# techmum21p/hybrid-rag-ColBERTv2

Measured on AMD Instinct MI355X. Metric: queries/sec + p50 retrieval latency, 1M-chunk corpus, top-10 rerank, higher is better.
Workload: dtype fp32 (faithful: bf16 hi/lo split, fp32 accumulate)

## Files before the change

hybrid-rag-colbertv2_amd/_lib.py:

```python
from __future__ import annotations

import ctypes
import os
import re

PKG = os.path.dirname(os.path.abspath(__file__))
LIB_PATH = os.path.join(PKG, "libcolbert_mi355x.so")
HEADER = os.path.join(os.path.dirname(PKG), "include", "colbert_mi355x.h")

DTYPE_BF16 = 1
DTYPE_F32 = 2
DTYPE_MXFP8 = 3
SCORER_MAXSIM = 0
SCORER_REF_MEANPOOL_COSINE = 1
SCORERS = {"maxsim": SCORER_MAXSIM, "ref_meanpool_cosine": SCORER_REF_MEANPOOL_COSINE}
ERR_EINVAL, ERR_EUNSUPPORTED, ERR_EHIP, ERR_ESTATE = -1, -2, -3, -4
F32_SCORE, F32_SEARCH, F32_RERANK = 0, 1, 2
(OPT_FUSED_TOPK, OPT_DYNAMIC_TAIL, OPT_BAND_DOC_MAJOR, OPT_BAND_LOWER_BOUND, OPT_TOPK_BMAX, OPT_BAND_FUSED,
 OPT_RESCORE_SPLIT, OPT_BAND_REUSE, OPT_BAND_BLOCK_SKIP, OPT_RESCORE_GRID, OPT_DENSE_DOCS, OPT_P1_COLLECT_FUSED,
 OPT_FOLD_KEYS, OPT_FILTER_PATH, OPT_FILTER_BATCH_CHUNK_DOCS, OPT_FILTER_BAND) = (1, 2, 3, 4, 5, 6, 7, 8, 9, 10, 11, 12,
                                                                                 13, 14, 15, 16)
FILTER_AUTO, FILTER_SUBSET, FILTER_DENSE = 0, 1, 2
FILTER_BAND_AUTO, FILTER_BAND_ON, FILTER_BAND_OFF = 0, 1, 2

_p, _i32, _i64, _sz = ctypes.c_void_p, ctypes.c_int32, ctypes.c_int64, ctypes.c_size_t
_SIGS = {
    "cbv2_abi_version": (ctypes.c_int, []),
    "cbv2_last_error": (ctypes.c_char_p, []),
    "cbv2_build_stamp": (ctypes.c_char_p, []),
    "cbv2_index_create": (ctypes.c_int, [ctypes.c_int, _p, _i32, _i64, _i32, _i32, _p, _i64,
                                         ctypes.POINTER(ctypes.c_void_p)]),
    "cbv2_index_destroy": (ctypes.c_int, [_p]),
    "cbv2_hbm_alloc": (ctypes.c_int, [ctypes.c_int, ctypes.c_size_t, ctypes.POINTER(ctypes.c_void_p),
                                      ctypes.POINTER(ctypes.c_int32)]),
    "cbv2_hbm_free": (ctypes.c_int, [ctypes.c_int, _p]),
    "cbv2_index_time_scans": (ctypes.c_int, [_p, _i32]),
    "cbv2_index_scan_times": (ctypes.c_int, [_p, _p, _i32, ctypes.POINTER(ctypes.c_int32)]),
    "cbv2_index_band_times": (ctypes.c_int, [_p, _p, _i32, ctypes.POINTER(ctypes.c_int32)]),
    "cbv2_index_scan_clock": (ctypes.c_int, [_p, _p, _i32]),
    "cbv2_index_create_mxfp8": (ctypes.c_int, [ctypes.c_int, _p, _p, _i64, _i32, _i32, _p, _i64,
                                               ctypes.POINTER(ctypes.c_void_p)]),
    "cbv2_quantize_mxfp8": (ctypes.c_int, [_p, _i32, _i64, _p, _p, _p]),
    "cbv2_index_build_means": (ctypes.c_int, [_p, _p, _i32, _p, _p]),
    "cbv2_score": (ctypes.c_int, [_p, _i32, _p, _i32, _i32, _i32, _p, _i64, _p]),
    "cbv2_search_workspace_bytes": (_sz, [_p, _i32]),
    "cbv2_search_workspace_size": (_sz, [_p, _i32, _i32, _i32]),
    "cbv2_index_set_option": (ctypes.c_int, [_p, _i32, _i64]),
    "cbv2_search_fused_slots": (_i64, [_p, _i32, _i32, _i32]),
    "cbv2_index_last_scan_plan": (ctypes.c_int, [_p, _p]),
    "cbv2_search": (ctypes.c_int, [_p, _i32, _p, _i32, _i32, _i32, _i32, _p, _sz, _p, _p, _p]),
    "cbv2_filter_bytes": (_sz, [_i64]),
    "cbv2_filter_create": (ctypes.c_int, [_p, _p, _p, _sz, _p, ctypes.POINTER(ctypes.c_void_p)]),
    "cbv2_filter_count": (_i64, [_p]),
    "cbv2_filter_destroy": (ctypes.c_int, [_p]),
    "cbv2_search_filtered_workspace_size": (_sz, [_p, _p, _i32, _i32, _i32, _i32]),
    "cbv2_search_filtered": (ctypes.c_int, [_p, _p, _i32, _p, _i32, _i32, _i32, _i32, _p, _sz, _p, _p, _p]),
    "cbv2_search_filtered_f32_workspace_size": (_sz, [_p, _p, _i32, _i32, _i32, _i32]),
    "cbv2_search_filtered_f32": (ctypes.c_int, [_p, _p, _p, _i32, _i32, _i32, _i32, _p, _sz, _p, _p, _p, _p]),
    "cbv2_filter_batch_bytes": (_sz, [_i32]),
    "cbv2_filter_batch_create": (ctypes.c_int, [_p, _p, _i32, _p, _sz, _p, ctypes.POINTER(ctypes.c_void_p)]),
    "cbv2_filter_batch_pairs": (_i64, [_p]),
    "cbv2_filter_batch_max_count": (_i64, [_p]),
    "cbv2_filter_batch_destroy": (ctypes.c_int, [_p]),
    "cbv2_search_filtered_batch_workspace_size": (_sz, [_p, _p, _i32, _i32, _i32, _i32]),
    "cbv2_search_filtered_batch": (ctypes.c_int, [_p, _p, _i32, _p, _i32, _i32, _i32, _i32, _p, _sz, _p, _p, _p]),
    "cbv2_rerank": (ctypes.c_int, [_p, _p, _i32, _i32, _p, _i32, _i32, _p, _p, _p, _p]),
    "cbv2_rerank_workspace_bytes": (_sz, [_i32, _i32]),
    "cbv2_rerank_ws": (ctypes.c_int, [_p, _p, _i32, _i32, _p, _i32, _i32, _p, _sz, _p, _p, _p, _p]),
    "cbv2_select_topk": (ctypes.c_int, [_p, _p, _i32, _i32, _i32, _p, _p, _p, _p]),
    "cbv2_topk_workspace_bytes": (_sz, [_i32, _i64]),
    "cbv2_topk_rows": (ctypes.c_int, [_p, _i32, _i64, _i64, _i32, _i64, _p, _sz, _p, _p, _p]),
    "cbv2_merge_topk": (ctypes.c_int, [_p, _p, _i32, _i32, _i32, _p, _p, _p]),
    "cbv2_rrf_fuse": (ctypes.c_int, [_p, _i32, _p, _i32, _i32, _i32, _i32, _p, _p, _p]),
    "cbv2_bm25_build": (ctypes.c_int, [_p, _p, _i64, _i32, ctypes.c_float, ctypes.c_float,
                                       ctypes.POINTER(ctypes.c_void_p)]),
    "cbv2_bm25_search": (ctypes.c_int, [_p, _p, _p, _i32, _i32, _i32, _p, _p]),
    "cbv2_bm25_search_filtered": (ctypes.c_int, [_p, _p, _p, _i32, _i32, _i32, _p, _p, _p]),
    "cbv2_bm25_search_filtered_batch": (ctypes.c_int, [_p, _p, _p, _i32, _i32, _i32, _p, _p, _p]),
    "cbv2_bm25_doc_freq": (ctypes.c_int, [_p, _p, _i64, _i32, _p]),
    "cbv2_bm25_build_shard": (ctypes.c_int, [_p, _p, _i64, _i32, ctypes.c_float, ctypes.c_float, _i64, _i64,
                                             _i64, _p, ctypes.POINTER(ctypes.c_void_p)]),
    "cbv2_bm25_num_docs": (_i64, [_p]),
    "cbv2_stem_en": (ctypes.c_int, [_p, _p, _i64, _p, _i64, _p]),
    "cbv2_index_file_info": (ctypes.c_int, [ctypes.c_char_p, _p, _p, _p]),
    "cbv2_index_file_write": (ctypes.c_int, [ctypes.c_char_p, _i32, _i64, _p, _p, _p, _i64, _p]),
    "cbv2_index_file_read": (ctypes.c_int, [ctypes.c_char_p, _i64, _i64, _p, _p, _p, _p]),
    "cbv2_index_file_write_host": (ctypes.c_int, [ctypes.c_char_p, _i32, _i64, _p, _p, _p, _i64]),
    "cbv2_index_file_read_host": (ctypes.c_int, [ctypes.c_char_p, _i64, _i64, _p, _p, _p]),
    "cbv2_index_writer_open": (ctypes.c_int, [ctypes.c_char_p, _i32, _i64, _i64, ctypes.POINTER(ctypes.c_void_p)]),
    "cbv2_index_file_info_ld": (ctypes.c_int, [ctypes.c_char_p, _p, _p, _p, _p]),
    "cbv2_index_file_write_ld": (ctypes.c_int, [ctypes.c_char_p, _i32, _i64, _i32, _p, _p, _p, _i64, _p]),
    "cbv2_index_file_write_host_ld": (ctypes.c_int, [ctypes.c_char_p, _i32, _i64, _i32, _p, _p, _p, _i64]),
    "cbv2_index_writer_open_ld": (ctypes.c_int, [ctypes.c_char_p, _i32, _i64, _i32, _i64,
                                                 ctypes.POINTER(ctypes.c_void_p)]),
    "cbv2_index_writer_append": (ctypes.c_int, [_p, _i64, _p, _p, _p, _i32, _p]),
    "cbv2_index_writer_count": (_i64, [_p]),
    "cbv2_index_writer_close": (ctypes.c_int, [_p]),
    "cbv2_comm_init": (ctypes.c_int, [_p, ctypes.c_char_p, ctypes.POINTER(ctypes.c_void_p)]),
    "cbv2_comm_loopback_init": (ctypes.c_int, [_i32, ctypes.POINTER(ctypes.c_void_p)]),
    "cbv2_comm_size": (ctypes.c_int, [_p]),
    "cbv2_comm_rank": (ctypes.c_int, [_p]),
    "cbv2_comm_destroy": (ctypes.c_int, [_p]),
    "cbv2_sharded_workspace_bytes": (_sz, [_p, _p, _i32, _i32, _i32, _i32]),
    "cbv2_search_sharded": (ctypes.c_int, [_p, _p, _i32, _p, _i32, _i32, _i32, _i32, _p, _p, _i32, _p, _sz, _p, _p,
                                           _p, _p]),
    "cbv2_search_sharded_local": (ctypes.c_int, [_p, _p, _i32, _p, _i32, _i32, _i32, _i32, _i32, _p, _sz, _p]),
    "cbv2_search_sharded_exchange": (ctypes.c_int, [_p, _p, _p, _i32, _i32, _i32, _i32, _p, _p, _i32, _p, _sz, _p,
                                                    _p, _p, _p]),
    "cbv2_rerank_sharded": (ctypes.c_int, [_p, _p, _p, _i32, _i32, _p, _i32, _i32, _p, _sz, _p, _p, _p, _p]),
    "cbv2_rerank_sharded_prescored": (ctypes.c_int, [_p, _p, _i32, _i32, _i32, _p, _i32, _i32, _p, _sz, _p, _p, _p,
                                                     _p, _p]),
    "cbv2_comm_stats": (ctypes.c_int, [_p, _p]),
    "cbv2_bm25_destroy": (ctypes.c_int, [_p]),
    "cbv2_split_f32": (ctypes.c_int, [_p, _i64, _i32, _p, _p, _p, _p, _p]),
    "cbv2_index_attach_residual": (ctypes.c_int, [_p, _p, ctypes.c_float, ctypes.c_float]),
    "cbv2_f32_workspace_bytes": (_sz, [_p, _i32, _i32, _i32, _i32]),
    "cbv2_score_f32": (ctypes.c_int, [_p, _p, _i32, _i32, _p, _sz, _p, _i64, _p]),
    "cbv2_search_f32": (ctypes.c_int, [_p, _p, _i32, _i32, _i32, _i32, _p, _sz, _p, _p, _p, _p]),
    "cbv2_search_f32_begin": (ctypes.c_int, [_p, _p, _i32, _i32, _i32, _i32, _p, _sz, _p, _p, _p, _p, _p]),
    "cbv2_search_f32_finish": (ctypes.c_int, [_p, _i32, _i32, _i32, _i32, _p, _sz, _p, _p, _p, _p, _p]),
    "cbv2_rerank_f32": (ctypes.c_int, [_p, _p, _i32, _i32, _p, _i32, _i32, _p, _sz, _p, _p, _p, _p]),
    "cbv2_index_kind": (ctypes.c_int, [_p, ctypes.POINTER(ctypes.c_int32), ctypes.POINTER(ctypes.c_int32)]),
    "cbv2_retrieve_workspace_bytes": (_sz, [_p, _p, _i32, _i32, _i32, _i32, _i32]),
    "cbv2_retrieve_host_bytes": (_sz, [_i32, _i32, _i32, _i32]),
    "cbv2_retrieve_host_marks": (ctypes.c_int, [_p, _i32]),
    "cbv2_retrieve_cancel": (ctypes.c_int, [_p, _p, _p]),
    "cbv2_retrieve_pool_stats": (ctypes.c_int, [_p, _i32]),
    "cbv2_retrieve_begin": (ctypes.c_int, [_p, _p, _p, _i32, _i32, _i32, _i32, _i32, _i32, _p, _sz, _p]),
    "cbv2_retrieve_finish": (ctypes.c_int, [_p, _p, _p, _i32, _i32, _i32, _i32, _p, _p, _i32, _i32, _i32, _i32,
                                            _p, _sz, _p, _sz, _p, _p, _p, _p]),
    "cbv2_retrieve_finish_host": (ctypes.c_int, [_p, _p, _p, _i32, _i32, _i32, _i32, _p, _p, _i32, _i32, _i32,
                                                 _i32, _p, _sz, _p, _sz, _p, _p, _p, _p, _p, _p, _p]),
}

_lib = None


def header_symbols(path: str = HEADER):
    text = open(path).read()
    return sorted(set(re.findall(r"^\s*(?:[\w\s\*]+?)\b(cbv2_\w+)\s*\(", text, re.M)))


def lib():
    global _lib
    if _lib is None:
        from . import _build
        if not os.path.exists(LIB_PATH):
            raise RuntimeError(f"{LIB_PATH} is not built: run `python -c 'import __graft_entry__ as g; g.build()'`")
        want, have = _build.source_stamp(), _build.library_stamp(LIB_PATH)
        if have != want:
            raise RuntimeError(f"{LIB_PATH} was built from other sources (stamp {have}, sources {want}): "
                               "rebuild with `python -c 'import __graft_entry__ as g; g.build()'`")
        L = ctypes.CDLL(LIB_PATH)
        for name, (res, args) in _SIGS.items():
            fn = getattr(L, name)
            fn.restype = res
            fn.argtypes = args
        _lib = L
    return _lib


class Cbv2Error(RuntimeError):
    def __init__(self, code: int, msg: str):
        super().__init__(f"cbv2 error {code}: {msg}")
        self.code = code


def check(rc: int):
    if rc != 0:
        msg = lib().cbv2_last_error().decode(errors="replace")
        if rc == ERR_EINVAL:
            raise ValueError(msg)
        raise Cbv2Error(rc, msg)
    return rc
```

hybrid-rag-colbertv2_amd/csrc/colbert_mi355x.hip:

```cpp
#include <hip/hip_runtime.h>

#include <stdarg.h>
#include <stdint.h>

#include <algorithm>
#include <atomic>
#include <mutex>
#include <type_traits>
#include <vector>
#include <stdio.h>
#include <string.h>

#include "colbert_mi355x.h"

namespace {

constexpr int kDim = 128;
constexpr int kLd = 128;
constexpr int kLqMax = 32;
constexpr int kRowBytes = kDim * 2;
constexpr int kDocBytes = kLd * kRowBytes;
constexpr int kTopkMax = 1024;
constexpr int kSmallMax = 1024;
constexpr int kMergeMax = 8192;
// ... 3407 lines not shown
  const int b = blockIdx.y;
  const int c = blockIdx.x * kRrWaves + wave;
  if (c >= C) return;
  const int32_t id = cand[(size_t)b * C + c];
  float v;
  if constexpr (F8) {
    i32x8 qa[1][2];
    int qs[1][2];
    load_qfrag_f8(Qb, Qs, b, b + 1, lq, lane, qa[0], qs[0]);
    v = rerank_one_f8(tokens, tscales, doclens, n, id_base, qa, qs, lq, id, lane, ld);
  } else {
    bf16x8 qf[1][2][4];
    load_qfrag16(reinterpret_cast<const uint16_t*>(Qb), b, b + 1, lq, lane, qf[0]);
    v = rerank_one_bf16(tokens, doclens, n, id_base, qf, lq, id, lane, ld);
  }
  if (lane == 0) raw[(size_t)b * C + c] = v;
}

__global__ __launch_bounds__(256, 2) void rerank_split_kernel(
    const uint8_t* __restrict__ tokens, const int32_t* __restrict__ doclens, int64_t n, int64_t id_base,
    const uint16_t* __restrict__ Q, int lq, const int32_t* __restrict__ cand, int C, float* __restrict__ raw, int ld,
    TaggedCand tc = TaggedCand(), Mirror raw_words = Mirror()) {
  __shared__ float s_m[4][32];
  __shared__ int32_t s_cid;
  const int lane = threadIdx.x & 63, g = lane >> 4, c16 = lane & 15;
  const int wave = __builtin_amdgcn_readfirstlane(threadIdx.x >> 6);
  const int b = blockIdx.y, c = blockIdx.x;
  int32_t id;
  if (tc.w != nullptr) {
    if (threadIdx.x == 0) s_cid = wait_tagged(tc.w + (size_t)b * C + c, tc);
    __syncthreads();
    id = s_cid;
  } else {
    id = cand[(size_t)b * C + c];
  }
  const int64_t loc = (int64_t)id - id_base;
  if (id < 0 || loc < 0 || loc >= n) {
    if (threadIdx.x == 0) {
      raw[(size_t)b * C + c] = neg_inf();
      if (raw_words.w != nullptr) raw_words.put((size_t)b * C + c, (int32_t)__float_as_uint(neg_inf()), 0.0f);
    }
    return;
  }
  bf16x8 qf[1][2][4];
  load_qfrag16(Q, b, b + 1, lq, lane, qf[0]);
  int dl = doclens[loc];
  float m[1][2] = {{neg_inf(), neg_inf()}};
  for (int blk = 0; blk == 0 || kLd * blk < dl; ++blk) {
    const uint8_t* dbase = tokens + (size_t)loc * (size_t)ld * kRowBytes + (size_t)blk * kDocBytes;
    bf16x8 af[2][4];
#pragma unroll
    for (int t = 0; t < 2; ++t)
      if (blk == 0 || 16 * (2 * wave + t) < dl - kLd * blk) gbl_afrag16(dbase, 2 * wave + t, lane, af[t]);
    if (blk == 0) dl = dl < 0 ? 0 : (dl > ld ? ld : dl);
    const int dlb = dl - kLd * blk;
#pragma unroll
    for (int t = 0; t < 2; ++t) {
      const int rt = 2 * wave + t;
      if (16 * rt < dlb) {
        const f32x4 init = (dlb >= 16 * rt + 16) ? f32x4{} : row_mask_init16(16 * rt + 4 * g, dlb);
        tile16<1>(af[t], qf, init, m);
      }
    }
  }
  const float w0 = fold16_max(fold32_max(m[0][0])), w1 = fold16_max(fold32_max(m[0][1]));
  if (lane < 16) {
    s_m[wave][lane] = w0;
    s_m[wave][16 + lane] = w1;
  }
  __syncthreads();
  if (wave == 0) {
    const float m0 = fmaxf(fmaxf(s_m[0][c16], s_m[1][c16]), fmaxf(s_m[2][c16], s_m[3][c16]));
    const float m1 = fmaxf(fmaxf(s_m[0][16 + c16], s_m[1][16 + c16]), fmaxf(s_m[2][16 + c16], s_m[3][16 + c16]));
    const float v = dpp_row_sum16((c16 < lq ? m0 : 0.0f) + (16 + c16 < lq ? m1 : 0.0f));
    if (lane == 0) {
      raw[(size_t)b * C + c] = v;
      if (raw_words.w != nullptr) raw_words.put((size_t)b * C + c, (int32_t)__float_as_uint(v), 0.0f);
    }
  }
}

constexpr float kBoundUp = 1.0f + 1.0f / 1024.0f;
constexpr float kAccSlack = 1.0f / 4096.0f;

__device__ __forceinline__ void split_row8(const float* __restrict__ src, uint16_t* __restrict__ hi,
                                           uint16_t* __restrict__ lo, int sub, float& xx, float& rr, float& hh) {
  const f32x4* s4 = reinterpret_cast<const f32x4*>(src + 8 * sub);
  const f32x4 v0 = s4[0], v1 = s4[1];
  float x[8] = {v0[0], v0[1], v0[2], v0[3], v1[0], v1[1], v1[2], v1[3]};
  uint16_t h[8], l[8];
  xx = rr = hh = 0.0f;
#pragma unroll
  for (int e = 0; e < 8; ++e) {
    const __bf16 bh = (__bf16)x[e];
    const float fh = (float)bh;
    const float r = x[e] - fh;
    const __bf16 bl = (__bf16)r;
    h[e] = __builtin_bit_cast(uint16_t, bh);
    l[e] = __builtin_bit_cast(uint16_t, bl);
    xx += x[e] * x[e];
    rr += r * r;
    hh += fh * fh;
  }
  u32x4 ph, pl;
#pragma unroll
  for (int e = 0; e < 4; ++e) {
    ph[e] = (uint32_t)h[2 * e] | ((uint32_t)h[2 * e + 1] << 16);
    pl[e] = (uint32_t)l[2 * e] | ((uint32_t)l[2 * e + 1] << 16);
  }
  *reinterpret_cast<u32x4*>(hi + 8 * sub) = ph;
  *reinterpret_cast<u32x4*>(lo + 8 * sub) = pl;
#pragma unroll
  for (int off = 1; off < 16; off <<= 1) {
    xx += __shfl_xor(xx, off);
    rr += __shfl_xor(rr, off);
    hh += __shfl_xor(hh, off);
  }
}

__global__ __launch_bounds__(256) void split_f32_kernel(const float* __restrict__ x, int64_t rows, int ld,
                                                        const int32_t* __restrict__ doclens,
                                                        uint16_t* __restrict__ hi, uint16_t* __restrict__ lo,
                                                        float* __restrict__ bounds) {
  const int sub = threadIdx.x & 15;
  float rmax = 0.0f, hmax = 0.0f;
  for (int64_t r = ((int64_t)blockIdx.x * blockDim.x + threadIdx.x) >> 4; r < rows;
       r += ((int64_t)gridDim.x * blockDim.x) >> 4) {
    float xx, rr, hh;
    split_row8(x + r * kDim, hi + r * kDim, lo + r * kDim, sub, xx, rr, hh);
    if (doclens == nullptr || (int)(r % ld) < doclens[r / ld]) {
      rmax = fmaxf(rmax, sqrtf(rr) * kBoundUp);
      hmax = fmaxf(hmax, sqrtf(hh) * kBoundUp);
    }
  }
#pragma unroll
  for (int off = 16; off < 64; off <<= 1) {
    rmax = fmaxf(rmax, __shfl_xor(rmax, off));
    hmax = fmaxf(hmax, __shfl_xor(hmax, off));
  }
  if ((threadIdx.x & 63) == 0) {
    atomicMax(reinterpret_cast<unsigned int*>(bounds), __float_as_uint(rmax));
    atomicMax(reinterpret_cast<unsigned int*>(bounds) + 1, __float_as_uint(hmax));
  }
}

constexpr int kArriveSlotsK = 4;
constexpr int kArrPhase1K = 3;
constexpr int64_t kSplitZeroInts = 16384;
__global__ __launch_bounds__(512) void split_query_kernel(const float* __restrict__ Q, int lq,
                                                          uint16_t* __restrict__ qhi, uint16_t* __restrict__ qlo,
                                                          float E, float M, float* __restrict__ beta,
                                                          int32_t* __restrict__ count = nullptr,
                                                          uint32_t* __restrict__ lbu = nullptr,
                                                          int32_t* __restrict__ done = nullptr, int count0 = 0,
                                                          int32_t* __restrict__ arrive = nullptr, int narrive = 0,
                                                          int* __restrict__ ctr = nullptr, int nctr = 0,
                                                          uint32_t ready_seq = 0, int nrows = 0,
                                                          uint32_t* __restrict__ zkeys = nullptr, int64_t nz = 0,
                                                          int32_t* __restrict__ ready_words = nullptr) {
  __shared__ float s_t[kLqMax];
  const int b = blockIdx.x, tid = threadIdx.x, r = tid >> 4, sub = tid & 15;
  if (nrows > 0 && b >= nrows) {
    const int64_t per = kSplitZeroInts, i0 = (int64_t)(b - nrows) * per;
    for (int64_t i = i0 + 4 * tid; i < i0 + per && i < nz; i += 4 * blockDim.x) {
      if (i + 3 < nz)
        *reinterpret_cast<uint4*>(zkeys + i) = make_uint4(0u, 0u, 0u, 0u);
      else
        for (int64_t e = i; e < nz; ++e) zkeys[e] = 0u;
    }
    return;
  }
  if (r < lq) {
    const size_t row = (size_t)b * lq + r;
    float xx, rr, hh;
    split_row8(Q + row * kDim, qhi + row * kDim, qlo + row * kDim, sub, xx, rr, hh);
    const float nq = sqrtf(xx) * kBoundUp, eq = sqrtf(rr) * kBoundUp;
    const float t = nq * E + eq * M + kAccSlack * (nq + eq) * M;
    if (sub == 0) s_t[r] = t;
  }
  __syncthreads();
  if (tid == 0) {
    float a[4];
#pragma unroll
    for (int g = 0; g < 4; ++g) {
      a[g] = 0.0f;
      for (int rr = g; rr < lq; rr += 4) a[g] += s_t[rr];
    }
    beta[b] = ((a[0] + a[1]) + (a[2] + a[3])) * kBoundUp;
    if (count != nullptr) count[b] = count0;
    if (lbu != nullptr) lbu[b] = 0xffffffffu;
    if (done != nullptr) done[b] = 0;
  }
  if (arrive != nullptr) {
    const int per = narrive / kArriveSlotsK;
    for (int i = tid; i < narrive; i += blockDim.x) {
      const int j = i / per, e = i - j * per;
      arrive[((size_t)j * nrows + b) * per + e] = 0;
    }
  }
  if (ctr != nullptr && b == 0)
    for (int i = tid; i < nctr; i += blockDim.x) ctr[i] = 0;
  if (ready_seq != 0 && ready_words != nullptr) {
    __syncthreads();
    if (tid == 0) {
      __threadfence();
      asm volatile("s_waitcnt vmcnt(0)" ::: "memory");
      __hip_atomic_store(ready_words + b, (int32_t)ready_seq, __ATOMIC_RELAXED, __HIP_MEMORY_SCOPE_SYSTEM);
    }
  }
}

__device__ __forceinline__ void tile16_x3(const bf16x8 (&ah)[4], const bf16x8 (&al)[4], const bf16x8 (&qh)[2][4],
                                          const bf16x8 (&ql)[2][4], const f32x4& init, float (&m)[2]) {
#pragma unroll
  for (int ct = 0; ct < 2; ++ct) {
    f32x4 acc = init;
#pragma unroll
    for (int s = 0; s < 4; ++s) acc = __builtin_amdgcn_mfma_f32_16x16x32_bf16(al[s], qh[ct][s], acc, 0, 0, 0);
#pragma unroll
    for (int s = 0; s < 4; ++s) acc = __builtin_amdgcn_mfma_f32_16x16x32_bf16(ah[s], ql[ct][s], acc, 0, 0, 0);
#pragma unroll
    for (int s = 0; s < 4; ++s) acc = __builtin_amdgcn_mfma_f32_16x16x32_bf16(ah[s], qh[ct][s], acc, 0, 0, 0);
    m[ct] = fmaxf(fmaxf(m[ct], fmaxf(acc[0], acc[1])), fmaxf(acc[2], acc[3]));
  }
}

template <bool LONG>
__device__ __forceinline__ float faithful_doc16(const uint8_t* __restrict__ hi, const uint8_t* __restrict__ lo,
                                                int64_t loc, int ld, int dl, const bf16x8 (&qh)[2][4],
                                                const bf16x8 (&ql)[2][4], int lane, int lq) {
  const int g = lane >> 4;
  const int lmax = LONG ? ld : kLd;
  float m[2] = {neg_inf(), neg_inf()};
  for (int blk = 0; blk == 0 || (LONG && kLd * blk < dl); ++blk) {
    const int dlb = dl - kLd * blk;
    const size_t at = ((size_t)loc * lmax + (size_t)kLd * blk) * kRowBytes;
    const uint8_t* dh = hi + at;
    const uint8_t* dlo = lo + at;
#pragma unroll
    for (int half = 0; half < 2; ++half) {
      bf16x8 ah[4][4], al[4][4];
#pragma unroll
      for (int t = 0; t < 4; ++t) {
        const int rt = 4 * half + t;
        if (16 * rt < dlb) {
          gbl_afrag16(dh, rt, lane, ah[t]);
          gbl_afrag16(dlo, rt, lane, al[t]);
        }
      }
#pragma unroll
      for (int t = 0; t < 4; ++t) {
        const int rt = 4 * half + t;
        if (16 * rt < dlb) {
          const f32x4 init = (dlb >= 16 * rt + 16) ? f32x4{} : row_mask_init16(16 * rt + 4 * g, dlb);
          tile16_x3(ah[t], al[t], qh, ql, init, m);
        }
      }
    }
  }
  return reduce16(m[0], m[1], lane, lq);
}

constexpr int kRsPerWave = 4;
template <bool LONG = false>
__global__ __launch_bounds__(256, 2) void rescore_x3_kernel(
    const uint8_t* __restrict__ hi, const uint8_t* __restrict__ lo, const int32_t* __restrict__ doclens, int64_t n,
    int64_t id_base, const uint16_t* __restrict__ qhi, const uint16_t* __restrict__ qlo, int lq,
    const int32_t* __restrict__ cand, const int32_t* __restrict__ count, int64_t limit, int64_t ld_c,
    float* __restrict__ out, int64_t ld_out, const int32_t* __restrict__ only_neg, int ld, int pw,
    uint32_t* __restrict__ lb_min) {
  const int lane = threadIdx.x & 63;
  const int wave = __builtin_amdgcn_readfirstlane(threadIdx.x >> 6);
  const int b = blockIdx.y;
  if (only_neg != nullptr && only_neg[b] >= 0) return;
  int64_t lim = limit;
  if (count != nullptr) {
    const int64_t cb = count[b];
    lim = cb < lim ? cb : lim;
  }
  const int64_t step = (int64_t)gridDim.x * 4 * pw;
  int64_t c0 = ((int64_t)blockIdx.x * 4 + wave) * pw;
  if (c0 >= lim) return;
  bf16x8 qh[2][4], ql[2][4];
  load_qfrag16(qhi, b, b + 1, lq, lane, qh);
  load_qfrag16(qlo, b, b + 1, lq, lane, ql);
  for (; c0 < lim; c0 += step)
  for (int64_t c = c0; c < c0 + pw && c < lim; ++c) {
    const int64_t id = cand ? (int64_t)cand[b * ld_c + c] : id_base + c;
    const int64_t loc = id - id_base;
    float v = neg_inf();
    if (id >= 0 && loc >= 0 && loc < n) {
      const int lmax = LONG ? ld : kLd;
      int dl = doclens[loc];
      dl = dl < 0 ? 0 : (dl > lmax ? lmax : dl);
      v = faithful_doc16<LONG>(hi, lo, loc, ld, dl, qh, ql, lane, lq);
    }
    if (lane == 0) {
      out[(size_t)b * ld_out + c] = v;
      if (lb_min != nullptr) atomicMin(lb_min + b, f2u(v));
    }
  }
}

template <bool LONG, int NW = 4>
__device__ __forceinline__ float faithful_doc_split(const uint8_t* __restrict__ hi, const uint8_t* __restrict__ lo,
                                                    int64_t loc, int ld, int dl, const bf16x8 (&qh)[2][4],
                                                    const bf16x8 (&ql)[2][4], int lane, int wave, int lq,
                                                    float (&s_m)[4][32]) {
  constexpr int TPW = 8 / NW;
  const int g = lane >> 4, c16 = lane & 15;
  const int lmax = LONG ? ld : kLd;
  float m[2] = {neg_inf(), neg_inf()};
  for (int blk = 0; blk == 0 || (LONG && kLd * blk < dl); ++blk) {
    const size_t at = ((size_t)loc * lmax + (size_t)kLd * blk) * kRowBytes;
    bf16x8 ah[TPW][4], al[TPW][4];
#pragma unroll
    for (int t = 0; t < TPW; ++t) {
      const int rt = TPW * wave + t;
      if (blk == 0 || 16 * rt < dl - kLd * blk) {
        gbl_afrag16(hi + at, rt, lane, ah[t]);
        gbl_afrag16(lo + at, rt, lane, al[t]);
      }
    }
    if (blk == 0) dl = dl < 0 ? 0 : (dl > lmax ? lmax : dl);
    const int dlb = dl - kLd * blk;
#pragma unroll
    for (int t = 0; t < TPW; ++t) {
      const int rt = TPW * wave + t;
      if (16 * rt < dlb) {
        const f32x4 init = (dlb >= 16 * rt + 16) ? f32x4{} : row_mask_init16(16 * rt + 4 * g, dlb);
        tile16_x3(ah[t], al[t], qh, ql, init, m);
      }
    }
  }
  const float w0 = fold16_max(fold32_max(m[0])), w1 = fold16_max(fold32_max(m[1]));
  if (lane < 16) {
    s_m[wave][lane] = w0;
    s_m[wave][16 + lane] = w1;
  }
  __syncthreads();
  float v = 0.0f;
  if (wave == 0) {
    float m0 = s_m[0][c16], m1 = s_m[0][16 + c16];
#pragma unroll
    for (int w = 1; w < NW; ++w) {
      m0 = fmaxf(m0, s_m[w][c16]);
      m1 = fmaxf(m1, s_m[w][16 + c16]);
    }
    v = dpp_row_sum16((c16 < lq ? m0 : 0.0f) + (16 + c16 < lq ? m1 : 0.0f));
  }
  __syncthreads();
  return v;
}

struct RowSelect {
  int mode = 0;
  int32_t* arrive = nullptr;
  int k = 0;
  float* out_s = nullptr;
  int32_t* out_i = nullptr;
  int32_t* out_p = nullptr;
  const float* lb = nullptr;
  const uint32_t* lbu = nullptr;
  int32_t* status = nullptr;
  Mirror ids_mirror;
  FinalMirror fin;
  Mirror raw;
  uint64_t* stamps = nullptr;
};
constexpr int kSelNone = 0, kSelCand = 1, kSelBand = 2;

__device__ void select_cand_row(const float* raw, const int32_t* crow, int C, int k, float* os, int32_t* oi,
                                int32_t* op, float* sc, uint64_t* keys, FinalMirror fin = FinalMirror(),
                                size_t b = 0) {
  for (int t = threadIdx.x; t < C; t += blockDim.x) {
    sc[t] = ld_sc1(raw + t);
    keys[t] = rank_key(sc[t], (uint32_t)t);
  }
  __syncthreads();
  select_from_lds(sc, keys, C, k, crow, os, oi, op, fin, b);
}

__device__ void select_band_row(const float* F, const int32_t* cand, int cnt, int k, int64_t id_base, bool has_lb,
                                float lbv, float* os, int32_t* oi, uint64_t* sel, uint32_t* hist, uint32_t* misc,
                                Mirror mirror) {
  const int tid = threadIdx.x, nth = blockDim.x, wave = tid >> 6;
  const int kk = k < cnt ? k : cnt;
  auto key_at = [&](int i) { return rank_key(ld_sc1(F + i), (uint32_t)((int64_t)cand[i] - id_base)); };
  if (tid < 8) misc[tid] = 0;
  __syncthreads();
  const uint32_t ulb = has_lb ? f2u(lbv) : 0u;
  constexpr int U = 8;
  for (int i0 = tid; i0 < cnt; i0 += nth * U) {
    uint64_t kv[U];
#pragma unroll
    for (int u = 0; u < U; ++u) kv[u] = i0 + u * nth < cnt ? key_at(i0 + u * nth) : 0ull;
#pragma unroll
    for (int u = 0; u < U; ++u)
      if (i0 + u * nth < cnt && (uint32_t)(kv[u] >> 32) >= ulb) {
        const uint32_t pos = atomicAdd(&misc[0], 1u);
        if (pos < (uint32_t)kTopkMax) sel[pos] = kv[u];
      }
  }
  __syncthreads();
  int m = (int)misc[0];
  __syncthreads();
  if (m < kk || m > kTopkMax) {
    const int shifts[6] = {53, 42, 32, 21, 10, 0};
    const int bits[6] = {11, 11, 10, 11, 11, 10};
    uint64_t prefix = 0, mask = 0;
    uint32_t kleft = (uint32_t)kk;
    for (int p = 0; p < 6; ++p) {
      const int nb = 1 << bits[p];
      for (int i = tid; i < nb; i += nth) hist[i] = 0;
      __syncthreads();
      for (int i = tid; i < cnt; i += nth) {
        const uint64_t key = key_at(i);
        hist_add(hist, (uint32_t)(key >> shifts[p]) & (uint32_t)(nb - 1), (key & mask) == prefix);
      }
      __syncthreads();
      if (wave == 0) find_bin(hist, nb, kleft, &misc[4], &misc[5], &misc[6]);
      __syncthreads();
      kleft -= misc[5];
      prefix |= (uint64_t)misc[4] << shifts[p];
      mask |= (uint64_t)(nb - 1) << shifts[p];
      __syncthreads();
    }
    if (tid == 0) misc[0] = 0;
    __syncthreads();
    for (int i = tid; i < cnt; i += nth) {
      const uint64_t key = key_at(i);
      if (key >= prefix) {
        const uint32_t pos = atomicAdd(&misc[0], 1u);
        if (pos < (uint32_t)kTopkMax) sel[pos] = key;
      }
    }
    __syncthreads();
    m = kk;
  }
  for (int i = tid; i < m; i += nth) {
    const uint64_t key = sel[i];
    int r = 0;
    for (int j = 0; j < m; ++j) r += sel[j] > key ? 1 : 0;
    if (r < k) {
      os[r] = u2f((uint32_t)(key >> 32));
      oi[r] = (int32_t)(id_base + (int64_t)(~(uint32_t)key));
      if (mirror.w != nullptr) mirror.put(r, oi[r], os[r]);
    }
  }
  for (int j = m + tid; j < k; j += nth) {
    os[j] = neg_inf();
    oi[j] = -1;
    if (mirror.w != nullptr) mirror.put(j, -1, neg_inf());
  }
}

template <bool LONG = false, int NW = 4>
__global__ __launch_bounds__(NW * 64, 2) void rescore_split_kernel(
    const uint8_t* __restrict__ hi, const uint8_t* __restrict__ lo, const int32_t* __restrict__ doclens, int64_t n,
    int64_t id_base, const uint16_t* __restrict__ qhi, const uint16_t* __restrict__ qlo, int lq,
    const int32_t* __restrict__ cand, const int32_t* __restrict__ count, int64_t limit, int64_t ld_c,
    float* __restrict__ out, int64_t ld_out, const int32_t* __restrict__ only_neg, int ld,
    uint32_t* __restrict__ lb_min, int64_t c0, float* __restrict__ fb_T = nullptr, int32_t* __restrict__ fb_done = nullptr,
    int fb_k = 0, float* __restrict__ fb_s = nullptr, int32_t* __restrict__ fb_i = nullptr, RowSelect rs = RowSelect(),
    TaggedCand tc = TaggedCand()) {
  __shared__ float s_m[4][32];
  __shared__ uint64_t sel[kTopkMax];
  __shared__ uint32_t hist[2048];
  __shared__ uint32_t s_bin, s_above, s_bincount, s_cnt;
  __shared__ uint32_t misc[8];
  __shared__ int s_last;
  __shared__ int32_t s_cid;
  const int lane = threadIdx.x & 63;
  const int wave = __builtin_amdgcn_readfirstlane(threadIdx.x >> 6);
  const int b = blockIdx.y;
  if (rs.stamps != nullptr && threadIdx.x == 0 && blockIdx.x < kLabWgs)
    rs.stamps[16 + 2 * blockIdx.x] = __builtin_amdgcn_s_memrealtime();
  if (only_neg != nullptr && only_neg[b] >= 0) return;
  int64_t lim = limit;
  if (count != nullptr) {
    const int64_t cb = count[b];
    lim = cb < lim ? cb : lim;
    if (fb_T != nullptr && cb > limit) {
      bf16x8 qh[2][4], ql[2][4];
      load_qfrag16(qhi, b, b + 1, lq, lane, qh);
      load_qfrag16(qlo, b, b + 1, lq, lane, ql);
      float* row = fb_T + (size_t)b * n;
      for (int64_t c = blockIdx.x; c < n; c += gridDim.x) {
        const float v = faithful_doc_split<LONG, NW>(hi, lo, c, ld, doclens[c], qh, ql, lane, wave, lq, s_m);
        if (threadIdx.x == 0) row[c] = v;
      }
      __threadfence();
      __syncthreads();
      if (threadIdx.x == 0) s_last = atomicAdd(fb_done + b, 1) == (int)gridDim.x - 1;
      __syncthreads();
      if (!s_last) return;
      __threadfence();
      const int kk = (int)((int64_t)fb_k < n ? fb_k : n);
      topk_exact_row(row, n, kk, sel, hist, &s_bin, &s_above, &s_bincount, &s_cnt);
      sort_and_write(sel, kk, fb_k, id_base, fb_s + (size_t)b * fb_k, fb_i + (size_t)b * fb_k,
                     rs.ids_mirror.row(b, fb_k));
      if (rs.mode == kSelBand && threadIdx.x == 0) rs.status[b] = cb >= kWaitTimedOut ? -2 : -1;
      return;
    }
  }
  const bool idle = c0 + (int64_t)blockIdx.x >= lim;
  if (idle && rs.mode == kSelNone) return;
  if (!idle) {
    bf16x8 qh[2][4], ql[2][4];
    load_qfrag16(qhi, b, b + 1, lq, lane, qh);
    load_qfrag16(qlo, b, b + 1, lq, lane, ql);
    for (int64_t c = c0 + blockIdx.x; c < lim; c += gridDim.x) {
      int64_t id;
      if (tc.w != nullptr) {
        if (threadIdx.x == 0) {
          s_cid = wait_tagged(tc.w + (size_t)b * ld_c + c, tc);
          if (rs.mode != kSelNone)
            st_sc1(reinterpret_cast<uint32_t*>(const_cast<int32_t*>(cand)) + (size_t)b * ld_c + c, (uint32_t)s_cid);
        }
        __syncthreads();
        id = s_cid;
        __syncthreads();
      } else {
        id = cand ? (int64_t)cand[b * ld_c + c] : id_base + c;
      }
      const int64_t loc = id - id_base;
      float v = neg_inf();
      if (id >= 0 && loc >= 0 && loc < n)
        v = faithful_doc_split<LONG, NW>(hi, lo, loc, ld, doclens[loc], qh, ql, lane, wave, lq, s_m);
      if (threadIdx.x == 0) {
        if (rs.mode != kSelNone)
          st_sc1(out + (size_t)b * ld_out + c, v);
        else
          out[(size_t)b * ld_out + c] = v;
        if (rs.raw.w != nullptr) rs.raw.put((size_t)b * ld_c + c, (int32_t)__float_as_uint(v), 0.0f);
        if (lb_min != nullptr) atomicMin(lb_min + b, f2u(v));
      }
    }
  }
  if (rs.stamps != nullptr && threadIdx.x == 0 && blockIdx.x < kLabWgs)
    rs.stamps[17 + 2 * blockIdx.x] = __builtin_amdgcn_s_memrealtime();
  if (rs.mode == kSelNone) return;
  if (!row_last_arrival(rs.arrive + (size_t)b * kArriveInts, (int)gridDim.x, 8, &s_last)) return;
  lab_stamp(rs.stamps, 6);
  if (rs.mode == kSelCand) {
    const int32_t* crow = cand + (size_t)b * ld_c;
    if (tc.w != nullptr) {
      int32_t* ids_lds = reinterpret_cast<int32_t*>(hist) + kSmallMax;
      for (int t = threadIdx.x; t < (int)limit; t += blockDim.x)
        ids_lds[t] = (int32_t)ld_sc1(reinterpret_cast<const uint32_t*>(crow) + t);
      crow = ids_lds;
    }
    select_cand_row(out + (size_t)b * ld_out, crow, (int)limit, rs.k, rs.out_s + (size_t)b * rs.k,
                    rs.out_i + (size_t)b * rs.k, rs.out_p ? rs.out_p + (size_t)b * rs.k : nullptr,
                    reinterpret_cast<float*>(hist), sel, rs.fin, (size_t)b);
  } else {
    const bool has_lb = rs.lb != nullptr || rs.lbu != nullptr;
    const float lbv = rs.lbu != nullptr ? u2f(rs.lbu[b]) : (rs.lb != nullptr ? rs.lb[b] : 0.0f);
    select_band_row(out + (size_t)b * ld_out, cand + (size_t)b * ld_c, (int)lim, rs.k, id_base, has_lb, lbv,
                    rs.out_s + (size_t)b * rs.k, rs.out_i + (size_t)b * rs.k, sel, hist, misc,
                    rs.ids_mirror.row(b, rs.k));
    if (threadIdx.x == 0) rs.status[b] = (int32_t)lim;
  }
  if (rs.stamps != nullptr) {
    __syncthreads();
    lab_stamp(rs.stamps, 4);
    if (threadIdx.x == 0) rs.stamps[5] = (uint64_t)lim;
  }
}

template <bool LONG = false>
__global__ __launch_bounds__(256, 2) void fallback_split_kernel(
    const uint8_t* __restrict__ hi, const uint8_t* __restrict__ lo, const int32_t* __restrict__ doclens, int64_t n,
    int64_t id_base, const uint16_t* __restrict__ qhi, const uint16_t* __restrict__ qlo, int lq,
    float* __restrict__ T, const int32_t* __restrict__ status, int ld, int32_t* __restrict__ done, int k,
    float* __restrict__ out_s, int32_t* __restrict__ out_i) {
  __shared__ float s_m[4][32];
  __shared__ uint64_t sel[kTopkMax];
  __shared__ uint32_t hist[2048];
  __shared__ uint32_t s_bin, s_above, s_bincount, s_cnt;
  __shared__ int s_last;
  const int lane = threadIdx.x & 63;
  const int wave = __builtin_amdgcn_readfirstlane(threadIdx.x >> 6);
  const int b = blockIdx.y;
  if (status[b] >= 0) return;
  bf16x8 qh[2][4], ql[2][4];
  load_qfrag16(qhi, b, b + 1, lq, lane, qh);
  load_qfrag16(qlo, b, b + 1, lq, lane, ql);
  float* row = T + (size_t)b * n;
  for (int64_t c = blockIdx.x; c < n; c += gridDim.x) {
    const float v = faithful_doc_split<LONG>(hi, lo, c, ld, doclens[c], qh, ql, lane, wave, lq, s_m);
    if (threadIdx.x == 0) row[c] = v;
  }
  __threadfence();
  __syncthreads();
  if (threadIdx.x == 0) s_last = atomicAdd(done + b, 1) == (int)gridDim.x - 1;
  __syncthreads();
  if (!s_last) return;
  __threadfence();
  const int kk = (int)((int64_t)k < n ? k : n);
  topk_exact_row(row, n, kk, sel, hist, &s_bin, &s_above, &s_bincount, &s_cnt);
  sort_and_write(sel, kk, k, id_base, out_s + (size_t)b * k, out_i + (size_t)b * k);
}

__global__ __launch_bounds__(256) void band_count_kernel(const int32_t* __restrict__ cand,
                                                         const int32_t* __restrict__ count, int cap,
                                                         int64_t id_base, int64_t n, int32_t* __restrict__ dcnt,
                                                         int c0) {
  const int b = blockIdx.y;
  const int tot = count[b];
  if (tot > cap) return;
  for (int c = c0 + blockIdx.x * blockDim.x + threadIdx.x; c < tot; c += gridDim.x * blockDim.x) {
    const int64_t d = (int64_t)cand[(size_t)b * cap + c] - id_base;
    if (d >= 0 && d < n) atomicAdd(dcnt + d, 1);
  }
}

__global__ __launch_bounds__(256) void band_offsets_kernel(const int32_t* __restrict__ dcnt, int64_t n,
                                                           int32_t* __restrict__ doff, int32_t* __restrict__ act,
                                                           int32_t* __restrict__ act_off,
                                                           int32_t* __restrict__ act_cnt, int32_t* __restrict__ ctr) {
// ... 237 lines not shown
      }
      const float w0 = fold16_max(fold32_max(m[0])), w1 = fold16_max(fold32_max(m[1]));
      if (lane < 16) {
        s_m[wave][lane] = w0;
        s_m[wave][16 + lane] = w1;
      }
      __syncthreads();
      if (wave == 0) {
        float m0 = s_m[0][c16], m1 = s_m[0][16 + c16];
#pragma unroll
        for (int w = 1; w < NW; ++w) {
          m0 = fmaxf(m0, s_m[w][c16]);
          m1 = fmaxf(m1, s_m[w][16 + c16]);
        }
        const float v = dpp_row_sum16((c16 < lq ? m0 : 0.0f) + (16 + c16 < lq ? m1 : 0.0f));
        if (lane == 0) F[(size_t)b * cap + pair_c[o + p]] = v;
      }
      __syncthreads();
    }
    d = d_next;
  }
}

__device__ __forceinline__ float band_threshold(int b, const float* __restrict__ lb, const uint32_t* __restrict__ lbu,
                                                const float* __restrict__ topk_s, int k,
                                                const float* __restrict__ beta) {
  if (lbu != nullptr) return u2f(lbu[b]) - beta[b];
  if (lb != nullptr) return lb[b] - beta[b];
  return topk_s[(size_t)b * k + k - 1] - 2.0f * beta[b];
}

constexpr int kBandLds = 2048;
__global__ __launch_bounds__(256) void band_collect_kernel(const float* __restrict__ T, int64_t n,
                                                           const float* __restrict__ topk_s, int k,
                                                           const float* __restrict__ beta, int64_t id_base,
                                                           int cap, int32_t* __restrict__ cand,
                                                           int32_t* __restrict__ count,
                                                           const float* __restrict__ lb,
                                                           const uint32_t* __restrict__ lbu,
                                                           const int32_t* __restrict__ topk_i,
                                                           const uint32_t* __restrict__ bm,
                                                           uint64_t* __restrict__ stamps = nullptr) {
  __shared__ int32_t s_ids[kBandLds];
  __shared__ int s_n, s_base;
  const int b = blockIdx.y, lane = threadIdx.x & 63;
  if (stamps != nullptr && threadIdx.x == 0 && blockIdx.x < kLabWgs)
    stamps[16 + 2 * blockIdx.x] = __builtin_amdgcn_s_memrealtime();
  if (threadIdx.x == 0) s_n = 0;
  __syncthreads();
  const float thr = band_threshold(b, lb, lbu, topk_s, k, beta);
  const float* row = T + (size_t)b * n;
  int32_t* crow = cand + (size_t)b * cap;
  uint64_t kth = 0;
  if (topk_i != nullptr) {
    kth = rank_key(topk_s[(size_t)b * k + k - 1], (uint32_t)((int64_t)topk_i[(size_t)b * k + k - 1] - id_base));
    if (blockIdx.x == 0)
      for (int j = threadIdx.x; j < k; j += blockDim.x) crow[j] = topk_i[(size_t)b * k + j];
  }
  auto offer = [&](int64_t i, float v) {
    const bool take = i < n && v >= thr && (topk_i == nullptr || rank_key(v, (uint32_t)i) < kth);
    const uint64_t mask = __ballot(take);
    if (mask == 0) return;
    const int nh = __popcll(mask);
    int base = 0;
    if (lane == 0) base = atomicAdd(&s_n, nh);
    base = __shfl(base, 0);
    const int pos = base + __popcll(mask & ((1ull << lane) - 1ull));
    if (take) {
      if (pos < kBandLds) {
        s_ids[pos] = (int32_t)(id_base + i);
      } else {
        const int gp = atomicAdd(count + b, 1);
        if (gp < cap) crow[gp] = (int32_t)(id_base + i);
      }
    }
  };
  if (bm != nullptr) {
    const int64_t nb = (n + 63) >> 6;
    const uint32_t* krow = bm + (size_t)b * nb;
    const uint32_t uthr = f2u(thr);
    const int wave = threadIdx.x >> 6, nw = blockDim.x >> 6;
    const int c16 = lane & 15, r4 = lane >> 4;
    const bool vec = (n & 3) == 0 && (reinterpret_cast<uintptr_t>(T) & 15) == 0;
    for (int64_t g0 = (int64_t)blockIdx.x * 64; g0 < nb; g0 += (int64_t)gridDim.x * 64) {
      const int64_t kb = g0 + lane;
      const uint64_t qual = __ballot(kb < nb && krow[kb] >= uthr);
      uint64_t mine = 0;
      int q = 0;
      for (uint64_t m = qual; m != 0; m &= m - 1, ++q)
        if (q % nw == wave) mine |= m & (~m + 1);
      while (mine != 0) {
        int64_t i0[4];
#pragma unroll
        for (int s4 = 0; s4 < 4; ++s4) {
          int64_t blk = -1;
#pragma unroll
          for (int u = 0; u < 4; ++u) {
            const int64_t bu = mine != 0 ? g0 + (__ffsll((long long)mine) - 1) : -1;
            if (mine != 0) mine &= mine - 1;
            if (u == r4) blk = bu;
          }
          i0[s4] = blk >= 0 ? (blk << 6) + 4 * c16 : n;
        }
        float v[4][4];
#pragma unroll
        for (int s4 = 0; s4 < 4; ++s4) {
          if (vec && i0[s4] + 3 < n) {
            const f32x4 x4 = *reinterpret_cast<const f32x4*>(row + i0[s4]);
            v[s4][0] = x4[0], v[s4][1] = x4[1], v[s4][2] = x4[2], v[s4][3] = x4[3];
          } else {
#pragma unroll
            for (int e = 0; e < 4; ++e) v[s4][e] = i0[s4] + e < n ? row[i0[s4] + e] : 0.0f;
          }
        }
#pragma unroll
        for (int s4 = 0; s4 < 4; ++s4)
#pragma unroll
          for (int e = 0; e < 4; ++e) offer(i0[s4] + e < n ? i0[s4] + e : n, v[s4][e]);
      }
    }
  } else {
    constexpr int U = 8;
    const int64_t step = (int64_t)gridDim.x * blockDim.x * U;
    for (int64_t i0 = (int64_t)blockIdx.x * blockDim.x * U; i0 < n; i0 += step) {
      float v[U];
#pragma unroll
      for (int u = 0; u < U; ++u) {
        const int64_t i = i0 + (int64_t)u * blockDim.x + threadIdx.x;
        v[u] = i < n ? row[i] : 0.0f;
      }
#pragma unroll
      for (int u = 0; u < U; ++u) offer(i0 + (int64_t)u * blockDim.x + threadIdx.x, v[u]);
    }
  }
  __syncthreads();
  const int nl = s_n < kBandLds ? s_n : kBandLds;
  if (threadIdx.x == 0) s_base = nl > 0 ? atomicAdd(count + b, nl) : 0;
  __syncthreads();
  for (int t = threadIdx.x; t < nl; t += blockDim.x)
    if (s_base + t < cap) crow[s_base + t] = s_ids[t];
  if (stamps != nullptr && threadIdx.x == 0 && blockIdx.x < kLabWgs) {
    stamps[17 + 2 * blockIdx.x] = __builtin_amdgcn_s_memrealtime();
    atomicAdd(reinterpret_cast<unsigned long long*>(stamps + 5), (unsigned long long)s_n);
  }
}

constexpr int kP1Replicas = 8;
static_assert(32 * kP1Replicas <= kArriveInts, "done1's replicas fit one arrival slot");
__global__ __launch_bounds__(256, 2) void phase1_collect_kernel(
    const uint8_t* __restrict__ hi, const uint8_t* __restrict__ lo, const int32_t* __restrict__ doclens, int64_t n,
    int64_t id_base, const uint16_t* __restrict__ qhi, const uint16_t* __restrict__ qlo, int lq,
    const int32_t* __restrict__ topk_i, const float* __restrict__ topk_s, int k, float* __restrict__ F,
    int64_t ld_F, uint32_t* __restrict__ lbu, int32_t* __restrict__ done1, int64_t done_ld,
    const float* __restrict__ T, const float* __restrict__ beta, const uint32_t* __restrict__ bm, int cap,
    int32_t* __restrict__ cand, int32_t* __restrict__ count, uint64_t wait_ticks,
    uint64_t* __restrict__ stamps = nullptr) {
  __shared__ float s_m[4][32];
  __shared__ int32_t s_ids[kBandLds];
  __shared__ int s_n, s_base, s_timed_out;
  __shared__ uint32_t s_lb;
  const int lane = threadIdx.x & 63;
  const int wave = __builtin_amdgcn_readfirstlane(threadIdx.x >> 6);
  const int b = blockIdx.y;
  const int x = blockIdx.x;
  if (stamps != nullptr && threadIdx.x == 0 && x < kLabWgs) stamps[16 + 2 * x] = __builtin_amdgcn_s_memrealtime();
  if (x < k) {
    bf16x8 qh[2][4], ql[2][4];
    load_qfrag16(qhi, b, b + 1, lq, lane, qh);
    load_qfrag16(qlo, b, b + 1, lq, lane, ql);
    const int64_t id = topk_i[(size_t)b * k + x];
    const int64_t loc = id - id_base;
    float v = neg_inf();
    if (id >= 0 && loc >= 0 && loc < n)
// ... 358 lines not shown
  const size_t doc = blockIdx.x;
  const int d = threadIdx.x;
  int dl = doclens[doc];
  dl = dl < 0 ? 0 : (dl > ld_src ? ld_src : dl);
  float s = 0.0f;
  for (int t = 0; t < dl; ++t) s += tok[(doc * ld_src + t) * kDim + d];
  const float mean = dl > 0 ? s / (float)dl : 0.0f;
  float sq = mean * mean;
  for (int off = 32; off > 0; off >>= 1) sq += __shfl_xor(sq, off);
  if ((threadIdx.x & 63) == 0) red[threadIdx.x >> 6] = sq;
  __syncthreads();
  const float nrm = sqrtf(red[0] + red[1]);
  means[doc * kDim + d] = mean / fmaxf(nrm, 1e-8f);
}

constexpr int kMpDocs = 64, kMpQ = 16;
__global__ __launch_bounds__(256) void meanpool_scores_kernel(const float* __restrict__ means, int64_t n,
                                                              const float* __restrict__ Q, int B, int lq,
                                                              float* __restrict__ out, int64_t ld_out) {
  __shared__ float qn[kMpQ][kDim];
  __shared__ float dm[kMpDocs][kDim + 1];
  const int tid = threadIdx.x;
  const int64_t doc0 = (int64_t)blockIdx.x * kMpDocs;
  const int q0 = blockIdx.y * kMpQ;
  {
    const int qq = tid >> 4, part = tid & 15;
    const int qi = q0 + qq;
    float mv[8];
    float sq = 0.0f;
#pragma unroll
    for (int j = 0; j < 8; ++j) {
      float s = 0.0f;
      if (qi < B)
        for (int t = 0; t < lq; ++t) s += Q[((size_t)qi * lq + t) * kDim + part * 8 + j];
      mv[j] = s / (float)lq;
      sq += mv[j] * mv[j];
    }
    for (int off = 8; off > 0; off >>= 1) sq += __shfl_xor(sq, off);
    const float inv = 1.0f / fmaxf(sqrtf(sq), 1e-8f);
#pragma unroll
    for (int j = 0; j < 8; ++j) qn[qq][part * 8 + j] = mv[j] * inv;
  }
  for (int e = tid; e < kMpDocs * kDim; e += 256) {
    const int dd = e / kDim, c = e % kDim;
    dm[dd][c] = (doc0 + dd < n) ? means[(size_t)(doc0 + dd) * kDim + c] : 0.0f;
  }
  __syncthreads();
  const int dd = tid & 63;
#pragma unroll
  for (int j = 0; j < 4; ++j) {
    const int qq = (tid >> 6) * 4 + j;
    float s = 0.0f;
    for (int c = 0; c < kDim; ++c) s += qn[qq][c] * dm[dd][c];
    if (q0 + qq < B && doc0 + dd < n) out[(size_t)(q0 + qq) * ld_out + doc0 + dd] = s;
  }
}

}

struct cbv2_index {
  int device;
  const uint8_t* tokens;
  int64_t n;
  int32_t ld, d;
  const int32_t* doclens;
  int64_t id_base;
  const float* doc_means;
  int32_t dtype;
  const uint8_t* scales;
  int* task_ring = nullptr;
  uint32_t task_seq = 0;
  hipEvent_t ring_ev[128] = {};
  bool ring_ev_used[128] = {};
  int64_t last_plan[4] = {0, 0, 0, 0};
  bool fused_topk = false;
  int fused_topk_mode = 0;
  int dynamic_tail = 1;
  int topk_bmax = 1;
  int band_doc_major = 0;
  bool band_lower_bound = true;
  bool band_fused = false;
  bool rescore_split = true;
  bool band_reuse = true;
  bool band_block_skip = true;
  int rescore_grid = 0;
  bool dense_docs = false;
  bool p1_collect_fused = true;
  bool fold_keys = true;
  std::mutex mu;
  const uint8_t* resid = nullptr;
  float resid_max = 0.0f, norm_max = 0.0f;
  bool time_scans = false;
  uint64_t* clk = nullptr;
  bool clock_on = false;
  size_t scan_ev_used = 0;
  std::vector<hipEvent_t> scan_ev;
  size_t band_ev_used = 0;
  bool band_open = false;
  std::vector<hipEvent_t> band_ev;
  int filter_path = 0;
  int filter_band = 0;
  int64_t filter_batch_chunk_docs = 0;
};

struct cbv2_filter {
  int device = 0;
  int64_t n = 0, id_base = 0;
  int64_t m = 0;
  const int32_t* ids = nullptr;
};

struct cbv2_filter_batch {
  int device = 0;
  int64_t n = 0, id_base = 0;
  int32_t B = 0;
  int64_t pairs = 0, max_m = 0;
  int64_t chunk_docs = 1;
  int64_t chunks = 0;
  const int32_t* table = nullptr;
};

namespace {
thread_local char g_err[512] = "";

int fail(int code, const char* fmt, ...) {
  va_list ap;
  va_start(ap, fmt);
  vsnprintf(g_err, sizeof(g_err), fmt, ap);
  va_end(ap);
  return code;
}

#define CBV2_HIP(call)                                                                    \
  do {                                                                                    \
    hipError_t e_ = (call);                                                               \
    if (e_ != hipSuccess) return fail(CBV2_EHIP, "%s: %s", #call, hipGetErrorString(e_)); \
  } while (0)

#define CBV2_REQUIRE(cond, ...) \
  do {                          \
    if (!(cond)) return fail(CBV2_EINVAL, __VA_ARGS__); \
  } while (0)

struct DeviceGuard {
  int prev = -1;
  bool ok = true;
  explicit DeviceGuard(int dev) {
    if (hipGetDevice(&prev) != hipSuccess) { ok = false; return; }
    if (prev != dev && hipSetDevice(dev) != hipSuccess) ok = false;
  }
  ~DeviceGuard() {
    int cur = -1;
    if (prev >= 0 && hipGetDevice(&cur) == hipSuccess && cur != prev) (void)hipSetDevice(prev);
  }
};

constexpr int kRingSlots = 128;
constexpr int kTailSlices = 8;
constexpr int kRingInts = 64 * kTailSlices;
constexpr size_t kCtrBytes = kRingInts * sizeof(int);

void alloc_task_ring(cbv2_index* ix) {
  if (ix->n == 0) return;
  int prev = 0;
  if (hipGetDevice(&prev) != hipSuccess || hipSetDevice(ix->device) != hipSuccess) return;
  void* p = nullptr;
// ... 713 lines not shown
      ix->band_ev.push_back(e);
    }
    CBV2_HIP(hipEventRecord(ix->band_ev[2 * i], st));
    ix->band_open = true;
    return CBV2_OK;
  }
  if (!ix->band_open) return CBV2_OK;
  CBV2_HIP(hipEventRecord(ix->band_ev[2 * i + 1], st));
  ix->band_open = false;
  ++ix->band_ev_used;
  return CBV2_OK;
}

int score_impl(cbv2_index* ix, int32_t scorer, const void* Q, int32_t B, int32_t lq, float* out,
               int64_t ld_out, hipStream_t st, int* ctr_ws = nullptr) {
  if (scorer == CBV2_SCORER_MAXSIM) return scan_maxsim_timed(ix, Q, B, lq, out, ld_out, st, ctr_ws);
  return scan_meanpool(ix, (const float*)Q, B, lq, out, ld_out, st);
}

__global__ void fill_neg_inf_kernel(float* x, int64_t n) {
  const int64_t i = (int64_t)blockIdx.x * blockDim.x + threadIdx.x;
  if (i < n) x[i] = neg_inf();
}

__global__ void fill_empty_kernel(float* out_s, int32_t* out_i, int64_t total) {
  const int64_t i = (int64_t)blockIdx.x * blockDim.x + threadIdx.x;
  if (i < total) {
    out_s[i] = neg_inf();
    out_i[i] = -1;
  }
}

int topk_impl_empty(int32_t B, int32_t k, float* out_s, int32_t* out_i, hipStream_t st) {
  const int64_t total = (int64_t)B * k;
  hipLaunchKernelGGL(fill_empty_kernel, dim3((unsigned)((total + 255) / 256)), dim3(256), 0, st, out_s, out_i, total);
  return launch_check("fill_empty_kernel");
}

size_t topk_ws_bytes(int32_t B, int64_t n) {
  if (n < kSampledMinN) return 0;
  return (size_t)B * kCandCap * sizeof(uint64_t) + (((size_t)B * sizeof(uint32_t) + 255) & ~(size_t)255);
}

int topk_multi(const float* scores, int32_t B, int64_t n, int64_t ld, int32_t k, int64_t id_base,
               const int32_t* ids, int64_t ids_ld, float* out_s, int32_t* out_i, int32_t* out_p, hipStream_t st,
               const int32_t* only_neg = nullptr) {
  hipLaunchKernelGGL(topk_multi_kernel, dim3((unsigned)B), dim3(kTkThreads), 0, st, scores, n, ld, k, id_base, ids,
                     ids_ld, out_s, out_i, out_p, only_neg);
  return launch_check("topk_multi_kernel");
}

int topk_impl(const float* scores, int32_t B, int64_t n, int64_t ld, int32_t k, int64_t id_base, void* ws,
              size_t ws_bytes, float* out_s, int32_t* out_i, hipStream_t st, int dev) {
  if (k > kTopkMax) return topk_multi(scores, B, n, ld, k, id_base, nullptr, 0, out_s, out_i, nullptr, st);
  const size_t need = topk_ws_bytes(B, n);
  if (need == 0 || ws == nullptr || ws_bytes < need || B > 65535) {
    const Mirror mirror = g_ids_mirror;
    if (mirror.w != nullptr) g_ids_mirror_used = true;
    hipLaunchKernelGGL(topk_rows_kernel, dim3((unsigned)B), dim3(kTkThreads), 0, st, scores, n, ld, k, id_base,
                       out_s, out_i, nullptr, mirror);
    return launch_check("topk_rows_kernel");
  }
  uint64_t* cand = (uint64_t*)ws;
  uint32_t* cnt = (uint32_t*)((uint8_t*)ws + (size_t)B * kCandCap * sizeof(uint64_t));
  CBV2_HIP(hipMemsetAsync(cnt, 0, (size_t)B * sizeof(uint32_t), st));
  int64_t splits = (2LL * cu_count(dev) + B - 1) / B;
  const int64_t max_splits = n / 16384;
  if (splits > max_splits) splits = max_splits;
  if (splits < 1) splits = 1;
  hipLaunchKernelGGL(topk_filter_kernel, dim3((unsigned)splits, (unsigned)B), dim3(256), 0, st, scores, n, ld, k, cnt,
                     cand);
  int rc = launch_check("topk_filter_kernel");
  if (rc) return rc;
  hipLaunchKernelGGL(topk_select_kernel, dim3((unsigned)B), dim3(kTkThreads), 0, st, scores, n, ld, k, id_base, cnt,
                     cand, out_s, out_i);
  return launch_check("topk_select_kernel");
}

struct F32Ws {
  int* ctr = nullptr;
  uint16_t* qhi = nullptr;
  uint16_t* qlo = nullptr;
  float* beta = nullptr;
  float* lb = nullptr;
  int32_t* count = nullptr;
  int32_t* done = nullptr;
  int32_t* arrive = nullptr;
  int32_t* cand = nullptr;
  float* F = nullptr;
  void* tk = nullptr;
  size_t tk_bytes = 0;
  float* T = nullptr;
  int32_t* dcnt = nullptr;
  int32_t* doff = nullptr;
  int32_t* act = nullptr;
  int32_t* act_off = nullptr;
  int32_t* act_cnt = nullptr;
  int32_t* dctr = nullptr;
  int32_t* pair_b = nullptr;
  int32_t* pair_c = nullptr;
};

constexpr int kArriveSlots = kArriveSlotsK;
constexpr int kArrBmax = 0, kArrBand = 1, kArrRerank = 2, kArrPhase1 = kArrPhase1K;
inline int32_t* arrive_row0(const F32Ws& w, int slot, int B) { return w.arrive + (size_t)slot * B * kArriveInts; }

size_t f32_ws_layout(const cbv2_index* ix, int op, int B, int lq, int cap, uint8_t* base, F32Ws* w) {
  size_t off = 0;
  auto take = [&](size_t bytes) -> uint8_t* {
    uint8_t* p = base ? base + off : nullptr;
    off += (bytes + 255) & ~(size_t)255;
    return p;
  };
  const size_t qbytes = (size_t)B * lq * kDim * sizeof(uint16_t);
  if (op == CBV2_F32_SEARCH) w->ctr = (int*)take(kCtrBytes);
  w->qhi = (uint16_t*)take(qbytes);
  w->qlo = (uint16_t*)take(qbytes);
  w->beta = (float*)take((size_t)B * sizeof(float));
  if (op == CBV2_F32_SEARCH) w->lb = (float*)take((size_t)B * sizeof(float));
  if (op == CBV2_F32_RERANK) w->F = (float*)take((size_t)B * cap * sizeof(float));
  if (op != CBV2_F32_SCORE) w->arrive = (int32_t*)take((size_t)kArriveSlots * B * kArriveInts * sizeof(int32_t));
  if (op == CBV2_F32_SEARCH) {
    w->count = (int32_t*)take((size_t)B * sizeof(int32_t));
    w->done = (int32_t*)take((size_t)B * sizeof(int32_t));
    w->cand = (int32_t*)take((size_t)B * cap * sizeof(int32_t));
    w->F = (float*)take((size_t)B * cap * sizeof(float));
    w->tk_bytes = std::max(topk_ws_bytes(B, ix->n), bm_ws_bytes(B, ix->n));
    w->tk = take(w->tk_bytes);
    w->T = (float*)take((size_t)B * (size_t)(ix->n > 0 ? ix->n : 1) * sizeof(float));
    const size_t nd = (size_t)(ix->n > 0 ? ix->n : 1) * sizeof(int32_t);
    w->dcnt = (int32_t*)take(nd);
    w->doff = (int32_t*)take(nd);
    w->act = (int32_t*)take(nd);
    w->act_off = (int32_t*)take(nd);
    w->act_cnt = (int32_t*)take(nd);
    w->dctr = (int32_t*)take(2 * sizeof(int32_t));
    w->pair_b = (int32_t*)take((size_t)B * cap * sizeof(int32_t));
    w->pair_c = (int32_t*)take((size_t)B * cap * sizeof(int32_t));
  }
  return off;
}

int check_f32(cbv2_index* ix, int op, const float* Q, int32_t B, int32_t lq, int32_t cap, void* ws, size_t wsb,
              F32Ws* w) {
  CBV2_REQUIRE(ix != nullptr, "null index");
  if (ix->resid == nullptr) return fail(CBV2_ESTATE, "index has no fp32 residual (cbv2_index_attach_residual)");
  CBV2_REQUIRE(Q != nullptr && aligned16(Q), "query pointer must be non-null and 16-byte aligned");
  CBV2_REQUIRE(B >= 1 && B <= 65535, "B must be in [1, 65535] (got %d)", B);
  CBV2_REQUIRE(lq >= 1 && lq <= kLqMax, "lq must be in [1, %d] (got %d)", kLqMax, lq);
  const size_t need = f32_ws_layout(ix, op, B, lq, cap, nullptr, w);
  CBV2_REQUIRE(ws != nullptr && wsb >= need && aligned16(ws), "workspace too small or misaligned (%zu < %zu)",
               wsb, need);
  f32_ws_layout(ix, op, B, lq, cap, (uint8_t*)ws, w);
  return CBV2_OK;
}

struct SplitTag {
  const void* qhi = nullptr;
  const cbv2_index* ix = nullptr;
  const float* Q = nullptr;
  int B = 0, lq = 0;
};
constexpr int kSplitTags = 64;
std::mutex g_split_mu;
SplitTag g_split_tags[kSplitTags];
int g_split_next = 0;

void note_split(const cbv2_index* ix, const float* Q, int B, int lq, const void* qhi) {
  std::lock_guard<std::mutex> lk(g_split_mu);
  int slot = -1;
  for (int i = 0; i < kSplitTags && slot < 0; ++i)
    if (g_split_tags[i].qhi == qhi) slot = i;
  if (slot < 0) slot = g_split_next++ % kSplitTags;
  g_split_tags[slot] = SplitTag{qhi, ix, Q, B, lq};
}

bool split_holds(const cbv2_index* ix, const float* Q, int B, int lq, const void* qhi) {
  std::lock_guard<std::mutex> lk(g_split_mu);
  for (int i = 0; i < kSplitTags; ++i) {
    const SplitTag& t = g_split_tags[i];
    if (t.qhi == qhi) return t.ix == ix && t.Q == Q && t.B == B && t.lq == lq;
  }
  return false;
}

int split_queries(cbv2_index* ix, const float* Q, int B, int lq, F32Ws* w, hipStream_t st, int count0 = 0,
                  bool zero_ctr = false, uint32_t* zkeys = nullptr, int64_t nz = 0) {
  note_split(ix, Q, B, lq, w->qhi);
  const int64_t extra = zkeys != nullptr ? (nz + kSplitZeroInts - 1) / kSplitZeroInts : 0;
  const bool publish = g_split_ready_seq != 0 && g_split_ready_word != nullptr;
  if (publish) {
    g_ready_flag = g_split_ready_word;
    g_ready_flag_ld = 1;
  }
  hipLaunchKernelGGL(split_query_kernel, dim3((unsigned)(B + extra)), dim3(512), 0, st, Q, lq, w->qhi, w->qlo,
                     ix->resid_max, ix->norm_max, w->beta, w->count, reinterpret_cast<uint32_t*>(w->lb), w->done,
                     count0, w->arrive, kArriveSlots * kArriveInts, zero_ctr ? w->ctr : nullptr,
                     zero_ctr ? kRingInts : 0, publish ? g_split_ready_seq : 0u, B, zkeys, nz,
                     publish ? g_split_ready_word : nullptr);
  return launch_check("split_query_kernel");
}

constexpr int64_t kRsSmallPairs = 4096;
constexpr int64_t kRsSplitGrid = 1024;
struct RescoreGrid { unsigned gx; bool two; };
RescoreGrid rescore_grid(const cbv2_index* ix, int B, int64_t span) {
  const int64_t grid_auto = std::min<int64_t>(kRsSplitGrid, std::max<int64_t>(256, 4096 / std::max(B, 1)));
  const int64_t grid_max = ix->rescore_grid > 0 ? ix->rescore_grid : grid_auto;
  const unsigned gx = (unsigned)(span < grid_max ? span : grid_max);
  return {gx, ix->ld == kLd && (int64_t)gx * B > 3LL * cu_count(ix->device)};
}
int launch_rescore(cbv2_index* ix, const F32Ws* w, int B, int lq, const int32_t* cand, const int32_t* count,
                   int64_t limit, int64_t ld_c, float* out, int64_t ld_out, hipStream_t st,
                   const int32_t* only_neg = nullptr, int pw = 0, uint32_t* lb_min = nullptr, int64_t c0 = 0,
                   float* fb_T = nullptr, int32_t* fb_done = nullptr, int fb_k = 0, float* fb_s = nullptr,
                   int32_t* fb_i = nullptr, const RowSelect& rs = RowSelect(), TaggedCand tc = TaggedCand()) {
  if (limit <= c0 && fb_T == nullptr && rs.mode == kSelNone) return CBV2_OK;
  if (ix->rescore_split) {
    int64_t span = limit - c0;
    if (fb_T != nullptr) span = std::max<int64_t>(span, std::min<int64_t>(ix->n, 256));
    if (span < 1) span = 1;
    const auto [gx, two] = rescore_grid(ix, B, span);
    auto kern = ix->ld != kLd ? rescore_split_kernel<true, 4>
                              : (two ? rescore_split_kernel<false, 2> : rescore_split_kernel<false, 4>);
    hipLaunchKernelGGL(kern, dim3(gx, (unsigned)B), dim3(two ? 128 : 256), 0, st, ix->tokens, ix->resid, ix->doclens,
                       ix->n, ix->id_base, w->qhi, w->qlo, lq, cand, count, limit, ld_c, out, ld_out, only_neg,
                       (int)ix->ld, lb_min, c0, fb_T, fb_done, fb_k, fb_s, fb_i, rs, tc);
    return launch_check("rescore_split_kernel");
  }
  if (c0 != 0 || fb_T != nullptr || rs.mode != kSelNone || tc.w != nullptr)
    return fail(CBV2_EUNSUPPORTED, "pair offset / fallback / row select need the split rescoring");
  if (pw <= 0) pw = (int64_t)B * limit <= kRsSmallPairs ? 1 : kRsPerWave;
  const int64_t per_wg = 4LL * pw;
  int64_t gx = (limit + per_wg - 1) / per_wg;
  gx = gx < 1024 ? gx : 1024;
  hipLaunchKernelGGL(ix->ld != kLd ? rescore_x3_kernel<true> : rescore_x3_kernel<false>, dim3((unsigned)gx, (unsigned)B),
                     dim3(256), 0, st, ix->tokens, ix->resid,
                     ix->doclens, ix->n, ix->id_base, w->qhi, w->qlo, lq, cand, count, limit, ld_c, out, ld_out,
                     only_neg, (int)ix->ld, pw, lb_min);
  return launch_check("rescore_x3_kernel");
}

constexpr int kFltWords = 256;

__device__ __forceinline__ uint32_t filter_word(const uint32_t* __restrict__ allow, int64_t w, int64_t n) {
  const int64_t nw = (n + 31) >> 5;
  if (w >= nw) return 0u;
  uint32_t v = allow[w];
  if (w == nw - 1 && (n & 31) != 0) v &= (1u << (n & 31)) - 1u;
  return v;
}

__device__ __forceinline__ int block_scan256(int v, int* s) {
  s[threadIdx.x] = v;
  __syncthreads();
  for (int d = 1; d < 256; d <<= 1) {
    const int t = (int)threadIdx.x >= d ? s[threadIdx.x - d] : 0;
    __syncthreads();
    s[threadIdx.x] += t;
    __syncthreads();
  }
  return s[threadIdx.x];
}

__global__ __launch_bounds__(kFltWords) void filter_count_kernel(const uint32_t* __restrict__ allow, int64_t n,
                                                                 int32_t* __restrict__ blk) {
  __shared__ int s[256];
  const int c = __popc(filter_word(allow, (int64_t)blockIdx.x * kFltWords + threadIdx.x, n));
  const int incl = block_scan256(c, s);
  if (threadIdx.x == 255) blk[blockIdx.x] = incl;
}

__global__ __launch_bounds__(256) void filter_offsets_kernel(const int32_t* __restrict__ blk, int64_t nblk,
                                                             int32_t* __restrict__ off, int32_t* __restrict__ total) {
  __shared__ int s[256];
  __shared__ int carry;
  if (threadIdx.x == 0) carry = 0;
  __syncthreads();
  for (int64_t base = 0; base < nblk; base += 256) {
    const int64_t i = base + threadIdx.x;
    const int v = i < nblk ? blk[i] : 0;
    const int incl = block_scan256(v, s);
    const int c = carry;
    if (i < nblk) off[i] = c + incl - v;
    __syncthreads();
    if (threadIdx.x == 255) carry = c + incl;
    __syncthreads();
  }
  if (threadIdx.x == 0) *total = carry;
}

__global__ __launch_bounds__(kFltWords) void filter_scatter_kernel(const uint32_t* __restrict__ allow, int64_t n,
                                                                   const int32_t* __restrict__ off,
                                                                   int32_t* __restrict__ ids) {
  __shared__ int s[256];
  const int64_t w = (int64_t)blockIdx.x * kFltWords + threadIdx.x;
  uint32_t v = filter_word(allow, w, n);
  const int c = __popc(v);
  int64_t pos = (int64_t)off[blockIdx.x] + block_scan256(c, s) - c;
  while (v != 0u) {
    const int b = __ffs((int)v) - 1;
    if (pos < n) ids[pos] = (int32_t)(w * 32 + b);
    ++pos;
    v &= v - 1u;
  }
}

__global__ __launch_bounds__(256) void filter_gather_kernel(const float* __restrict__ dense, int64_t ld,
                                                            const int32_t* __restrict__ ids, int64_t m, int B,
                                                            float* __restrict__ row) {
// ... 62 lines not shown
  constexpr int U = 8;
  const int64_t step = (int64_t)gridDim.x * blockDim.x * U;
  for (int64_t p0 = (int64_t)blockIdx.x * blockDim.x * U; p0 < m; p0 += step) {
    float v[U];
#pragma unroll
    for (int u = 0; u < U; ++u) {
      const int64_t p = p0 + (int64_t)u * blockDim.x + threadIdx.x;
      v[u] = p < m ? row[p] : 0.0f;
    }
#pragma unroll
    for (int u = 0; u < U; ++u) offer(p0 + (int64_t)u * blockDim.x + threadIdx.x, v[u]);
  }
  __syncthreads();
  const int nl = s_n < kBandLds ? s_n : kBandLds;
  if (threadIdx.x == 0) s_base = nl > 0 ? atomicAdd(count + b, nl) : 0;
  __syncthreads();
  for (int t = threadIdx.x; t < nl; t += blockDim.x)
    if (s_base + t < cap) crow[s_base + t] = s_ids[t];
}

size_t filter_buf_layout(int64_t n, size_t* off_blk, size_t* off_off, size_t* off_total) {
  auto r256 = [](size_t b) { return (b + 255) & ~(size_t)255; };
  const int64_t nn = n > 0 ? n : 1;
  const int64_t nblk = ((nn + 31) / 32 + kFltWords - 1) / kFltWords;
  size_t off = r256((size_t)nn * sizeof(int32_t));
  if (off_blk) *off_blk = off;
  off += r256((size_t)nblk * sizeof(int32_t));
  if (off_off) *off_off = off;
  off += r256((size_t)nblk * sizeof(int32_t));
  if (off_total) *off_total = off;
  return off + 256;
}

template <int QW>
int launch_stream_ids(cbv2_index* ix, const cbv2_filter* f, const uint16_t* Q, int B, int lq, float* out,
                      hipStream_t st) {
  const int64_t m = f->m;
  const int nq_groups = (B + QW - 1) / QW;
  const auto [n_chunks, chunk_docs] = chunk_split(m, 4LL * cu_count(ix->device) * kDirectOversub, nq_groups);
  const int64_t grid = ((int64_t)nq_groups * n_chunks + 3) / 4;
  if (grid > 0x7fffffff) return fail(CBV2_EUNSUPPORTED, "scan grid too large");
  constexpr StreamCfg C{.qw = QW, .aux = 2, .idx = true};
  hipLaunchKernelGGL(maxsim_scan_stream_kernel<C>, dim3((unsigned)grid), dim3(256), 0, st, ix->tokens, ix->doclens, m,
                     Q, B, lq, out, m, chunk_docs, (int)ix->ld, (uint32_t*)nullptr, (int64_t)0, (uint32_t*)nullptr,
                     (int64_t)0, f->ids);
  return launch_check("maxsim_scan_stream_kernel (subset)");
}

template <Scan16x4Cfg C, int PER_CU>
int launch_scan16x4_ids(cbv2_index* ix, const cbv2_filter* f, const uint16_t* Q, int B, int lq, float* out,
                        hipStream_t st) {
  constexpr int QPB = C.waves * C.qw;
  const int64_t m = f->m;
  const int nq_groups = (B + QPB - 1) / QPB;
  const auto [n_chunks, chunk_docs] = chunk_split(m, (int64_t)PER_CU * cu_count(ix->device), nq_groups);
  if ((int64_t)nq_groups * n_chunks > 0x7fffffff) return fail(CBV2_EUNSUPPORTED, "scan grid too large");
  hipLaunchKernelGGL(maxsim_scan16x4_kernel<with_idx(C)>, dim3((unsigned)(nq_groups * n_chunks)), dim3(C.waves * 64),
                     0, st, ix->tokens, ix->doclens, m, Q, B, lq, out, m, chunk_docs, m, (int*)nullptr,
                     0, (uint64_t*)nullptr, 0, (uint64_t*)nullptr, 0, 1, (uint32_t*)nullptr, (int64_t)0,
                     (uint32_t*)nullptr, (int64_t)0, f->ids);
  return launch_check("maxsim_scan16x4_kernel (subset)");
}

int scan_maxsim_subset(cbv2_index* ix, const cbv2_filter* f, const uint16_t* Q, int B, int lq, float* out,
                       hipStream_t st) {
  if (B <= kDirectMaxB)
    return B == 1 ? launch_stream_ids<1>(ix, f, Q, B, lq, out, st) : launch_stream_ids<2>(ix, f, Q, B, lq, out, st);
  switch (pick_shape(kBf16Shapes, B)) {
    case kScan16x4W4Q1: return launch_scan16x4_ids<kW4Q1, 2>(ix, f, Q, B, lq, out, st);
    case kScan16x4W4Q2: return launch_scan16x4_ids<kW4Q2, 2>(ix, f, Q, B, lq, out, st);
    case kScan16x4W4: return launch_scan16x4_ids<kW4, 2>(ix, f, Q, B, lq, out, st);
    default: return launch_scan16x4_ids<kW8, 1>(ix, f, Q, B, lq, out, st);
  }
}

int rescore_subset(cbv2_index* ix, const cbv2_filter* f, const F32Ws* w, int B, int lq, float* out, hipStream_t st,
                   const int32_t* only_neg = nullptr) {
  const int64_t span = only_neg != nullptr ? std::min<int64_t>(f->m, std::max<int64_t>(64, 256 / B)) : f->m;
  const auto [gx, two] = rescore_grid(ix, B, span);
  auto kern = two ? rescore_split_kernel<false, 2> : rescore_split_kernel<false, 4>;
  hipLaunchKernelGGL(kern, dim3(gx, (unsigned)B), dim3(two ? 128 : 256), 0, st, ix->tokens, ix->resid, ix->doclens,
                     ix->n, (int64_t)0, w->qhi, w->qlo, lq, f->ids, (const int32_t*)nullptr, f->m, (int64_t)0, out,
                     f->m, only_neg, (int)ix->ld, (uint32_t*)nullptr, (int64_t)0, (float*)nullptr,
                     (int32_t*)nullptr, 0, (float*)nullptr, (int32_t*)nullptr, RowSelect(), TaggedCand());
  return launch_check("rescore_split_kernel (subset)");
}

constexpr double kFilterSubsetMaxFrac = 0.5;
bool filter_takes_subset(const cbv2_index* ix, int64_t m_allowed, int32_t scorer) {
  const bool supported = scorer == CBV2_SCORER_MAXSIM && ix->dtype == CBV2_DTYPE_BF16 && ix->ld == kLd;
  return supported && (ix->filter_path == 1 ||
                       (ix->filter_path == 0 && (double)m_allowed <= kFilterSubsetMaxFrac * (double)ix->n));
}

constexpr int64_t kFilterBandMinSavedPairs = 4000;
constexpr int64_t kFilterBandSavedPairsPerK = 16;
enum { kFfDense = 0, kFfPair = 1, kFfBand = 2 };
int filter_f32_mode(const cbv2_index* ix, int64_t m, int32_t B, int32_t k) {
  if (!filter_takes_subset(ix, m, CBV2_SCORER_MAXSIM)) return kFfDense;
  if (m <= k || k > kBandCapMax || !ix->rescore_split || ix->filter_band == 2) return kFfPair;
  if (ix->filter_band == 1) return kFfBand;
  return (int64_t)B * (m - 2LL * k) >= kFilterBandMinSavedPairs + kFilterBandSavedPairsPerK * k ? kFfBand : kFfPair;
}

struct FilterF32Ws {
  F32Ws w;
  int32_t* status = nullptr;
  float* tks = nullptr;
  int32_t* pos = nullptr;
  float* dense = nullptr;
};
size_t filter_f32_layout(const cbv2_index* ix, int64_t m_allowed, int mode, int B, int lq, int k, int cap, uint8_t* base,
                         FilterF32Ws* fw) {
  size_t off = 0;
  auto take = [&](size_t bytes) -> uint8_t* {
    uint8_t* p = base ? base + off : nullptr;
    off += (bytes + 255) & ~(size_t)255;
    return p;
  };
  F32Ws& w = fw->w;
  const size_t m = (size_t)(m_allowed > 0 ? m_allowed : 1);
  const size_t qbytes = (size_t)B * lq * kDim * sizeof(uint16_t);
  w.qhi = (uint16_t*)take(qbytes);
  w.qlo = (uint16_t*)take(qbytes);
  w.beta = (float*)take((size_t)B * sizeof(float));
  fw->status = (int32_t*)take((size_t)B * sizeof(int32_t));
  w.tk_bytes = topk_ws_bytes(B, m_allowed);
  w.tk = take(w.tk_bytes);
  w.T = (float*)take((size_t)B * m * sizeof(float));
  if (mode == kFfBand) {
    w.lb = (float*)take((size_t)B * sizeof(float));
    w.count = (int32_t*)take((size_t)B * sizeof(int32_t));
    w.done = (int32_t*)take((size_t)B * sizeof(int32_t));
    w.arrive = (int32_t*)take((size_t)kArriveSlots * B * kArriveInts * sizeof(int32_t));
    w.cand = (int32_t*)take((size_t)B * cap * sizeof(int32_t));
    w.F = (float*)take((size_t)B * cap * sizeof(float));
    fw->tks = (float*)take((size_t)B * k * sizeof(float));
    fw->pos = (int32_t*)take((size_t)B * k * sizeof(int32_t));
  }
  if (mode == kFfDense) fw->dense = (float*)take((size_t)B * (size_t)(ix->n > 0 ? ix->n : 1) * sizeof(float));
  return off;
}

int search_filtered_f32_impl(cbv2_index* ix, const cbv2_filter* f, const float* Q, int32_t B, int32_t lq, int32_t k,
                             int32_t cap, int mode, FilterF32Ws& fw, float* out_scores, int32_t* out_ids,
                             int32_t* out_status, hipStream_t st) {
  const int64_t m = f->m;
  F32Ws& w = fw.w;
  int rc;
  if (m == 0) {
    CBV2_HIP(hipMemsetAsync(out_status, 0, (size_t)B * sizeof(int32_t), st));
    return topk_impl_empty(B, k, out_scores, out_ids, st);
  }
  const int64_t total = (int64_t)B * k;
  if (mode != kFfBand) {
    if (out_status != nullptr) CBV2_HIP(hipMemsetAsync(out_status, 0xff, (size_t)B * sizeof(int32_t), st));
    if ((rc = split_queries(ix, Q, B, lq, &w, st))) return rc;
    if (mode == kFfPair) {
      if ((rc = rescore_subset(ix, f, &w, B, lq, w.T, st))) return rc;
    } else {
      if ((rc = launch_rescore(ix, &w, B, lq, nullptr, nullptr, ix->n, 0, fw.dense, ix->n, st))) return rc;
      const int64_t gx = std::min<int64_t>((m + 255) / 256, 4096);
      hipLaunchKernelGGL(filter_gather_kernel, dim3((unsigned)gx, (unsigned)std::min(B, 65535)), dim3(256), 0, st,
                         fw.dense, ix->n, f->ids, m, B, w.T);
      if ((rc = launch_check("filter_gather_kernel"))) return rc;
    }
    if ((rc = topk_impl(w.T, B, m, m, k, 0, w.tk, w.tk_bytes, out_scores, out_ids, st, ix->device))) return rc;
// ... 45 lines not shown
  auto r256 = [](size_t b) { return (b + 255) & ~(size_t)255; };
  FilterPlan p;
  p.subset = filter_takes_subset(ix, m_allowed, scorer);
  const bool f32 = ix->resid != nullptr && scorer == CBV2_SCORER_MAXSIM;
  const int64_t m = m_allowed > 0 ? m_allowed : 1;
  p.off_tk = kCtrBytes;
  p.tk_bytes = r256(topk_ws_bytes(B, m_allowed));
  p.off_row = p.off_tk + p.tk_bytes;
  p.off_cand = p.off_row + r256((size_t)B * (size_t)m * sizeof(float));
  p.off_dense = p.off_cand + (cand && p.subset && f32 ? r256((size_t)B * (size_t)m * sizeof(int32_t)) : 0);
  p.off_f32 = p.off_dense + (p.subset ? 0 : r256((size_t)B * (size_t)(ix->n > 0 ? ix->n : 1) * sizeof(float)));
  p.total = p.off_f32;
  if (f32) {
    F32Ws w;
    p.total += f32_ws_layout(ix, CBV2_F32_SCORE, B, lq, 0, nullptr, &w);
  }
  return p;
}
FilterPlan filter_plan(const cbv2_index* ix, const cbv2_filter* f, int32_t B, int32_t lq, int32_t k, int32_t scorer) {
  FilterPlan p = filter_plan_m(ix, f->m, false, B, lq, scorer);
  if (ix->resid != nullptr && scorer == CBV2_SCORER_MAXSIM && lq <= kLqMax) {
    FilterF32Ws fw;
    p.total = std::max(p.total, filter_f32_layout(ix, f->m, filter_f32_mode(ix, f->m, B, k), B, lq, k,
                                                  std::max<int32_t>(CBV2_RETRIEVE_BAND_CAP, k), nullptr, &fw));
  }
  return p;
}

__device__ __forceinline__ const int32_t* fb_list(const int32_t* __restrict__ tab, int B, int b) {
  const uint32_t lo = (uint32_t)tab[fb_off_list(B) + 2 * b], hi = (uint32_t)tab[fb_off_list(B) + 2 * b + 1];
  return reinterpret_cast<const int32_t*>(((uint64_t)hi << 32) | lo);
}

__global__ __launch_bounds__(256) void fb_prepare_kernel(const int32_t* __restrict__ tab, int B, int64_t M,
                                                         int32_t* __restrict__ cand, float* __restrict__ row) {
  for (int b = blockIdx.y; b < B; b += gridDim.y) {
    const int64_t m = tab[fb_off_count(B) + b];
    const int32_t* ids = fb_list(tab, B, b);
    for (int64_t p = (int64_t)blockIdx.x * blockDim.x + threadIdx.x; p < M; p += (int64_t)gridDim.x * blockDim.x) {
      if (cand != nullptr) cand[(size_t)b * M + p] = p < m ? ids[p] : -1;
      if (p >= m) row[(size_t)b * M + p] = neg_inf();
    }
  }
}

__global__ __launch_bounds__(256) void fb_gather_kernel(const float* __restrict__ dense, int64_t ld,
                                                        const int32_t* __restrict__ tab, int B, int64_t M,
                                                        float* __restrict__ row) {
  for (int b = blockIdx.y; b < B; b += gridDim.y) {
    const int64_t m = tab[fb_off_count(B) + b];
    const int32_t* ids = fb_list(tab, B, b);
    for (int64_t p = (int64_t)blockIdx.x * blockDim.x + threadIdx.x; p < M; p += (int64_t)gridDim.x * blockDim.x)
      row[(size_t)b * M + p] = p < m ? dense[(size_t)b * ld + ids[p]] : neg_inf();
  }
}

__global__ __launch_bounds__(256) void fb_map_ids_kernel(int32_t* __restrict__ out_i, int B, int k,
                                                         const int32_t* __restrict__ tab, int64_t id_base) {
  const int64_t i = (int64_t)blockIdx.x * blockDim.x + threadIdx.x;
  if (i >= (int64_t)B * k) return;
  const int b = (int)(i / k);
  const int32_t p = out_i[i];
  out_i[i] = (p >= 0 && p < tab[fb_off_count(B) + b]) ? (int32_t)(id_base + fb_list(tab, B, b)[p]) : -1;
}

int launch_stream_ragged(cbv2_index* ix, const cbv2_filter_batch* fb, const uint16_t* Q, int B, int lq, float* out,
                         int64_t M, hipStream_t st) {
  const int64_t grid = (fb->chunks + 3) / 4;
  if (grid < 1 || grid > 0x1fffffff) return fail(CBV2_EUNSUPPORTED, "scan grid too large");
  constexpr StreamCfg C{.qw = 1, .aux = 2, .idx = true, .rag = true};
  hipLaunchKernelGGL(maxsim_scan_stream_kernel<C>, dim3((unsigned)grid), dim3(256), 0, st, ix->tokens, ix->doclens,
                     (int64_t)0, Q, B, lq, out, M, fb->chunk_docs, (int)ix->ld, (uint32_t*)nullptr, (int64_t)0,
                     (uint32_t*)nullptr, (int64_t)0, (const int32_t*)nullptr, fb->table);
  return launch_check("maxsim_scan_stream_kernel (ragged)");
}

int rescore_ragged(cbv2_index* ix, const cbv2_filter_batch* fb, const F32Ws* w, int B, int lq, const int32_t* cand,
                   float* out, int64_t M, hipStream_t st) {
  const auto [gx, two] = rescore_grid(ix, B, M);
  auto kern = two ? rescore_split_kernel<false, 2> : rescore_split_kernel<false, 4>;
  hipLaunchKernelGGL(kern, dim3(gx, (unsigned)B), dim3(two ? 128 : 256), 0, st, ix->tokens, ix->resid, ix->doclens,
                     ix->n, (int64_t)0, w->qhi, w->qlo, lq, cand, fb->table + fb_off_count(B), M, M, out, M,
                     (const int32_t*)nullptr, (int)ix->ld, (uint32_t*)nullptr, (int64_t)0, (float*)nullptr,
                     (int32_t*)nullptr, 0, (float*)nullptr, (int32_t*)nullptr, RowSelect(), TaggedCand());
  return launch_check("rescore_split_kernel (ragged)");
}

FilterPlan filter_batch_plan(const cbv2_index* ix, const cbv2_filter_batch* fb, int32_t B, int32_t lq,
                             int32_t scorer) {
  return filter_plan_m(ix, fb->max_m, true, B, lq, scorer);
}
}

extern "C" {

int cbv2_set_error(int code, const char* msg) { return fail(code, "%s", msg); }

int cbv2_abi_version(void) { return CBV2_ABI_VERSION; }

#ifndef CBV2_BUILD_STAMP
#define CBV2_BUILD_STAMP "unstamped"
#endif
const char* cbv2_build_stamp(void) { return "cbv2-build-stamp:" CBV2_BUILD_STAMP; }

const char* cbv2_last_error(void) { return g_err; }

int cbv2_index_create(int device, const void* tokens, int32_t dtype, int64_t n, int32_t ld, int32_t d,
                      const int32_t* doclens, int64_t id_base, cbv2_index** out) {
  CBV2_REQUIRE(out != nullptr, "null output handle pointer");
  *out = nullptr;
  CBV2_REQUIRE(n >= 0 && n <= 0x7fffffffLL, "n out of range (%lld)", (long long)n);
  CBV2_REQUIRE(id_base >= 0 && id_base + n <= 0x7fffffffLL, "global ids must fit int32");
  if (dtype != CBV2_DTYPE_BF16) return fail(CBV2_EUNSUPPORTED, "index dtype %d not built (bf16 only)", dtype);
  if ((ld != 128 && ld != 256 && ld != 512 && ld != 1024) || d != kDim)
    return fail(CBV2_EUNSUPPORTED, "index geometry ld=%d d=%d not built (ld = 128, 256, 512 or 1024; d = 128)", ld,
                d);
  if (n > 0) {
    CBV2_REQUIRE(tokens != nullptr && doclens != nullptr, "null tokens/doclens");
    CBV2_REQUIRE(aligned16(tokens), "tokens must be 16-byte aligned");
  }
  int ndev = 0;
  CBV2_HIP(hipGetDeviceCount(&ndev));
  CBV2_REQUIRE(device >= 0 && device < ndev, "device %d out of range (%d devices)", device, ndev);
  cbv2_index* ix = new cbv2_index{device, (const uint8_t*)tokens, n, ld, d, doclens, id_base, nullptr,
                                  CBV2_DTYPE_BF16, nullptr};
  alloc_task_ring(ix);
  *out = ix;
  return CBV2_OK;
}

int cbv2_index_create_mxfp8(int device, const void* tokens, const void* scales, int64_t n, int32_t ld, int32_t d,
                            const int32_t* doclens, int64_t id_base, cbv2_index** out) {
  CBV2_REQUIRE(out != nullptr, "null output handle pointer");
  *out = nullptr;
  CBV2_REQUIRE(n >= 0 && n <= 0x7fffffffLL, "n out of range (%lld)", (long long)n);
  CBV2_REQUIRE(id_base >= 0 && id_base + n <= 0x7fffffffLL, "global ids must fit int32");
  if ((ld != 128 && ld != 256 && ld != 512 && ld != 1024) || d != kDim)
    return fail(CBV2_EUNSUPPORTED, "index geometry ld=%d d=%d not built (ld = 128, 256, 512 or 1024; d = 128)", ld,
                d);
  if (n > 0) {
    CBV2_REQUIRE(tokens != nullptr && scales != nullptr && doclens != nullptr, "null tokens/scales/doclens");
    CBV2_REQUIRE(aligned16(tokens), "tokens must be 16-byte aligned");
    CBV2_REQUIRE(((uintptr_t)scales & 3u) == 0, "scales must be 4-byte aligned");
  }
  int ndev = 0;
  CBV2_HIP(hipGetDeviceCount(&ndev));
  CBV2_REQUIRE(device >= 0 && device < ndev, "device %d out of range (%d devices)", device, ndev);
  *out = new cbv2_index{device, (const uint8_t*)tokens, n, ld, d, doclens, id_base, nullptr, CBV2_DTYPE_MXFP8,
                        (const uint8_t*)scales};
  alloc_task_ring(*out);
  return CBV2_OK;
}

int cbv2_quantize_mxfp8(const void* x, int32_t dtype, int64_t rows, void* q, void* scales, void* stream) {
  CBV2_REQUIRE(rows >= 0, "rows must be >= 0");
  if (rows == 0) return CBV2_OK;
  CBV2_REQUIRE(x && q && scales, "null pointer");
  const int64_t want = (rows + 3) / 4;
  const unsigned grid = (unsigned)(want < 65536 ? want : 65536);
  if (dtype == CBV2_DTYPE_F32) {
    hipLaunchKernelGGL(quantize_mxfp8_kernel<float>, dim3(grid), dim3(256), 0, (hipStream_t)stream, (const float*)x,
                       rows, (uint8_t*)q, (uint8_t*)scales);
  } else if (dtype == CBV2_DTYPE_BF16) {
    hipLaunchKernelGGL(quantize_mxfp8_kernel<uint16_t>, dim3(grid), dim3(256), 0, (hipStream_t)stream,
                       (const uint16_t*)x, rows, (uint8_t*)q, (uint8_t*)scales);
  } else {
    return fail(CBV2_EINVAL, "quantize takes bf16 or f32 input (got dtype %d)", dtype);
// ... 434 lines not shown
  if (faithful) {
    CBV2_REQUIRE(Q != nullptr && aligned16(Q), "query pointer must be non-null and 16-byte aligned");
    CBV2_REQUIRE(B >= 1 && B <= 65535, "B must be in [1, 65535] (got %d)", B);
    CBV2_REQUIRE(lq >= 1 && lq <= kLqMax, "lq must be in [1, %d] (got %d)", kLqMax, lq);
  } else if (int rc = check_query(ix, scorer, Q, q_dtype, B, lq)) {
    return rc;
  }
  CBV2_REQUIRE(fb->n == ix->n && fb->id_base == ix->id_base && fb->device == ix->device,
               "the filter batch was created for another index (n %lld / %lld, id_base %lld / %lld, device %d / %d)",
               (long long)fb->n, (long long)ix->n, (long long)fb->id_base, (long long)ix->id_base, fb->device,
               ix->device);
  CBV2_REQUIRE(B == fb->B, "the filter batch holds %d queries, the call %d", fb->B, B);
  CBV2_REQUIRE(k >= 1, "k must be >= 1 (got %d)", k);
  CBV2_REQUIRE(out_scores && out_ids, "null outputs");
  const FilterPlan p = filter_batch_plan(ix, fb, B, lq, scorer);
  CBV2_REQUIRE(ws != nullptr && ws_bytes >= p.total && aligned16(ws), "workspace too small or misaligned (%zu < %zu)",
               ws_bytes, p.total);
  DeviceGuard dg(ix->device);
  if (!dg.ok) return fail(CBV2_EHIP, "cannot select device %d", ix->device);
  hipStream_t st = (hipStream_t)stream;
  const int64_t M = fb->max_m;
  if (M == 0) return topk_impl_empty(B, k, out_scores, out_ids, st);
  int* ctr = (int*)ws;
  float* row = (float*)((uint8_t*)ws + p.off_row);
  int32_t* cand = (int32_t*)((uint8_t*)ws + p.off_cand);
  float* dense = (float*)((uint8_t*)ws + p.off_dense);
  const unsigned gy = (unsigned)std::min(B, 65535);
  const unsigned gx = (unsigned)std::min<int64_t>((M + 255) / 256, 4096);
  int rc;
  F32Ws w;
  if (faithful) {
    f32_ws_layout(ix, CBV2_F32_SCORE, B, lq, 0, (uint8_t*)ws + p.off_f32, &w);
    if ((rc = split_queries(ix, (const float*)Q, B, lq, &w, st))) return rc;
  }
  if (p.subset) {
    hipLaunchKernelGGL(fb_prepare_kernel, dim3(gx, gy), dim3(256), 0, st, fb->table, B, M,
                       faithful ? cand : (int32_t*)nullptr, row);
    if ((rc = launch_check("fb_prepare_kernel"))) return rc;
    rc = faithful ? rescore_ragged(ix, fb, &w, B, lq, cand, row, M, st)
                  : launch_stream_ragged(ix, fb, (const uint16_t*)Q, B, lq, row, M, st);
    if (rc) return rc;
  } else {
    rc = faithful ? launch_rescore(ix, &w, B, lq, nullptr, nullptr, ix->n, 0, dense, ix->n, st)
                  : score_impl(ix, scorer, Q, B, lq, dense, ix->n, st, ctr);
    if (rc) return rc;
    hipLaunchKernelGGL(fb_gather_kernel, dim3(gx, gy), dim3(256), 0, st, dense, ix->n, fb->table, B, M, row);
    if ((rc = launch_check("fb_gather_kernel"))) return rc;
  }
  rc = topk_impl(row, B, M, M, k, 0, (uint8_t*)ws + p.off_tk, p.tk_bytes, out_scores, out_ids, st, ix->device);
  if (rc) return rc;
  const int64_t total = (int64_t)B * k;
  hipLaunchKernelGGL(fb_map_ids_kernel, dim3((unsigned)((total + 255) / 256)), dim3(256), 0, st, out_ids, B, k,
                     fb->table, fb->id_base);
  return launch_check("fb_map_ids_kernel");
}

int cbv2_index_set_option(cbv2_index* ix, int32_t option, int64_t value) {
  CBV2_REQUIRE(ix != nullptr, "null index");
  switch (option) {
    case CBV2_OPT_FUSED_TOPK:
      ix->fused_topk = value != 0;
      ix->fused_topk_mode = (int)value;
      return CBV2_OK;
    case CBV2_OPT_DYNAMIC_TAIL:
      ix->dynamic_tail = (int)value;
      return CBV2_OK;
    case CBV2_OPT_BAND_DOC_MAJOR:
      ix->band_doc_major = (int)value;
      return CBV2_OK;
    case CBV2_OPT_BAND_LOWER_BOUND:
      ix->band_lower_bound = value != 0;
      return CBV2_OK;
    case CBV2_OPT_TOPK_BMAX:
      ix->topk_bmax = (int)value;
      return CBV2_OK;
    case CBV2_OPT_BAND_FUSED:
      ix->band_fused = value != 0;
      return CBV2_OK;
    case CBV2_OPT_RESCORE_SPLIT:
      ix->rescore_split = value != 0;
      return CBV2_OK;
    case CBV2_OPT_BAND_REUSE:
      ix->band_reuse = value != 0;
      return CBV2_OK;
    case CBV2_OPT_BAND_BLOCK_SKIP:
      ix->band_block_skip = value != 0;
      return CBV2_OK;
    case CBV2_OPT_DENSE_DOCS:
      ix->dense_docs = value != 0;
      return CBV2_OK;
    case CBV2_OPT_P1_COLLECT_FUSED:
      ix->p1_collect_fused = value != 0;
      return CBV2_OK;
    case CBV2_OPT_FOLD_KEYS:
      ix->fold_keys = value != 0;
      return CBV2_OK;
    case CBV2_OPT_FILTER_PATH:
      if (value < 0 || value > 2) return fail(CBV2_EINVAL, "filter path must be 0 (automatic), 1 (subset) or 2 (dense)");
      ix->filter_path = (int)value;
      return CBV2_OK;
    case CBV2_OPT_FILTER_BAND:
      if (value < 0 || value > 2) return fail(CBV2_EINVAL, "filter band must be 0 (automatic), 1 (on) or 2 (never)");
      ix->filter_band = (int)value;
      return CBV2_OK;
    case CBV2_OPT_FILTER_BATCH_CHUNK_DOCS:
      if (value < 0 || value > 0x7fffffffLL) return fail(CBV2_EINVAL, "filter batch chunk docs must be in [0, 2^31)");
      ix->filter_batch_chunk_docs = value;
      return CBV2_OK;
    case CBV2_OPT_RESCORE_GRID:
      if (value < 0 || value > 65535) return fail(CBV2_EINVAL, "rescore grid must be in [0, 65535]");
      ix->rescore_grid = (int)value;
      return CBV2_OK;
    default:
      return fail(CBV2_EINVAL, "unknown option %d", option);
  }
}

int64_t cbv2_search_fused_slots(const cbv2_index* ix, int32_t B, int32_t k, int32_t scorer) {
  if (!ix || B < 1 || k < 1) return 0;
  return fused_slots(ix, scorer, B, k);
}

int cbv2_index_last_scan_plan(const cbv2_index* ix, int64_t* out4) {
  CBV2_REQUIRE(ix != nullptr && out4 != nullptr, "null index or output");
  for (int i = 0; i < 4; ++i) out4[i] = ix->last_plan[i];
  return CBV2_OK;
}

int cbv2_index_kind(const cbv2_index* ix, int32_t* dtype, int32_t* faithful) {
  CBV2_REQUIRE(ix != nullptr && dtype != nullptr && faithful != nullptr, "null index or output");
  *dtype = ix->dtype;
  *faithful = ix->resid != nullptr ? 1 : 0;
  return CBV2_OK;
}

constexpr int kRrSplitMaxB = 32;

size_t cbv2_rerank_workspace_bytes(int32_t B, int32_t C) {
  if (B < 1 || C < 1) return 0;
  return ((size_t)B * (size_t)C * sizeof(float) + 255) & ~(size_t)255;
}

static int rerank_impl(cbv2_index* ix, const void* Q, int32_t B, int32_t lq, const int32_t* cand, int32_t C,
                       int32_t k, void* ws, size_t ws_bytes, float* out_scores, int32_t* out_ids, int32_t* out_pos,
                       void* stream) {
  const int32_t qdt = ix && ix->dtype == CBV2_DTYPE_MXFP8 ? CBV2_DTYPE_MXFP8 : CBV2_DTYPE_BF16;
  int rc = check_query(ix, CBV2_SCORER_MAXSIM, Q, qdt, B, lq);
  if (rc) return rc;
  CBV2_REQUIRE(cand != nullptr, "null candidates");
  CBV2_REQUIRE(C >= 1 && C <= kRerankMaxC, "C must be in [1, %d] (got %d)", kRerankMaxC, C);
  CBV2_REQUIRE(k >= 0, "k must be >= 0 (got %d)", k);
  CBV2_REQUIRE(out_scores != nullptr, "null out_scores");
  CBV2_REQUIRE(k == 0 || out_ids != nullptr, "null out_ids");
  DeviceGuard dg(ix->device);
  if (!dg.ok) return fail(CBV2_EHIP, "cannot select device %d", ix->device);
  const hipStream_t st = (hipStream_t)stream;
  const bool big = C > kSmallMax;
  const unsigned dyn = big ? (unsigned)C * sizeof(float) : 0u;
  const bool f8 = ix->dtype == CBV2_DTYPE_MXFP8;
  const uint8_t* Qb = (const uint8_t*)Q;
  const uint8_t* Qs = f8 ? Qb + (size_t)B * lq * kDim : nullptr;
  const size_t raw_bytes = (size_t)B * (size_t)C * sizeof(float);
  if (B <= kRrSplitMaxB && (k == 0 || (!big && ws != nullptr && ws_bytes >= raw_bytes))) {
    float* raw = k == 0 ? out_scores : (float*)ws;
    const dim3 grid((unsigned)((C + kRrWaves - 1) / kRrWaves), (unsigned)B);
    TaggedCand tc;
// ... 36 lines not shown
  if (big) {
    CBV2_HIP(hipFuncSetAttribute((const void*)rerank_kernel<true>, hipFuncAttributeMaxDynamicSharedMemorySize,
                                 (int)dyn));
    hipLaunchKernelGGL(rerank_kernel<true>, dim3((unsigned)B), dim3(kRrWaves * 64), dyn, st, ix->tokens, ix->doclens,
                       ix->n, ix->id_base, (const uint16_t*)Q, lq, cand, C, k, out_scores, out_ids, out_pos,
                       (int)ix->ld);
  } else {
    hipLaunchKernelGGL(rerank_kernel<false>, dim3((unsigned)B), dim3(kRrWaves * 64), 0, st, ix->tokens, ix->doclens,
                       ix->n, ix->id_base, (const uint16_t*)Q, lq, cand, C, k, out_scores, out_ids, out_pos,
                       (int)ix->ld);
  }
  return launch_check("rerank_kernel");
}

int cbv2_rerank(cbv2_index* ix, const void* Q, int32_t B, int32_t lq, const int32_t* cand, int32_t C, int32_t k,
                float* out_scores, int32_t* out_ids, int32_t* out_pos, void* stream) {
  return rerank_impl(ix, Q, B, lq, cand, C, k, nullptr, 0, out_scores, out_ids, out_pos, stream);
}

int cbv2_rerank_ws(cbv2_index* ix, const void* Q, int32_t B, int32_t lq, const int32_t* cand, int32_t C, int32_t k,
                   void* workspace, size_t workspace_bytes, float* out_scores, int32_t* out_ids, int32_t* out_pos,
                   void* stream) {
  return rerank_impl(ix, Q, B, lq, cand, C, k, workspace, workspace_bytes, out_scores, out_ids, out_pos, stream);
}

int cbv2_select_topk(const float* scores, const int32_t* ids, int32_t B, int32_t C, int32_t k, float* out_scores,
                     int32_t* out_ids, int32_t* out_pos, void* stream) {
  CBV2_REQUIRE(scores && out_scores, "null scores/out_scores");
  CBV2_REQUIRE(B >= 1, "B must be >= 1");
  CBV2_REQUIRE(C >= 1, "C must be >= 1 (got %d)", C);
  CBV2_REQUIRE(k >= 1, "k must be >= 1 (got %d)", k);
  if (C > kSmallMax)
    return topk_multi(scores, B, C, C, k, 0, ids, C, out_scores, out_ids, out_pos, (hipStream_t)stream);
  hipLaunchKernelGGL(select_small_kernel, dim3((unsigned)B), dim3(256), 0, (hipStream_t)stream, scores, ids, C, k,
                     out_scores, out_ids, out_pos);
  return launch_check("select_small_kernel");
}

int cbv2_prescored_select(const int32_t* recv, int32_t G, int64_t blk, int32_t B, int32_t k, int32_t kb,
                          const int32_t* cand, int32_t C, int32_t fk, float* out_s, int32_t* out_i, int32_t* out_p,
                          int32_t* misses, void* stream) {
  CBV2_REQUIRE(recv && cand && out_s && out_i, "null blocks / candidates / outputs");
  CBV2_REQUIRE(G >= 1 && B >= 1 && k >= 1 && kb >= 0 && fk >= 1, "bad sizes (G %d, B %d, k %d, kb %d, k %d)", G, B,
               k, kb, fk);
  CBV2_REQUIRE(C >= 1 && C <= kSmallMax, "prescored select: C must be in [1, %d] (got %d)", kSmallMax, C);
  hipLaunchKernelGGL(prescored_select_kernel, dim3((unsigned)B), dim3(256), 0, (hipStream_t)stream, recv, G, blk, B,
                     k, kb, cand, C, fk, out_s, out_i, out_p, misses);
  return launch_check("prescored_select_kernel");
}

int cbv2_split_f32(const float* x, int64_t rows, int32_t ld, const int32_t* doclens, void* hi, void* lo,
                   float* bounds, void* stream) {
  CBV2_REQUIRE(rows >= 0, "rows must be >= 0");
  CBV2_REQUIRE(doclens == nullptr || (ld >= 1 && rows % ld == 0), "with doclens, rows must be docs of ld rows");
  if (rows == 0) return CBV2_OK;
  CBV2_REQUIRE(x && hi && lo && bounds, "null pointer");
  CBV2_REQUIRE(aligned16(x) && aligned16(hi) && aligned16(lo), "x, hi and lo must be 16-byte aligned");
  const int64_t want = (rows * 16 + 255) / 256;
  const unsigned grid = (unsigned)(want < 65536 ? want : 65536);
  hipLaunchKernelGGL(split_f32_kernel, dim3(grid), dim3(256), 0, (hipStream_t)stream, x, rows, ld, doclens,
                     (uint16_t*)hi,
                     (uint16_t*)lo, bounds);
  return launch_check("split_f32_kernel");
}

int cbv2_index_attach_residual(cbv2_index* ix, const void* lo, float resid_max, float norm_max) {
  CBV2_REQUIRE(ix != nullptr, "null index");
  CBV2_REQUIRE(ix->dtype == CBV2_DTYPE_BF16, "a residual attaches to a bf16 index");
  CBV2_REQUIRE(ix->n == 0 || (lo != nullptr && aligned16(lo)), "residual must be non-null and 16-byte aligned");
  CBV2_REQUIRE(resid_max >= 0.0f && norm_max >= 0.0f && resid_max < 3.0e38f && norm_max < 3.0e38f,
               "bounds must be finite and >= 0");
  ix->resid = (const uint8_t*)lo;
  ix->resid_max = resid_max;
  ix->norm_max = norm_max;
  return CBV2_OK;
}

size_t cbv2_f32_workspace_bytes(const cbv2_index* ix, int32_t op, int32_t B, int32_t lq, int32_t cap) {
  if (!ix || B < 1 || lq < 1 || cap < 0 || op < CBV2_F32_SCORE || op > CBV2_F32_RERANK) return 0;
  F32Ws w;
  return f32_ws_layout(ix, op, B, lq, cap, nullptr, &w);
}

int cbv2_score_f32(cbv2_index* ix, const float* Q, int32_t B, int32_t lq, void* ws, size_t wsb, float* out,
                   int64_t ld_out, void* stream) {
  F32Ws w;
  int rc = check_f32(ix, CBV2_F32_SCORE, Q, B, lq, 0, ws, wsb, &w);
  if (rc) return rc;
  CBV2_REQUIRE(ix->n == 0 || out != nullptr, "null output");
  CBV2_REQUIRE(ld_out >= ix->n, "ld_out (%lld) < n (%lld)", (long long)ld_out, (long long)ix->n);
  DeviceGuard dg(ix->device);
  if (!dg.ok) return fail(CBV2_EHIP, "cannot select device %d", ix->device);
  hipStream_t st = (hipStream_t)stream;
  if (ix->n == 0) return CBV2_OK;
  rc = split_queries(ix, Q, B, lq, &w, st);
  if (rc) return rc;
  return launch_rescore(ix, &w, B, lq, nullptr, nullptr, ix->n, 0, out, ld_out, st);
}

namespace {
bool band_reuses_topk(const cbv2_index* ix, int32_t B, int32_t k) {
  return ix->band_reuse && ix->rescore_split && ix->n >= k && !(B <= kBandPairMaxB && ix->ld == kLd && ix->band_fused);
}
bool phase1_collect_fused(const cbv2_index* ix, int32_t B, int32_t k) {
  return ix->p1_collect_fused && B <= kBandPairMaxB && k <= kTopkMax && band_reuses_topk(ix, B, k) &&
         bmax_eligible(ix, CBV2_SCORER_MAXSIM, B, k) && ix->band_block_skip && !ix->band_doc_major;
}

int search_f32_phase1(cbv2_index* ix, const float* Q, int32_t B, int32_t lq, int32_t k, int32_t cap, F32Ws& w,
                      float* out_scores, int32_t* out_ids, int32_t* out_status, bool want_lb, hipStream_t st,
                      float* fk_out = nullptr) {
  int rc;
  if (ix->n == 0) {
    CBV2_HIP(hipMemsetAsync(out_status, 0, (size_t)B * sizeof(int32_t), st));
    if ((rc = topk_impl_empty(B, k, out_scores, out_ids, st))) return rc;
    return 1;
  }
  const bool bmax = k <= kBandCapMax && bmax_eligible(ix, CBV2_SCORER_MAXSIM, B, k);
  const bool fold0 = bmax && !scan_folds_bmax(ix, B) && scan_folds_bmax_zeroed(ix, B);
  if ((rc = split_queries(ix, Q, B, lq, &w, st, want_lb && band_reuses_topk(ix, B, k) ? k : 0, true,
                          fold0 ? (uint32_t*)w.tk : nullptr,
                          fold0 ? (int64_t)B * (bm_blocks(ix->n) + bm_supers(ix->n)) : 0)))
    return rc;
  if (k > kBandCapMax) {
    CBV2_HIP(hipMemsetAsync(out_status, 0xff, (size_t)B * sizeof(int32_t), st));
    if ((rc = launch_rescore(ix, &w, B, lq, nullptr, nullptr, ix->n, 0, w.T, ix->n, st))) return rc;
    if ((rc = topk_multi(w.T, B, ix->n, ix->n, k, ix->id_base, nullptr, 0, out_scores, out_ids, nullptr, st)))
      return rc;
    return 1;
  }
  const bool fold = bmax && (scan_folds_bmax(ix, B) || fold0);
  {
    CtrPolicy cp(kCtrPrezeroed);
    if ((rc = scan_maxsim_timed(ix, w.qhi, B, lq, w.T, ix->n, st, w.ctr, nullptr, fold ? (uint32_t*)w.tk : nullptr)))
      return rc;
  }
  const Mirror mirror = g_ids_mirror;
  g_ids_mirror = Mirror();
  rc = bmax ? topk_bmax(w.T, B, ix->n, ix->n, k, ix->id_base, (uint32_t*)w.tk, out_scores, out_ids, st, ix->device,
                        fold, arrive_row0(w, kArrBmax, B), kArriveInts)
            : topk_impl(w.T, B, ix->n, ix->n, k, ix->id_base, w.tk, w.tk_bytes, out_scores, out_ids, st, ix->device);
  g_ids_mirror = mirror;
  if (rc) return rc;
  if ((rc = band_mark(ix, false, st))) return rc;
  if (fk_out != nullptr)
    return launch_rescore(ix, &w, B, lq, out_ids, nullptr, k, k, fk_out, k, st);
  if (want_lb && phase1_collect_fused(ix, B, k))
    return CBV2_OK;
  if (want_lb) {
    RowSelect lab;
    lab.stamps = LAB_STAMPS(1);
    return launch_rescore(ix, &w, B, lq, out_ids, nullptr, k, k, w.F, cap, st, nullptr, 0,
                          reinterpret_cast<uint32_t*>(w.lb), 0, nullptr, nullptr, 0, nullptr, nullptr, lab);
  }
  return CBV2_OK;
}

int search_f32_phase2_impl(cbv2_index* ix, int32_t B, int32_t lq, int32_t k, int32_t cap, F32Ws& w,
                           const float* lb, const uint32_t* lbu, float* out_scores, int32_t* out_ids,
                           int32_t* out_status, hipStream_t st) {
  int rc;
  const bool reuse = lbu != nullptr && band_reuses_topk(ix, B, k);
  const int c0 = reuse ? k : 0;
  const bool pair_path = !(B <= kBandPairMaxB && ix->ld == kLd && ix->band_fused) &&
                         !(ix->band_doc_major && B > kBandPairMaxB);
  const bool fb_fused = pair_path && ix->rescore_split && k <= kTopkMax;
  int64_t splits = (8LL * cu_count(ix->device) + B - 1) / B;
  const int64_t max_splits = (ix->n + 8191) / 8192;
  splits = splits < max_splits ? splits : max_splits;
  splits = splits < 1 ? 1 : splits;
  if (lbu != nullptr && phase1_collect_fused(ix, B, k)) {
    const int64_t groups = (bm_blocks(ix->n) + 63) / 64;
    hipLaunchKernelGGL(phase1_collect_kernel, dim3((unsigned)(k + groups), (unsigned)B), dim3(256), 0, st,
                       ix->tokens, ix->resid, ix->doclens, ix->n, ix->id_base, w.qhi, w.qlo, lq, out_ids, out_scores,
                       k, w.F, (int64_t)cap, const_cast<uint32_t*>(lbu), arrive_row0(w, kArrPhase1, B),
                       (int64_t)kArriveInts, w.T, w.beta, reinterpret_cast<const uint32_t*>(w.tk), cap, w.cand,
                       w.count, g_wait_ticks, LAB_STAMPS(1));
    if ((rc = launch_check("phase1_collect_kernel"))) return rc;
  } else if (B <= kBandPairMaxB && ix->ld == kLd && ix->band_fused) {
    const int64_t gx = (ix->n + kBcrDocs - 1) / kBcrDocs;
    hipLaunchKernelGGL(band_collect_rescore_kernel, dim3((unsigned)gx, (unsigned)B), dim3(256), 0, st, w.T, ix->n,
                       out_scores, k, w.beta, lb, lbu, ix->tokens, ix->resid, ix->doclens, ix->id_base, w.qhi, w.qlo,
                       lq, cap, w.cand, w.F, w.count);
    if ((rc = launch_check("band_collect_rescore_kernel"))) return rc;
  } else {
    const bool bkeys = bmax_eligible(ix, CBV2_SCORER_MAXSIM, B, k) && ix->band_block_skip;
    if (bkeys) {
      const int64_t per_row = (8LL * cu_count(ix->device) + B - 1) / B;
      const int64_t groups = (bm_blocks(ix->n) + 63) / 64;
      splits = std::max<int64_t>(1, std::min(per_row, groups));
    }
    hipLaunchKernelGGL(band_collect_kernel, dim3((unsigned)splits, (unsigned)B), dim3(256), 0, st, w.T, ix->n,
                       out_scores, k, w.beta, ix->id_base, cap, w.cand, w.count, lb, lbu,
                       reuse ? out_ids : nullptr, bkeys ? reinterpret_cast<const uint32_t*>(w.tk) : nullptr,
                       LAB_STAMPS(2));
    if ((rc = launch_check("band_collect_kernel"))) return rc;
  }
  if (B <= kBandPairMaxB && ix->ld == kLd && ix->band_fused) {
  } else if (ix->band_doc_major && B > kBandPairMaxB) {
    CBV2_HIP(hipMemsetAsync(w.dcnt, 0, (size_t)ix->n * sizeof(int32_t), st));
    CBV2_HIP(hipMemsetAsync(w.dctr, 0, 2 * sizeof(int32_t), st));
    const unsigned gc = (unsigned)std::min<int64_t>((cap + 255) / 256, 16);
    hipLaunchKernelGGL(band_count_kernel, dim3(gc, (unsigned)B), dim3(256), 0, st, w.cand, w.count, cap, ix->id_base,
                       ix->n, w.dcnt, c0);
    if ((rc = launch_check("band_count_kernel"))) return rc;
    const unsigned go = (unsigned)std::min<int64_t>((ix->n + 255) / 256, 1024);
    hipLaunchKernelGGL(band_offsets_kernel, dim3(go), dim3(256), 0, st, w.dcnt, ix->n, w.doff, w.act, w.act_off,
                       w.act_cnt, w.dctr);
    if ((rc = launch_check("band_offsets_kernel"))) return rc;
    hipLaunchKernelGGL(band_scatter_kernel, dim3(gc, (unsigned)B), dim3(256), 0, st, w.cand, w.count, cap,
                       ix->id_base, ix->n, w.dcnt, w.doff, w.pair_b, w.pair_c, c0);
    if ((rc = launch_check("band_scatter_kernel"))) return rc;
    if ((ix->band_doc_major == 3 || ix->band_doc_major == 4) && ix->ld == kLd) {
      const bool two = ix->band_doc_major == 4;
      const unsigned gs = (unsigned)((two ? 4 : 3) * cu_count(ix->device) * 4);
      hipLaunchKernelGGL(two ? rescore_docs_split_kernel<2> : rescore_docs_split_kernel<4>, dim3(gs),
                         dim3(two ? 128 : 256), 0, st, ix->tokens, ix->resid, ix->doclens, w.qhi, w.qlo, B, lq, w.act,
                         w.act_off, w.act_cnt, w.dctr, w.pair_b, w.pair_c, w.F, cap);
      if ((rc = launch_check("rescore_docs_split_kernel"))) return rc;
    } else {
      const unsigned gr = (unsigned)(2 * cu_count(ix->device) * 4);
      auto kern = ix->band_doc_major == 2 ? (ix->ld != kLd ? rescore_docs_kernel<true, true> : rescore_docs_kernel<true>)
                                          : (ix->ld != kLd ? rescore_docs_kernel<false, true> : rescore_docs_kernel<false>);
      hipLaunchKernelGGL(kern, dim3(gr), dim3(256), 0, st, ix->tokens, ix->resid, ix->doclens, w.qhi, w.qlo, B, lq,
                         w.act, w.act_off, w.act_cnt, w.dctr, w.pair_b, w.pair_c, w.F, cap, (int)ix->ld);
      if ((rc = launch_check("rescore_docs_kernel"))) return rc;
    }
  } else {
    RowSelect rs;
    if (fb_fused && B <= kBandPairMaxB) {
      rs.mode = kSelBand;
      rs.arrive = arrive_row0(w, kArrBand, B);
      rs.k = k;
      rs.out_s = out_scores;
      rs.out_i = out_ids;
      rs.lb = lb;
      rs.lbu = lbu;
      rs.status = out_status;
      rs.ids_mirror = g_ids_mirror;
      if (g_ids_mirror.w != nullptr) g_ids_mirror_used = true;
      rs.stamps = LAB_STAMPS(3);
    }
    if ((rc = launch_rescore(ix, &w, B, lq, w.cand, w.count, cap, cap, w.F, cap, st, nullptr,
                             B <= kBandPairMaxB ? 1 : 0, nullptr, c0, fb_fused ? w.T : nullptr,
                             fb_fused ? w.done : nullptr, k, out_scores, out_ids, rs)))
      return rc;
    if (rs.mode != kSelNone) return CBV2_OK;
  }
  hipLaunchKernelGGL(band_select_kernel, dim3((unsigned)B), dim3(kTkThreads), 0, st, w.F, w.cand, w.count, cap, k,
                     ix->id_base, out_scores, out_ids, out_status, lb, lbu);
  if ((rc = launch_check("band_select_kernel"))) return rc;
  if (fb_fused) return CBV2_OK;
  if (ix->rescore_split && k <= kTopkMax) {
    const int64_t fb = std::max<int64_t>(64, 256 / B);
    const unsigned gx = (unsigned)(ix->n < fb ? ix->n : fb);
    hipLaunchKernelGGL(ix->ld != kLd ? fallback_split_kernel<true> : fallback_split_kernel<false>, dim3(gx, (unsigned)B),
                       dim3(256), 0, st, ix->tokens, ix->resid, ix->doclens, ix->n, ix->id_base, w.qhi, w.qlo, lq,
                       w.T, out_status, (int)ix->ld, w.done, k, out_scores, out_ids);
    return launch_check("fallback_split_kernel");
  }
  if ((rc = launch_rescore(ix, &w, B, lq, nullptr, nullptr, ix->n, 0, w.T, ix->n, st, out_status))) return rc;
  if (k > kTopkMax)
    return topk_multi(w.T, B, ix->n, ix->n, k, ix->id_base, nullptr, 0, out_scores, out_ids, nullptr, st, out_status);
  hipLaunchKernelGGL(topk_rows_kernel, dim3((unsigned)B), dim3(kTkThreads), 0, st, w.T, ix->n, ix->n, k, ix->id_base,
                     out_scores, out_ids, out_status);
  return launch_check("topk_rows_kernel");
}

int search_f32_phase2(cbv2_index* ix, int32_t B, int32_t lq, int32_t k, int32_t cap, F32Ws& w, const float* lb,
                      const uint32_t* lbu, float* out_scores, int32_t* out_ids, int32_t* out_status,
                      hipStream_t st) {
  const int rc = search_f32_phase2_impl(ix, B, lq, k, cap, w, lb, lbu, out_scores, out_ids, out_status, st);
  if (rc) return rc;
  return band_mark(ix, true, st);
}

int rerank_f32_split(cbv2_index* ix, F32Ws& w, int32_t B, int32_t lq, const int32_t* cand, int32_t C, int32_t k,
                     float* out_scores, int32_t* out_ids, int32_t* out_pos, hipStream_t st,
                     int32_t* arrive = nullptr) {
  int rc;
  float* raw = k == 0 ? out_scores : w.F;
  if (k > 0 && C <= kSmallMax && arrive != nullptr && ix->rescore_split) {
    RowSelect rs;
    rs.mode = kSelCand;
    rs.arrive = arrive;
    rs.k = k;
    rs.out_s = out_scores;
    rs.out_i = out_ids;
    rs.out_p = out_pos;
    const TaggedCand tc = g_cand_tagged;
    if (tc.w != nullptr) g_cand_tagged_used = true;
    if (g_final_mirror.w != nullptr && g_final_mirror.k == k) {
      rs.fin = g_final_mirror;
      g_final_mirror_used = true;
    }
    rs.stamps = LAB_STAMPS(4);
    return launch_rescore(ix, &w, B, lq, cand, nullptr, C, C, raw, C, st, nullptr, 0, nullptr, 0, nullptr, nullptr, 0,
                          nullptr, nullptr, rs, tc);
  }
  RowSelect rw;
  if (k == 0 && g_raw_mirror.w != nullptr) {
    rw.raw = g_raw_mirror;
    g_raw_mirror_used = true;
  }

  if ((rc = launch_rescore(ix, &w, B, lq, cand, nullptr, C, C, raw, C, st, nullptr, 0, nullptr, 0, nullptr, nullptr, 0,
                           nullptr, nullptr, rw)))
    return rc;
  if (k == 0) return CBV2_OK;
  if (C > kSmallMax) return topk_multi(raw, B, C, C, k, 0, cand, C, out_scores, out_ids, out_pos, st);
  const FinalMirror fin = g_final_mirror.k == k ? g_final_mirror : FinalMirror();
  if (fin.w != nullptr) g_final_mirror_used = true;
  hipLaunchKernelGGL(select_small_kernel, dim3((unsigned)B), dim3(256), 0, st, raw, cand, C, k, out_scores, out_ids,
                     out_pos, nullptr, fin);
  return launch_check("select_small_kernel");
}

int check_search_f32(cbv2_index* ix, const float* Q, int32_t B, int32_t lq, int32_t k, int32_t cap, void* ws,
                     size_t wsb, F32Ws* w) {
  CBV2_REQUIRE(k >= 1, "k must be >= 1 (got %d)", k);
  CBV2_REQUIRE(k > kBandCapMax || (cap >= k && cap <= kBandCapMax), "cap must be in [k, %d] (got %d)", kBandCapMax,
               cap);
  return check_f32(ix, CBV2_F32_SEARCH, Q, B, lq, cap, ws, wsb, w);
}
}

int cbv2_search_f32(cbv2_index* ix, const float* Q, int32_t B, int32_t lq, int32_t k, int32_t cap, void* ws,
                    size_t wsb, float* out_scores, int32_t* out_ids, int32_t* out_status, void* stream) {
// ... 225 lines not shown
```

hybrid-rag-colbertv2_amd/index.py:

```python
from __future__ import annotations

import ctypes
import json
import os
from typing import Iterable, List, Optional, Sequence, Tuple, Union

import torch

from . import _lib

LD = 128
LONG_LDS = (128, 256, 512, 1024)
DIM = 128
LQ_MAX = 32
BAND_CAP = 16384


_raw_stream = getattr(torch._C, "_cuda_getCurrentRawStream", None)


def _stream_ptr(device: torch.device) -> int:
    if _raw_stream is not None:
        return _raw_stream(device.index if device.index is not None else torch.cuda.current_device())
    return torch.cuda.current_stream(device).cuda_stream
# ... 168 lines not shown

    def close(self) -> None:
        if getattr(self, "_h", None) is not None and self._h.value:
            _lib.lib().cbv2_filter_destroy(self._h)
            self._h = ctypes.c_void_p()

    def __len__(self):
        return self.count

    def __del__(self):
        try:
            self.close()
        except Exception:
            pass


class FilterBatch:

    def __init__(self, index: "ColbertIndex", filters: Sequence[DocFilter]):
        L = _lib.lib()
        self.index = index
        self.filters = list(filters)
        B = len(self.filters)
        if B < 1:
            raise ValueError("a filter batch needs at least one filter")
        for f in self.filters:
            if not isinstance(f, DocFilter):
                raise TypeError("filters must be DocFilter objects (ColbertIndex.filter)")
            if not f._h.value:
                raise ValueError("a filter of the batch is closed")
        need = int(L.cbv2_filter_batch_bytes(B))
        self._buf = torch.empty((max(need, 16),), dtype=torch.uint8, device=index.device)
        arr = (ctypes.c_void_p * B)(*[f._h.value for f in self.filters])
        h = ctypes.c_void_p()
        _lib.check(L.cbv2_filter_batch_create(index._h, arr, B, self._buf.data_ptr(), self._buf.numel(),
                                              _stream_ptr(index.device), ctypes.byref(h)))
        self._h = h
        self.B = B
        self.pairs = int(L.cbv2_filter_batch_pairs(h))
        self.max_count = int(L.cbv2_filter_batch_max_count(h))

    def close(self) -> None:
        if getattr(self, "_h", None) is not None and self._h.value:
            _lib.lib().cbv2_filter_batch_destroy(self._h)
            self._h = ctypes.c_void_p()

    def __len__(self):
        return self.B

    def __del__(self):
        try:
            self.close()
        except Exception:
            pass


class ColbertIndex:

    def __init__(self, tokens: torch.Tensor, doclens: torch.Tensor, id_base: int = 0,
                 scales: Optional[torch.Tensor] = None, residual: Optional[torch.Tensor] = None,
                 bounds: Optional[Tuple[float, float]] = None):
        _require_cuda(tokens, "tokens")
        _require_cuda(doclens, "doclens")
        self.fp8 = tokens.dtype == torch.uint8
        want = torch.uint8 if self.fp8 else torch.bfloat16
        if tokens.dtype != want or tokens.dim() != 3 or tokens.shape[2] != DIM or tokens.shape[1] not in LONG_LDS:
            raise ValueError(f"tokens must be bf16 or MXFP8 uint8 [n, ld, {DIM}] (ld in {LONG_LDS}) "
                             f"(got {tokens.dtype} {tuple(tokens.shape)})")
        self.ld = int(tokens.shape[1])
        if doclens.dtype != torch.int32 or doclens.shape != (tokens.shape[0],):
            raise ValueError("doclens must be int32 [n]")
        if self.fp8 and (scales is None or scales.dtype != torch.uint8
                         or tuple(scales.shape) != (tokens.shape[0], tokens.shape[1], 2)):
            raise ValueError("an MXFP8 index needs uint8 scales [n, ld, 2]")
        self.tokens = tokens.contiguous()
        self.scales = scales.contiguous() if self.fp8 else None
        self.doclens = doclens.contiguous()
        self.device = tokens.device
        self.n = int(tokens.shape[0])
        self.id_base = int(id_base)
        self.means: Optional[torch.Tensor] = None
        self._ws: Optional[torch.Tensor] = None
        self._rr_ws: Optional[torch.Tensor] = None
        self._all_filter: Optional[DocFilter] = None
        self._last_filter_batch: Optional[FilterBatch] = None
        h = ctypes.c_void_p()
        dev = self.device.index if self.device.index is not None else torch.cuda.current_device()
        if self.fp8:
            _lib.check(_lib.lib().cbv2_index_create_mxfp8(
                dev, self.tokens.data_ptr(), self.scales.data_ptr(), self.n, self.ld, DIM, self.doclens.data_ptr(),
                self.id_base, ctypes.byref(h)))
        else:
            _lib.check(_lib.lib().cbv2_index_create(
                dev, self.tokens.data_ptr(), _lib.DTYPE_BF16, self.n, self.ld, DIM, self.doclens.data_ptr(),
                self.id_base, ctypes.byref(h)))
        self._h = h
        self.dense_docs = False
        if self.ld == 128 and self.n > 0:
            tiles = int(((self.doclens.clamp(0, self.ld) + 15) // 16).sum().item())
            self.dense_docs = tiles >= 0.98 * self.n * (self.ld // 16)
            if self.dense_docs:
                self.set_option(_lib.OPT_DENSE_DOCS, 1)
        self.residual: Optional[torch.Tensor] = None
        self.bounds: Optional[Tuple[float, float]] = None
        if residual is not None:
            if self.fp8 or residual.dtype != torch.bfloat16 or residual.shape != self.tokens.shape \
                    or residual.device != self.device or bounds is None:
                raise ValueError("a residual is bf16 [n, ld, 128] like the tokens, on the index device, "
                                 "with (resid_max, norm_max)")
            self.residual = residual.contiguous()
            self.bounds = (float(bounds[0]), float(bounds[1]))
            _lib.check(_lib.lib().cbv2_index_attach_residual(self._h, self.residual.data_ptr(), self.bounds[0],
                                                             self.bounds[1]))

    @property
    def faithful(self) -> bool:
        return self.residual is not None

    @classmethod
    def faithful_f32(cls, tokens_f32: torch.Tensor, doclens: torch.Tensor, id_base: int = 0) -> "ColbertIndex":
        _require_cuda(tokens_f32, "tokens_f32")
        if tokens_f32.dtype != torch.float32 or tokens_f32.dim() != 3 or tokens_f32.shape[2] != DIM \
                or tokens_f32.shape[1] not in LONG_LDS:
            raise ValueError(f"tokens_f32 must be f32 [n, ld, {DIM}], ld in {LONG_LDS} (got {tokens_f32.dtype} "
                             f"{tuple(tokens_f32.shape)})")
        x = tokens_f32.contiguous()
        hi = hbm_empty(x.shape, torch.bfloat16, x.device)
        lo = hbm_empty(x.shape, torch.bfloat16, x.device)
        bounds = torch.zeros(2, dtype=torch.float32, device=x.device)
        _require_cuda(doclens, "doclens")
        if doclens.dtype != torch.int32 or doclens.shape != (x.shape[0],):
            raise ValueError("doclens must be int32 [n]")
        doclens = doclens.contiguous()
        _lib.check(_lib.lib().cbv2_split_f32(x.data_ptr(), x.numel() // DIM, x.shape[1], doclens.data_ptr(),
                                             hi.data_ptr(), lo.data_ptr(), bounds.data_ptr(), _stream_ptr(x.device)))
        b = bounds.tolist()
        return cls(hi, doclens, id_base=id_base, residual=lo, bounds=(b[0], b[1]))

    def _f32_ws(self, op: int, B: int, lq: int, cap: int) -> torch.Tensor:
        need = int(_lib.lib().cbv2_f32_workspace_bytes(self._h, op, B, lq, cap))
        if self._ws is None or self._ws.numel() * 4 < need:
            self._ws = torch.empty(((need + 3) // 4,), dtype=torch.float32, device=self.device)
        return self._ws

    @classmethod
    def mxfp8(cls, tokens: torch.Tensor, doclens: torch.Tensor, id_base: int = 0) -> "ColbertIndex":
        q, sc = quantize_mxfp8(tokens)
        return cls(q, doclens, id_base=id_base, scales=sc)

    @classmethod
    def from_embeddings(cls, embs, device="cuda", id_base: int = 0, build_means: bool = False,
                        dtype: str = "bf16"):
        device = torch.device(device)
        if dtype not in ("bf16", "fp8", "fp32"):
            raise ValueError(f"index dtype must be bf16, fp8 or fp32 (got {dtype!r})")
        tokens, doclens = pack_tokens(embs, device, ld=None,
                                      dtype=torch.float32 if dtype == "fp32" else torch.bfloat16)
        if dtype == "fp32":
            ix = cls.faithful_f32(tokens, doclens, id_base=id_base)
        elif dtype == "fp8":
            ix = cls.mxfp8(tokens, doclens, id_base=id_base)
        else:
            ix = cls(tokens, doclens, id_base=id_base)
        del tokens
        if build_means:
            if isinstance(embs, torch.Tensor):
                f32 = embs if embs.dim() == 3 else embs.unsqueeze(1)
                f32 = f32.to(device=device, dtype=torch.float32).contiguous()
            else:
                f32 = torch.zeros((ix.n, ix.ld, DIM), dtype=torch.float32, device=device)
                for i, e in enumerate(embs):
                    e = e if e.dim() == 2 else e.unsqueeze(0)
                    f32[i, : e.shape[0]] = e.to(device=device, dtype=torch.float32)
            ix.build_means(f32)
        return ix

    def save(self, path: str) -> None:
        dt = _lib.DTYPE_MXFP8 if self.fp8 else _lib.DTYPE_BF16
        torch.cuda.current_stream(self.device).synchronize()
        for side in (path + ".bounds.json", path + ".resid"):
            if os.path.exists(side):
                os.unlink(side)
        _lib.check(_lib.lib().cbv2_index_file_write_ld(
            os.fsencode(path), dt, self.n, self.ld, self.tokens.data_ptr(),
            self.scales.data_ptr() if self.fp8 else None, self.doclens.data_ptr(), self.id_base,
            _stream_ptr(self.device)))
        if self.faithful:
            _lib.check(_lib.lib().cbv2_index_file_write_ld(
                os.fsencode(path + ".resid"), _lib.DTYPE_BF16, self.n, self.ld, self.residual.data_ptr(), None,
                self.doclens.data_ptr(), self.id_base, _stream_ptr(self.device)))
            with open(path + ".bounds.json", "w") as f:
                json.dump({"resid_max": self.bounds[0], "norm_max": self.bounds[1],
                           "hi": file_fingerprint(path), "resid": file_fingerprint(path + ".resid")}, f)

    @classmethod
    def load(cls, path: str, device="cuda", begin: int = 0, end: Optional[int] = None) -> "ColbertIndex":
        device = torch.device(device)
        dt, n, id_base, ld = index_file_layout(path)
        end = n if end is None else int(end)
        begin = int(begin)
        m = end - begin
        if begin < 0 or m < 0 or end > n:
            raise ValueError(f"doc range [{begin}, {end}) outside [0, {n})")
        fp8 = dt == _lib.DTYPE_MXFP8
        tokens = hbm_empty((m, ld, DIM), torch.uint8 if fp8 else torch.bfloat16, device)
        scales = hbm_empty((m, ld, 2), torch.uint8, device) if fp8 else None
        doclens = torch.empty((m,), dtype=torch.int32, device=device)
        with torch.cuda.device(device):
            _lib.check(_lib.lib().cbv2_index_file_read(
                os.fsencode(path), begin, end, tokens.data_ptr() if m else None,
                scales.data_ptr() if (fp8 and m) else None, doclens.data_ptr() if m else None,
                _stream_ptr(device)))
        if not fp8 and os.path.exists(path + ".resid") and os.path.exists(path + ".bounds.json"):
            with open(path + ".bounds.json") as f:
                b = json.load(f)
            if index_file_layout(path + ".resid")[1:] != (n, id_base, ld) or \
                    b.get("hi") != file_fingerprint(path) or b.get("resid") != file_fingerprint(path + ".resid"):
                raise ValueError(f"{path}.resid / .bounds.json were not written with {path}")
            resid = hbm_empty((m, ld, DIM), torch.bfloat16, device)
            dl2 = torch.empty((m,), dtype=torch.int32, device=device)
            with torch.cuda.device(device):
                _lib.check(_lib.lib().cbv2_index_file_read(
                    os.fsencode(path + ".resid"), begin, end, resid.data_ptr() if m else None, None,
                    dl2.data_ptr() if m else None, _stream_ptr(device)))
            if not torch.equal(dl2, doclens):
                raise ValueError(f"{path}.resid does not match {path}")
# ... 176 lines not shown

    def all_docs_filter(self) -> DocFilter:
        if self._all_filter is None:
            self._all_filter = self.filter(mask=torch.ones(self.n, dtype=torch.bool))
        return self._all_filter

    def filter_batch(self, filters: Sequence[Optional[DocFilter]]) -> FilterBatch:
        return FilterBatch(self, [self.all_docs_filter() if f is None else f for f in filters])

    def _search_filtered_batch(self, Q: torch.Tensor, k: int, scorer: str, filters):
        k = int(k)
        B = int(Q.shape[0]) if Q.dim() == 3 else 1
        batch = filters if isinstance(filters, FilterBatch) else None
        flts = batch.filters if batch is not None else list(filters)
        if len(flts) != B:
            raise ValueError(f"filters must hold one entry per query ({len(flts)} for {B} queries)")
        if batch is None and all(f is flts[0] for f in flts) and flts[0] is not None:
            return self._search_filtered(Q, k, scorer, flts[0])
        if self._query_blocks(Q, scorer) is not None:
            Q3 = Q if Q.dim() == 3 else Q[None]
            rows = [self._search_filtered(Q3[b:b + 1], k, scorer, self.all_docs_filter() if f is None else f)
                    for b, f in enumerate(flts)]
            return torch.cat([r[0] for r in rows]), torch.cat([r[1] for r in rows])
        if batch is None:
            batch = self.filter_batch(flts)
        if not batch._h.value:
            raise ValueError("the filter batch is closed")
        sid = self._scorer(scorer)
        _keep, qptr, qdt, B, lq = self._prep_query(Q, scorer)
        L = _lib.lib()
        need = int(L.cbv2_search_filtered_batch_workspace_size(self._h, batch._h, B, lq, k, sid))
        if self._ws is None or self._ws.numel() * 4 < need:
            self._ws = torch.empty(((need + 3) // 4,), dtype=torch.float32, device=self.device)
        out_s = torch.empty((B, k), dtype=torch.float32, device=self.device)
        out_i = torch.empty((B, k), dtype=torch.int32, device=self.device)
        _lib.check(L.cbv2_search_filtered_batch(self._h, batch._h, sid, qptr, qdt, B, lq, k, self._ws.data_ptr(),
                                                self._ws.numel() * 4, out_s.data_ptr(), out_i.data_ptr(),
                                                _stream_ptr(self.device)))
        self._last_filter_batch = batch
        return out_s, out_i

    def search(self, Q: torch.Tensor, k: int, scorer: str = "maxsim",
               lb_reduce=None, filter: Optional[DocFilter] = None,
               filters=None) -> Tuple[torch.Tensor, torch.Tensor]:
        if filters is not None:
            if filter is not None:
                raise ValueError("pass filter (one for the call) or filters (one per query), not both")
            if lb_reduce is not None:
                raise ValueError("filters cannot be combined with lb_reduce (sharded faithful filtering is out of scope)")
            return self._search_filtered_batch(Q, k, scorer, filters)
        if filter is not None:
            if lb_reduce is not None:
                raise ValueError("filter cannot be combined with lb_reduce (sharded faithful filtering is out of scope)")
            return self._search_filtered(Q, k, scorer, filter)
        if self._query_blocks(Q, scorer) is not None:
            return topk_rows(self.score(Q, scorer), int(k), id_base=self.id_base)
        sid = self._scorer(scorer)
        _keep, qptr, qdt, B, lq = self._prep_query(Q, scorer)
        if self.faithful and scorer == "maxsim":
            if lb_reduce is not None:
                return self._search_f32_global(_keep, B, lq, k, lb_reduce)
            return self._search_f32(_keep, B, lq, k)
        L = _lib.lib()
        need = int(L.cbv2_search_workspace_size(self._h, B, int(k), sid))
        if self._ws is None or self._ws.numel() * 4 < need:
            self._ws = torch.empty(((need + 3) // 4,), dtype=torch.float32, device=self.device)
        out_s = torch.empty((B, k), dtype=torch.float32, device=self.device)
        out_i = torch.empty((B, k), dtype=torch.int32, device=self.device)
        _lib.check(L.cbv2_search(self._h, sid, qptr, qdt, B, lq, int(k), self._ws.data_ptr(),
                                 self._ws.numel() * 4, out_s.data_ptr(), out_i.data_ptr(),
                                 _stream_ptr(self.device)))
        return out_s, out_i

    def _search_f32(self, Qd: torch.Tensor, B: int, lq: int, k: int, cap: int = BAND_CAP):
        cap = max(int(cap), int(k))
        ws = self._f32_ws(_lib.F32_SEARCH, B, lq, cap)
        out_s = torch.empty((B, k), dtype=torch.float32, device=self.device)
        out_i = torch.empty((B, k), dtype=torch.int32, device=self.device)
        status = torch.empty((B,), dtype=torch.int32, device=self.device)
        _lib.check(_lib.lib().cbv2_search_f32(self._h, Qd.data_ptr(), B, lq, int(k), cap, ws.data_ptr(),
                                              ws.numel() * 4, out_s.data_ptr(), out_i.data_ptr(),
                                              status.data_ptr(), _stream_ptr(self.device)))
        self.last_band = status
        return out_s, out_i

    def _search_f32_global(self, Qd: torch.Tensor, B: int, lq: int, k: int, lb_reduce, cap: int = BAND_CAP):
        cap = max(int(cap), int(k))
        ws = self._f32_ws(_lib.F32_SEARCH, B, lq, cap)
        out_s = torch.empty((B, k), dtype=torch.float32, device=self.device)
        out_i = torch.empty((B, k), dtype=torch.int32, device=self.device)
        status = torch.empty((B,), dtype=torch.int32, device=self.device)
        fk = torch.empty((B, k), dtype=torch.float32, device=self.device)
        L = _lib.lib()
        _lib.check(L.cbv2_search_f32_begin(self._h, Qd.data_ptr(), B, lq, int(k), cap, ws.data_ptr(),
                                           ws.numel() * 4, fk.data_ptr(), out_s.data_ptr(), out_i.data_ptr(),
                                           status.data_ptr(), _stream_ptr(self.device)))
        lb = lb_reduce(fk).to(device=self.device, dtype=torch.float32).contiguous()
        if tuple(lb.shape) != (B,):
            raise ValueError(f"lb_reduce must return f32 [{B}] (got {tuple(lb.shape)})")
        _lib.check(L.cbv2_search_f32_finish(self._h, B, lq, int(k), cap, ws.data_ptr(), ws.numel() * 4,
                                            lb.data_ptr(), out_s.data_ptr(), out_i.data_ptr(), status.data_ptr(),
                                            _stream_ptr(self.device)))
        self.last_band = status
        return out_s, out_i

    def rerank(self, Q: torch.Tensor, cand: torch.Tensor, k: int):
        blocks = self._query_blocks(Q, "maxsim")
        if blocks is not None:
            raw = self.rerank(blocks[0], cand, 0).clone()
            for q in blocks[1:]:
                raw += self.rerank(q, cand, 0)
            if k == 0:
                return raw
            cand = cand.to(device=self.device, dtype=torch.int32)
            return select_topk(raw, int(k), ids=cand if cand.dim() == 2 else cand.unsqueeze(0))
        _keep, qptr, _, Bq, lq = self._prep_query(Q, "maxsim")
        cand = cand.to(device=self.device, dtype=torch.int32).contiguous()
        if cand.dim() == 1:
            cand = cand.unsqueeze(0)
        B, C = int(cand.shape[0]), int(cand.shape[1])
        if Bq != B:
            raise ValueError(f"{Bq} queries but {B} candidate rows")
        if self.faithful:
            ws = self._f32_ws(_lib.F32_RERANK, B, lq, C)
            out_s = torch.empty((B, C if k == 0 else k), dtype=torch.float32, device=self.device)
            out_i = torch.empty((B, k), dtype=torch.int32, device=self.device) if k else None
            out_p = torch.empty((B, k), dtype=torch.int32, device=self.device) if k else None
            _lib.check(_lib.lib().cbv2_rerank_f32(
                self._h, _keep.data_ptr(), B, lq, cand.data_ptr(), C, int(k), ws.data_ptr(), ws.numel() * 4,
                out_s.data_ptr(), out_i.data_ptr() if k else None, out_p.data_ptr() if k else None,
                _stream_ptr(self.device)))
            return out_s if k == 0 else (out_s, out_i, out_p)
        if k == 0:
            out_s = torch.empty((B, C), dtype=torch.float32, device=self.device)
            _lib.check(_lib.lib().cbv2_rerank(self._h, qptr, B, lq, cand.data_ptr(), C, 0,
                                              out_s.data_ptr(), None, None, _stream_ptr(self.device)))
            return out_s
        out_s = torch.empty((B, k), dtype=torch.float32, device=self.device)
        out_i = torch.empty((B, k), dtype=torch.int32, device=self.device)
        out_p = torch.empty((B, k), dtype=torch.int32, device=self.device)
        L = _lib.lib()
        need = int(L.cbv2_rerank_workspace_bytes(B, C))
        if self._rr_ws is None or self._rr_ws.numel() < need:
            self._rr_ws = torch.empty((need,), dtype=torch.uint8, device=self.device)
        _lib.check(L.cbv2_rerank_ws(self._h, qptr, B, lq, cand.data_ptr(), C, int(k), self._rr_ws.data_ptr(),
                                    self._rr_ws.numel(), out_s.data_ptr(), out_i.data_ptr(), out_p.data_ptr(),
                                    _stream_ptr(self.device)))
        return out_s, out_i, out_p


def _as_batch(embs, device, dtype, ld=LD):
    return pack_tokens(embs, device, ld=ld, dtype=dtype)


class IndexBuilder:

    def __init__(self, n: int, device="cuda", dtype: str = "bf16", id_base: int = 0, ld: Optional[int] = None):
        if dtype not in ("bf16", "fp8", "fp32"):
            raise ValueError(f"index dtype must be bf16, fp8 or fp32 (got {dtype!r})")
        if ld is not None and ld not in LONG_LDS:
            raise ValueError(f"ld must be one of {LONG_LDS} (got {ld})")
        self.n, self.dtype, self.id_base = int(n), dtype, int(id_base)
        self.grow = ld is None
        self.ld = LD if ld is None else int(ld)
        self.device = torch.device(device)
        self.pos = 0
        self.doclens = torch.zeros((self.n,), dtype=torch.int32, device=self.device)
        if dtype == "fp8":
            self.tokens = hbm_zeros((self.n, self.ld, DIM), torch.uint8, self.device)
            self.scales = hbm_empty((self.n, self.ld, 2), torch.uint8, self.device).fill_(127)
        else:
            self.tokens = hbm_zeros((self.n, self.ld, DIM), torch.bfloat16, self.device)
            self.scales = None
        if dtype == "fp32":
            self.residual = hbm_zeros((self.n, self.ld, DIM), torch.bfloat16, self.device)
            self.bounds = torch.zeros(2, dtype=torch.float32, device=self.device)

    def _relayout(self, ld: int) -> None:
        def grown(x, fill=0):
            y = hbm_empty((self.n, ld, x.shape[2]), x.dtype, self.device).fill_(fill)
            y[: self.pos, : self.ld] = x[: self.pos]
            return y
        self.tokens = grown(self.tokens)
        if self.dtype == "fp32":
            self.residual = grown(self.residual)
        if self.dtype == "fp8":
# ... 165 lines not shown
```

include/colbert_mi355x.h:

```cpp
#ifndef COLBERT_MI355X_H
#define COLBERT_MI355X_H

#include <stddef.h>
#include <stdint.h>

#ifdef __cplusplus
extern "C" {
#endif

#define CBV2_ABI_VERSION 2

#define CBV2_DTYPE_BF16 1
#define CBV2_DTYPE_F32 2
#define CBV2_DTYPE_MXFP8 3

#define CBV2_SCORER_MAXSIM 0
#define CBV2_SCORER_REF_MEANPOOL_COSINE 1

#define CBV2_OK 0
#define CBV2_EINVAL -1
#define CBV2_EUNSUPPORTED -2
#define CBV2_EHIP -3
#define CBV2_ESTATE -4

typedef struct cbv2_index cbv2_index;

int cbv2_abi_version(void);
const char* cbv2_last_error(void);
const char* cbv2_build_stamp(void);

int cbv2_index_create(int device, const void* tokens, int32_t dtype, int64_t n, int32_t ld,
                      int32_t d, const int32_t* doclens, int64_t id_base, cbv2_index** out);
int cbv2_index_destroy(cbv2_index* index);

int cbv2_hbm_alloc(int device, size_t bytes, void** out, int32_t* contiguous);
int cbv2_hbm_free(int device, void* p);

int cbv2_index_time_scans(cbv2_index* index, int32_t enable);
int cbv2_index_scan_times(cbv2_index* index, float* ms, int32_t max, int32_t* count);
int cbv2_index_band_times(cbv2_index* index, float* ms, int32_t max, int32_t* count);
int cbv2_index_scan_clock(cbv2_index* index, int64_t* out4, int32_t reset);

#define CBV2_OPT_FUSED_TOPK 1
#define CBV2_OPT_DYNAMIC_TAIL 2
#define CBV2_OPT_BAND_DOC_MAJOR 3
#define CBV2_OPT_BAND_LOWER_BOUND 4
#define CBV2_OPT_TOPK_BMAX 5
#define CBV2_OPT_BAND_FUSED 6
#define CBV2_OPT_RESCORE_SPLIT 7
#define CBV2_OPT_BAND_REUSE 8
#define CBV2_OPT_BAND_BLOCK_SKIP 9
#define CBV2_OPT_RESCORE_GRID 10
#define CBV2_OPT_DENSE_DOCS 11
#define CBV2_OPT_P1_COLLECT_FUSED 12
#define CBV2_OPT_FOLD_KEYS 13
#define CBV2_OPT_FILTER_PATH 14
#define CBV2_OPT_FILTER_BATCH_CHUNK_DOCS 15
#define CBV2_OPT_FILTER_BAND 16
int cbv2_index_set_option(cbv2_index* index, int32_t option, int64_t value);
int cbv2_index_last_scan_plan(const cbv2_index* index, int64_t* out4);
int64_t cbv2_search_fused_slots(const cbv2_index* index, int32_t B, int32_t k, int32_t scorer);

int cbv2_index_create_mxfp8(int device, const void* tokens, const void* scales, int64_t n, int32_t ld,
                            int32_t d, const int32_t* doclens, int64_t id_base, cbv2_index** out);

int cbv2_quantize_mxfp8(const void* x, int32_t dtype, int64_t rows, void* q, void* scales, void* stream);

int cbv2_index_build_means(cbv2_index* index, const float* tokens_f32, int32_t ld_src,
                           float* doc_means, void* stream);

int cbv2_score(cbv2_index* index, int32_t scorer, const void* Q, int32_t q_dtype, int32_t B,
               int32_t lq, float* out, int64_t ld_out, void* stream);

size_t cbv2_search_workspace_size(const cbv2_index* index, int32_t B, int32_t k, int32_t scorer);
size_t cbv2_search_workspace_bytes(const cbv2_index* index, int32_t B);
int cbv2_search(cbv2_index* index, int32_t scorer, const void* Q, int32_t q_dtype, int32_t B,
                int32_t lq, int32_t k, void* workspace, size_t workspace_bytes,
                float* out_scores, int32_t* out_ids, void* stream);

typedef struct cbv2_filter cbv2_filter;
size_t cbv2_filter_bytes(int64_t n);
int cbv2_filter_create(const cbv2_index* index, const uint32_t* allow, void* buf, size_t buf_bytes, void* stream,
                       cbv2_filter** out);
int64_t cbv2_filter_count(const cbv2_filter* filter);
int cbv2_filter_destroy(cbv2_filter* filter);
size_t cbv2_search_filtered_workspace_size(const cbv2_index* index, const cbv2_filter* filter, int32_t B, int32_t lq,
                                           int32_t k, int32_t scorer);
int cbv2_search_filtered(cbv2_index* index, const cbv2_filter* filter, int32_t scorer, const void* Q, int32_t q_dtype,
                         int32_t B, int32_t lq, int32_t k, void* workspace, size_t workspace_bytes,
                         float* out_scores, int32_t* out_ids, void* stream);

size_t cbv2_search_filtered_f32_workspace_size(const cbv2_index* index, const cbv2_filter* filter, int32_t B,
                                               int32_t lq, int32_t k, int32_t cap);
int
cbv2_search_filtered_f32(cbv2_index* index, const cbv2_filter* filter, const float* Q, int32_t B, int32_t lq,
                             int32_t k, int32_t cap, void* workspace, size_t workspace_bytes, float* out_scores,
                             int32_t* out_ids, int32_t* out_status, void* stream);

typedef struct cbv2_filter_batch cbv2_filter_batch;
size_t cbv2_filter_batch_bytes(int32_t B);
int cbv2_filter_batch_create(const cbv2_index* index, const cbv2_filter* const* per_query, int32_t B, void* buf,
                             size_t buf_bytes, void* stream, cbv2_filter_batch** out);
int64_t cbv2_filter_batch_pairs(const cbv2_filter_batch* fb);
int64_t cbv2_filter_batch_max_count(const cbv2_filter_batch* fb);
int cbv2_filter_batch_destroy(cbv2_filter_batch* fb);
size_t cbv2_search_filtered_batch_workspace_size(const cbv2_index* index, const cbv2_filter_batch* fb, int32_t B,
                                                 int32_t lq, int32_t k, int32_t scorer);
int cbv2_search_filtered_batch(cbv2_index* index, const cbv2_filter_batch* fb, int32_t scorer, const void* Q,
                               int32_t q_dtype, int32_t B, int32_t lq, int32_t k, void* workspace,
                               size_t workspace_bytes, float* out_scores, int32_t* out_ids, void* stream);

int cbv2_rerank(cbv2_index* index, const void* Q, int32_t B, int32_t lq, const int32_t* cand,
                int32_t C, int32_t k, float* out_scores, int32_t* out_ids, int32_t* out_pos,
                void* stream);

size_t cbv2_rerank_workspace_bytes(int32_t B, int32_t C);
int cbv2_rerank_ws(cbv2_index* index, const void* Q, int32_t B, int32_t lq, const int32_t* cand,
                   int32_t C, int32_t k, void* workspace, size_t workspace_bytes, float* out_scores,
                   int32_t* out_ids, int32_t* out_pos, void* stream);

#define CBV2_F32_SCORE 0
#define CBV2_F32_SEARCH 1
#define CBV2_F32_RERANK 2
int cbv2_split_f32(const float* x, int64_t rows, int32_t ld, const int32_t* doclens, void* hi, void* lo,
                   float* bounds, void* stream);
int cbv2_index_attach_residual(cbv2_index* index, const void* lo, float resid_max, float norm_max);
size_t cbv2_f32_workspace_bytes(const cbv2_index* index, int32_t op, int32_t B, int32_t lq, int32_t cap);
int cbv2_score_f32(cbv2_index* index, const float* Q, int32_t B, int32_t lq, void* workspace,
                   size_t workspace_bytes, float* out, int64_t ld_out, void* stream);
int cbv2_search_f32(cbv2_index* index, const float* Q, int32_t B, int32_t lq, int32_t k, int32_t cap,
                    void* workspace, size_t workspace_bytes, float* out_scores, int32_t* out_ids,
                    int32_t* out_status, void* stream);
int cbv2_search_f32_begin(cbv2_index* index, const float* Q, int32_t B, int32_t lq, int32_t k, int32_t cap,
                          void* workspace, size_t workspace_bytes, float* fk, float* out_scores, int32_t* out_ids,
                          int32_t* out_status, void* stream);
int cbv2_search_f32_finish(cbv2_index* index, int32_t B, int32_t lq, int32_t k, int32_t cap, void* workspace,
                           size_t workspace_bytes, const float* lb, float* out_scores, int32_t* out_ids,
                           int32_t* out_status, void* stream);
int cbv2_rerank_f32(cbv2_index* index, const float* Q, int32_t B, int32_t lq, const int32_t* cand,
                    int32_t C, int32_t k, void* workspace, size_t workspace_bytes, float* out_scores,
                    int32_t* out_ids, int32_t* out_pos, void* stream);

int cbv2_select_topk(const float* scores, const int32_t* ids, int32_t B, int32_t C, int32_t k,
                     float* out_scores, int32_t* out_ids, int32_t* out_pos, void* stream);

size_t cbv2_topk_workspace_bytes(int32_t B, int64_t n);
int cbv2_topk_rows(const float* scores, int32_t B, int64_t n, int64_t ld, int32_t k,
                   int64_t id_base, void* workspace, size_t workspace_bytes,
                   float* out_scores, int32_t* out_ids, void* stream);

int cbv2_merge_topk(const float* in_scores, const int32_t* in_ids, int32_t G, int32_t B,
                    int32_t k, float* out_scores, int32_t* out_ids, void* stream);

int cbv2_rrf_fuse(const int32_t* bm25_ids, int32_t kb, const int32_t* colbert_ids, int32_t kc, int32_t B,
                  int32_t rrf_k, int32_t C, int32_t* out_ids, double* out_scores, int32_t* out_count);

typedef struct cbv2_bm25 cbv2_bm25;
int cbv2_bm25_build(const int32_t* doc_terms, const int64_t* doc_offsets, int64_t n_docs, int32_t vocab,
                    float k1, float b, cbv2_bm25** out);
int cbv2_bm25_search(const cbv2_bm25* index, const int32_t* q_terms, const int64_t* q_offsets, int32_t B,
                     int32_t k, int32_t n_threads, int32_t* out_ids, float* out_scores);
int cbv2_bm25_search_filtered(const cbv2_bm25* index, const int32_t* q_terms, const int64_t* q_offsets, int32_t B,
                              int32_t k, int32_t n_threads, const uint32_t* allow, int32_t* out_ids,
                              float* out_scores);
int cbv2_bm25_search_filtered_batch(const cbv2_bm25* index, const int32_t* q_terms, const int64_t* q_offsets, int32_t B,
                                    int32_t k, int32_t n_threads, const uint32_t* const* allows, int32_t* out_ids,
                                    float* out_scores);
int cbv2_bm25_doc_freq(const int32_t* doc_terms, const int64_t* doc_offsets, int64_t n_docs, int32_t vocab,
                       int64_t* df_out);
int cbv2_bm25_build_shard(const int32_t* doc_terms, const int64_t* doc_offsets, int64_t n_docs, int32_t vocab,
                          float k1, float b, int64_t id_base, int64_t n_global, int64_t total_global,
                          const int64_t* df_global, cbv2_bm25** out);
int64_t cbv2_bm25_num_docs(const cbv2_bm25* index);
int cbv2_bm25_destroy(cbv2_bm25* index);

int cbv2_stem_en(const char* words, const int64_t* offsets, int64_t n, char* out, int64_t out_cap,
                 int64_t* out_offsets);

int cbv2_index_file_info(const char* path, int32_t* dtype, int64_t* n, int64_t* id_base);
int cbv2_index_file_info_ld(const char* path, int32_t* dtype, int64_t* n, int64_t* id_base, int32_t* ld);
int cbv2_index_file_write_ld(const char* path, int32_t dtype, int64_t n, int32_t ld, const void* tokens,
                             const void* scales, const int32_t* doclens, int64_t id_base, void* stream);
int cbv2_index_file_write_host_ld(const char* path, int32_t dtype, int64_t n, int32_t ld, const void* tokens,
                                  const void* scales, const int32_t* doclens, int64_t id_base);
int cbv2_index_file_write(const char* path, int32_t dtype, int64_t n, const void* tokens, const void* scales,
                          const int32_t* doclens, int64_t id_base, void* stream);
int cbv2_index_file_read(const char* path, int64_t begin, int64_t end, void* tokens, void* scales, int32_t* doclens,
                         void* stream);
int cbv2_index_file_write_host(const char* path, int32_t dtype, int64_t n, const void* tokens, const void* scales,
                               const int32_t* doclens, int64_t id_base);
int cbv2_index_file_read_host(const char* path, int64_t begin, int64_t end, void* tokens, void* scales,
                              int32_t* doclens);

typedef struct cbv2_index_writer cbv2_index_writer;
int cbv2_index_writer_open(const char* path, int32_t dtype, int64_t n, int64_t id_base, cbv2_index_writer** out);
int cbv2_index_writer_open_ld(const char* path, int32_t dtype, int64_t n, int32_t ld, int64_t id_base,
                              cbv2_index_writer** out);
int cbv2_index_writer_append(cbv2_index_writer* w, int64_t count, const void* tokens, const void* scales,
                             const int32_t* doclens, int32_t on_device, void* stream);
int64_t cbv2_index_writer_count(const cbv2_index_writer* w);
int cbv2_index_writer_close(cbv2_index_writer* w);

typedef struct cbv2_comm cbv2_comm;
int cbv2_comm_init(void* nccl_comm, const char* rccl_library, cbv2_comm** out);
int cbv2_comm_size(const cbv2_comm* comm);
int cbv2_comm_rank(const cbv2_comm* comm);
int cbv2_comm_destroy(cbv2_comm* comm);
size_t cbv2_sharded_workspace_bytes(const cbv2_index* index, const cbv2_comm* comm, int32_t B, int32_t k,
                                    int32_t kb, int32_t C);
int cbv2_search_sharded(cbv2_index* index, cbv2_comm* comm, int32_t scorer, const void* Q, int32_t q_dtype,
// ... 47 lines not shown
```

Baseline: 1776.

## Add bound-based early exit to faithful band rescore, skip lo-part MFMAs

Adds a per-query gamma bound, computed in the query split kernel, that limits the residual contribution. The band rescore kernel first scores each candidate doc using only the hi bf16 part. If that partial score plus gamma cannot reach the current lower bound, it skips loading the lo residual and the three-term MFMA pass. It also changes the key-qualification scan to assign 64-key groups per wave when there are more groups than blocks, and prefetches the next key. The cost is an extra hi-only MFMA pass and an extra barrier for docs that do not exit, plus a per-row exit counter exposed to Python.

```diff
diff --git a/hybrid-rag-colbertv2_amd/_lib.py b/hybrid-rag-colbertv2_amd/_lib.py
--- a/hybrid-rag-colbertv2_amd/_lib.py
+++ b/hybrid-rag-colbertv2_amd/_lib.py
@@ -18,8 +18,8 @@
 F32_SCORE, F32_SEARCH, F32_RERANK = 0, 1, 2
 (OPT_FUSED_TOPK, OPT_DYNAMIC_TAIL, OPT_BAND_DOC_MAJOR, OPT_BAND_LOWER_BOUND, OPT_TOPK_BMAX, OPT_BAND_FUSED,
  OPT_RESCORE_SPLIT, OPT_BAND_REUSE, OPT_BAND_BLOCK_SKIP, OPT_RESCORE_GRID, OPT_DENSE_DOCS, OPT_P1_COLLECT_FUSED,
- OPT_FOLD_KEYS, OPT_FILTER_PATH, OPT_FILTER_BATCH_CHUNK_DOCS, OPT_FILTER_BAND) = (1, 2, 3, 4, 5, 6, 7, 8, 9, 10, 11, 12,
-                                                                                 13, 14, 15, 16)
+ OPT_FOLD_KEYS, OPT_FILTER_PATH, OPT_FILTER_BATCH_CHUNK_DOCS, OPT_FILTER_BAND,
+ OPT_BAND_EARLY_EXIT) = (1, 2, 3, 4, 5, 6, 7, 8, 9, 10, 11, 12, 13, 14, 15, 16, 17)
 FILTER_AUTO, FILTER_SUBSET, FILTER_DENSE = 0, 1, 2
 FILTER_BAND_AUTO, FILTER_BAND_ON, FILTER_BAND_OFF = 0, 1, 2
 
@@ -115,6 +115,7 @@
     "cbv2_split_f32": (ctypes.c_int, [_p, _i64, _i32, _p, _p, _p, _p, _p]),
     "cbv2_index_attach_residual": (ctypes.c_int, [_p, _p, ctypes.c_float, ctypes.c_float]),
     "cbv2_f32_workspace_bytes": (_sz, [_p, _i32, _i32, _i32, _i32]),
+    "cbv2_f32_band_exits_offset": (_sz, [_p, _i32, _i32, _i32]),
     "cbv2_score_f32": (ctypes.c_int, [_p, _p, _i32, _i32, _p, _sz, _p, _i64, _p]),
     "cbv2_search_f32": (ctypes.c_int, [_p, _p, _i32, _i32, _i32, _i32, _p, _sz, _p, _p, _p, _p]),
     "cbv2_search_f32_begin": (ctypes.c_int, [_p, _p, _i32, _i32, _i32, _i32, _p, _sz, _p, _p, _p, _p, _p]),
diff --git a/hybrid-rag-colbertv2_amd/csrc/colbert_mi355x.hip b/hybrid-rag-colbertv2_amd/csrc/colbert_mi355x.hip
--- a/hybrid-rag-colbertv2_amd/csrc/colbert_mi355x.hip
+++ b/hybrid-rag-colbertv2_amd/csrc/colbert_mi355x.hip
@@ -3513,6 +3513,7 @@
 
 constexpr float kBoundUp = 1.0f + 1.0f / 1024.0f;
 constexpr float kAccSlack = 1.0f / 4096.0f;
+constexpr float kGammaUp = (1.0f + 1.0f / 256.0f) * (1.0f + 1.0f / 256.0f);
 
 __device__ __forceinline__ void split_row8(const float* __restrict__ src, uint16_t* __restrict__ hi,
                                            uint16_t* __restrict__ lo, int sub, float& xx, float& rr, float& hh) {
@@ -3588,8 +3589,11 @@
                                                           int* __restrict__ ctr = nullptr, int nctr = 0,
                                                           uint32_t ready_seq = 0, int nrows = 0,
                                                           uint32_t* __restrict__ zkeys = nullptr, int64_t nz = 0,
-                                                          int32_t* __restrict__ ready_words = nullptr) {
+                                                          int32_t* __restrict__ ready_words = nullptr,
+                                                          float* __restrict__ gamma = nullptr,
+                                                          int32_t* __restrict__ exits = nullptr) {
   __shared__ float s_t[kLqMax];
+  __shared__ float s_g[kLqMax];
   const int b = blockIdx.x, tid = threadIdx.x, r = tid >> 4, sub = tid & 15;
   if (nrows > 0 && b >= nrows) {
     const int64_t per = kSplitZeroInts, i0 = (int64_t)(b - nrows) * per;
@@ -3607,7 +3611,10 @@
     split_row8(Q + row * kDim, qhi + row * kDim, qlo + row * kDim, sub, xx, rr, hh);
     const float nq = sqrtf(xx) * kBoundUp, eq = sqrtf(rr) * kBoundUp;
     const float t = nq * E + eq * M + kAccSlack * (nq + eq) * M;
-    if (sub == 0) s_t[r] = t;
+    if (sub == 0) {
+      s_t[r] = t;
+      s_g[r] = kGammaUp * nq * E + kAccSlack * (nq + eq) * M;
+    }
   }
   __syncthreads();
   if (tid == 0) {
@@ -3618,6 +3625,15 @@
       for (int rr = g; rr < lq; rr += 4) a[g] += s_t[rr];
     }
     beta[b] = ((a[0] + a[1]) + (a[2] + a[3])) * kBoundUp;
+    if (gamma != nullptr) {
+#pragma unroll
+      for (int g = 0; g < 4; ++g) {
+        a[g] = 0.0f;
+        for (int rr = g; rr < lq; rr += 4) a[g] += s_g[rr];
+      }
+      gamma[b] = ((a[0] + a[1]) + (a[2] + a[3])) * kBoundUp;
+    }
+    if (exits != nullptr) exits[b] = 0;
     if (count != nullptr) count[b] = count0;
     if (lbu != nullptr) lbu[b] = 0xffffffffu;
     if (done != nullptr) done[b] = 0;
@@ -3783,6 +3799,94 @@
   __syncthreads();
   return v;
 }
+
+__device__ __forceinline__ void tile16_hi2(const bf16x8 (&ah)[4], const bf16x8 (&qh)[2][4], const bf16x8 (&ql)[2][4],
+                                           const f32x4& init, float (&m)[2]) {
+#pragma unroll
+  for (int ct = 0; ct < 2; ++ct) {
+    f32x4 acc = init;
+#pragma unroll
+    for (int s = 0; s < 4; ++s) acc = __builtin_amdgcn_mfma_f32_16x16x32_bf16(ah[s], ql[ct][s], acc, 0, 0, 0);
+#pragma unroll
+    for (int s = 0; s < 4; ++s) acc = __builtin_amdgcn_mfma_f32_16x16x32_bf16(ah[s], qh[ct][s], acc, 0, 0, 0);
+    m[ct] = fmaxf(fmaxf(m[ct], fmaxf(acc[0], acc[1])), fmaxf(acc[2], acc[3]));
+  }
+}
+
+template <int NW>
+__device__ __forceinline__ float faithful_doc_split_exit(const uint8_t* __restrict__ hi, const uint8_t* __restrict__ lo,
+                                                         int64_t loc, int dl, const bf16x8 (&qh)[2][4],
+                                                         const bf16x8 (&ql)[2][4], int lane, int wave, int lq,
+                                                         float gamma, float lb, float (&s_m)[4][32],
+                                                         float (&s_p)[4][32], bool& exited) {
+  constexpr int TPW = 8 / NW;
+  const int g = lane >> 4, c16 = lane & 15;
+  const size_t at = (size_t)loc * kLd * kRowBytes;
+  bf16x8 ah[TPW][4];
+#pragma unroll
+  for (int t = 0; t < TPW; ++t) gbl_afrag16(hi + at, TPW * wave + t, lane, ah[t]);
+  dl = dl < 0 ? 0 : (dl > kLd ? kLd : dl);
+  float p[2] = {neg_inf(), neg_inf()};
+#pragma unroll
+  for (int t = 0; t < TPW; ++t) {
+    const int rt = TPW * wave + t;
+    if (16 * rt < dl) {
+      const f32x4 init = (dl >= 16 * rt + 16) ? f32x4{} : row_mask_init16(16 * rt + 4 * g, dl);
+      tile16_hi2(ah[t], qh, ql, init, p);
+    }
+  }
+  const float u0 = fold16_max(fold32_max(p[0])), u1 = fold16_max(fold32_max(p[1]));
+  if (lane < 16) {
+    s_p[wave][lane] = u0;
+    s_p[wave][16 + lane] = u1;
+  }
+  __syncthreads();
+  float p0 = s_p[0][c16], p1 = s_p[0][16 + c16];
+#pragma unroll
+  for (int w = 1; w < NW; ++w) {
+    p0 = fmaxf(p0, s_p[w][c16]);
+    p1 = fmaxf(p1, s_p[w][16 + c16]);
+  }
+  const float P = dpp_row_sum16((c16 < lq ? p0 : 0.0f) + (16 + c16 < lq ? p1 : 0.0f));
+  exited = __builtin_amdgcn_readfirstlane((int)(P + gamma < lb)) != 0;
+  if (exited) return neg_inf();
+  bf16x8 al[TPW][4];
+#pragma unroll
+  for (int t = 0; t < TPW; ++t) gbl_afrag16(lo + at, TPW * wave + t, lane, al[t]);
+  float m[2] = {neg_inf(), neg_inf()};
+#pragma unroll
+  for (int t = 0; t < TPW; ++t) {
+    const int rt = TPW * wave + t;
+    if (16 * rt < dl) {
+      const f32x4 init = (dl >= 16 * rt + 16) ? f32x4{} : row_mask_init16(16 * rt + 4 * g, dl);
+      tile16_x3(ah[t], al[t], qh, ql, init, m);
+    }
+  }
+  const float w0 = fold16_max(fold32_max(m[0])), w1 = fold16_max(fold32_max(m[1]));
+  if (lane < 16) {
+    s_m[wave][lane] = w0;
+    s_m[wave][16 + lane] = w1;
+  }
+  __syncthreads();
+  float v = 0.0f;
+  if (wave == 0) {
+    float m0 = s_m[0][c16], m1 = s_m[0][16 + c16];
+#pragma unroll
+    for (int w = 1; w < NW; ++w) {
+      m0 = fmaxf(m0, s_m[w][c16]);
+      m1 = fmaxf(m1, s_m[w][16 + c16]);
+    }
+    v = dpp_row_sum16((c16 < lq ? m0 : 0.0f) + (16 + c16 < lq ? m1 : 0.0f));
+  }
+  __syncthreads();
+  return v;
+}
+
+struct BandExit {
+  const float* gamma = nullptr;
+  const uint32_t* lbu = nullptr;
+  int32_t* exits = nullptr;
+};
 
 struct RowSelect {
   int mode = 0;
@@ -3886,7 +3990,7 @@
   }
 }
 
-template <bool LONG = false, int NW = 4>
+template <bool LONG = false, int NW = 4, bool EXIT = false>
 __global__ __launch_bounds__(NW * 64, 2) void rescore_split_kernel(
     const uint8_t* __restrict__ hi, const uint8_t* __restrict__ lo, const int32_t* __restrict__ doclens, int64_t n,
     int64_t id_base, const uint16_t* __restrict__ qhi, const uint16_t* __restrict__ qlo, int lq,
@@ -3894,8 +3998,10 @@
     float* __restrict__ out, int64_t ld_out, const int32_t* __restrict__ only_neg, int ld,
     uint32_t* __restrict__ lb_min, int64_t c0, float* __restrict__ fb_T = nullptr, int32_t* __restrict__ fb_done = nullptr,
     int fb_k = 0, float* __restrict__ fb_s = nullptr, int32_t* __restrict__ fb_i = nullptr, RowSelect rs = RowSelect(),
-    TaggedCand tc = TaggedCand()) {
+    TaggedCand tc = TaggedCand(), BandExit be = BandExit()) {
+  static_assert(!(EXIT && LONG), "the early exit is built for 128-slot docs");
   __shared__ float s_m[4][32];
+  __shared__ float s_p[EXIT ? 2 : 1][4][32];
   __shared__ uint64_t sel[kTopkMax];
   __shared__ uint32_t hist[2048];
   __shared__ uint32_t s_bin, s_above, s_bincount, s_cnt;
@@ -3941,6 +4047,12 @@
     bf16x8 qh[2][4], ql[2][4];
     load_qfrag16(qhi, b, b + 1, lq, lane, qh);
     load_qfrag16(qlo, b, b + 1, lq, lane, ql);
+    float ex_gamma = 0.0f, ex_lb = 0.0f;
+    int ex_n = 0, ex_par = 0;
+    if constexpr (EXIT) {
+      ex_gamma = be.gamma[b];
+      ex_lb = u2f(be.lbu[b]);
+    }
     for (int64_t c = c0 + blockIdx.x; c < lim; c += gridDim.x) {
       int64_t id;
       if (tc.w != nullptr) {
@@ -3957,8 +4069,17 @@
       }
       const int64_t loc = id - id_base;
       float v = neg_inf();
-      if (id >= 0 && loc >= 0 && loc < n)
-        v = faithful_doc_split<LONG, NW>(hi, lo, loc, ld, doclens[loc], qh, ql, lane, wave, lq, s_m);
+      if (id >= 0 && loc >= 0 && loc < n) {
+        if constexpr (EXIT) {
+          bool exited;
+          v = faithful_doc_split_exit<NW>(hi, lo, loc, doclens[loc], qh, ql, lane, wave, lq, ex_gamma, ex_lb, s_m,
+                                          s_p[ex_par], exited);
+          ex_par ^= 1;
+          ex_n += exited ? 1 : 0;
+        } else {
+          v = faithful_doc_split<LONG, NW>(hi, lo, loc, ld, doclens[loc], qh, ql, lane, wave, lq, s_m);
+        }
+      }
       if (threadIdx.x == 0) {
         if (rs.mode != kSelNone)
           st_sc1(out + (size_t)b * ld_out + c, v);
@@ -3968,6 +4089,8 @@
         if (lb_min != nullptr) atomicMin(lb_min + b, f2u(v));
       }
     }
+    if constexpr (EXIT)
+      if (threadIdx.x == 0 && ex_n > 0) atomicAdd(be.exits + b, ex_n);
   }
   if (rs.stamps != nullptr && threadIdx.x == 0 && blockIdx.x < kLabWgs)
     rs.stamps[17 + 2 * blockIdx.x] = __builtin_amdgcn_s_memrealtime();
@@ -4371,13 +4494,19 @@
     const int wave = threadIdx.x >> 6, nw = blockDim.x >> 6;
     const int c16 = lane & 15, r4 = lane >> 4;
     const bool vec = (n & 3) == 0 && (reinterpret_cast<uintptr_t>(T) & 15) == 0;
-    for (int64_t g0 = (int64_t)blockIdx.x * 64; g0 < nb; g0 += (int64_t)gridDim.x * 64) {
+    const bool per_wave = (nb + 63) / 64 > (int64_t)gridDim.x;
+    const int64_t gstep = (per_wave ? (int64_t)gridDim.x * nw : (int64_t)gridDim.x) * 64;
+    int64_t g0 = (per_wave ? (int64_t)blockIdx.x * nw + wave : (int64_t)blockIdx.x) * 64;
+    uint32_t key = g0 + lane < nb ? krow[g0 + lane] : 0u;
+    for (; g0 < nb; g0 += gstep) {
       const int64_t kb = g0 + lane;
-      const uint64_t qual = __ballot(kb < nb && krow[kb] >= uthr);
-      uint64_t mine = 0;
+      const uint64_t qual = __ballot(kb < nb && key >= uthr);
+      key = g0 + gstep + lane < nb ? krow[g0 + gstep + lane] : 0u;
+      uint64_t mine = per_wave ? qual : 0;
       int q = 0;
-      for (uint64_t m = qual; m != 0; m &= m - 1, ++q)
-        if (q % nw == wave) mine |= m & (~m + 1);
+      if (!per_wave)
+        for (uint64_t m = qual; m != 0; m &= m - 1, ++q)
+          if (q % nw == wave) mine |= m & (~m + 1);
       while (mine != 0) {
         int64_t i0[4];
 #pragma unroll
@@ -4902,6 +5031,7 @@
   bool band_fused = false;
   bool rescore_split = true;
   bool band_reuse = true;
+  bool band_early_exit = true;
   bool band_block_skip = true;
   int rescore_grid = 0;
   bool dense_docs = false;
@@ -5781,6 +5911,8 @@
   uint16_t* qhi = nullptr;
   uint16_t* qlo = nullptr;
   float* beta = nullptr;
+  float* gamma = nullptr;
+  int32_t* exits = nullptr;
   float* lb = nullptr;
   int32_t* count = nullptr;
   int32_t* done = nullptr;
@@ -5816,7 +5948,11 @@
   w->qhi = (uint16_t*)take(qbytes);
   w->qlo = (uint16_t*)take(qbytes);
   w->beta = (float*)take((size_t)B * sizeof(float));
-  if (op == CBV2_F32_SEARCH) w->lb = (float*)take((size_t)B * sizeof(float));
+  if (op == CBV2_F32_SEARCH) {
+    w->gamma = (float*)take((size_t)B * sizeof(float));
+    w->exits = (int32_t*)take((size_t)B * sizeof(int32_t));
+    w->lb = (float*)take((size_t)B * sizeof(float));
+  }
   if (op == CBV2_F32_RERANK) w->F = (float*)take((size_t)B * cap * sizeof(float));
   if (op != CBV2_F32_SCORE) w->arrive = (int32_t*)take((size_t)kArriveSlots * B * kArriveInts * sizeof(int32_t));
   if (op == CBV2_F32_SEARCH) {
@@ -5896,7 +6032,7 @@
                      ix->resid_max, ix->norm_max, w->beta, w->count, reinterpret_cast<uint32_t*>(w->lb), w->done,
                      count0, w->arrive, kArriveSlots * kArriveInts, zero_ctr ? w->ctr : nullptr,
                      zero_ctr ? kRingInts : 0, publish ? g_split_ready_seq : 0u, B, zkeys, nz,
-                     publish ? g_split_ready_word : nullptr);
+                     publish ? g_split_ready_word : nullptr, w->gamma, w->exits);
   return launch_check("split_query_kernel");
 }
 
@@ -5913,18 +6049,23 @@
                    int64_t limit, int64_t ld_c, float* out, int64_t ld_out, hipStream_t st,
                    const int32_t* only_neg = nullptr, int pw = 0, uint32_t* lb_min = nullptr, int64_t c0 = 0,
                    float* fb_T = nullptr, int32_t* fb_done = nullptr, int fb_k = 0, float* fb_s = nullptr,
-                   int32_t* fb_i = nullptr, const RowSelect& rs = RowSelect(), TaggedCand tc = TaggedCand()) {
+                   int32_t* fb_i = nullptr, const RowSelect& rs = RowSelect(), TaggedCand tc = TaggedCand(),
+                   const BandExit& be = BandExit()) {
   if (limit <= c0 && fb_T == nullptr && rs.mode == kSelNone) return CBV2_OK;
   if (ix->rescore_split) {
     int64_t span = limit - c0;
     if (fb_T != nullptr) span = std::max<int64_t>(span, std::min<int64_t>(ix->n, 256));
     if (span < 1) span = 1;
     const auto [gx, two] = rescore_grid(ix, B, span);
+    const bool exit_hi = be.gamma != nullptr;
+    if (exit_hi && (ix->ld != kLd || be.lbu == nullptr || be.exits == nullptr))
+      return fail(CBV2_EUNSUPPORTED, "the band's early exit needs 128-slot docs, the row bound and the counter");
     auto kern = ix->ld != kLd ? rescore_split_kernel<true, 4>
+                : exit_hi     ? (two ? rescore_split_kernel<false, 2, true> : rescore_split_kernel<false, 4, true>)
                               : (two ? rescore_split_kernel<false, 2> : rescore_split_kernel<false, 4>);
     hipLaunchKernelGGL(kern, dim3(gx, (unsigned)B), dim3(two ? 128 : 256), 0, st, ix->tokens, ix->resid, ix->doclens,
                        ix->n, ix->id_base, w->qhi, w->qlo, lq, cand, count, limit, ld_c, out, ld_out, only_neg,
-                       (int)ix->ld, lb_min, c0, fb_T, fb_done, fb_k, fb_s, fb_i, rs, tc);
+                       (int)ix->ld, lb_min, c0, fb_T, fb_done, fb_k, fb_s, fb_i, rs, tc, be);
     return launch_check("rescore_split_kernel");
   }
   if (c0 != 0 || fb_T != nullptr || rs.mode != kSelNone || tc.w != nullptr)
@@ -6153,7 +6294,7 @@
   hipLaunchKernelGGL(kern, dim3(gx, (unsigned)B), dim3(two ? 128 : 256), 0, st, ix->tokens, ix->resid, ix->doclens,
                      ix->n, (int64_t)0, w->qhi, w->qlo, lq, f->ids, (const int32_t*)nullptr, f->m, (int64_t)0, out,
                      f->m, only_neg, (int)ix->ld, (uint32_t*)nullptr, (int64_t)0, (float*)nullptr,
-                     (int32_t*)nullptr, 0, (float*)nullptr, (int32_t*)nullptr, RowSelect(), TaggedCand());
+                     (int32_t*)nullptr, 0, (float*)nullptr, (int32_t*)nullptr, RowSelect(), TaggedCand(), BandExit());
   return launch_check("rescore_split_kernel (subset)");
 }
 
@@ -6365,7 +6506,7 @@
   hipLaunchKernelGGL(kern, dim3(gx, (unsigned)B), dim3(two ? 128 : 256), 0, st, ix->tokens, ix->resid, ix->doclens,
                      ix->n, (int64_t)0, w->qhi, w->qlo, lq, cand, fb->table + fb_off_count(B), M, M, out, M,
                      (const int32_t*)nullptr, (int)ix->ld, (uint32_t*)nullptr, (int64_t)0, (float*)nullptr,
-                     (int32_t*)nullptr, 0, (float*)nullptr, (int32_t*)nullptr, RowSelect(), TaggedCand());
+                     (int32_t*)nullptr, 0, (float*)nullptr, (int32_t*)nullptr, RowSelect(), TaggedCand(), BandExit());
   return launch_check("rescore_split_kernel (ragged)");
 }
 
@@ -6966,6 +7107,9 @@
       return CBV2_OK;
     case CBV2_OPT_BAND_REUSE:
       ix->band_reuse = value != 0;
+      return CBV2_OK;
+    case CBV2_OPT_BAND_EARLY_EXIT:
+      ix->band_early_exit = value != 0;
       return CBV2_OK;
     case CBV2_OPT_BAND_BLOCK_SKIP:
       ix->band_block_skip = value != 0;
@@ -7168,6 +7312,14 @@
   return f32_ws_layout(ix, op, B, lq, cap, nullptr, &w);
 }
 
+size_t cbv2_f32_band_exits_offset(const cbv2_index* ix, int32_t B, int32_t lq, int32_t cap) {
+  if (!ix || B < 1 || lq < 1 || cap < 0) return 0;
+  F32Ws w;
+  uint8_t* const base = reinterpret_cast<uint8_t*>(uintptr_t(256));
+  f32_ws_layout(ix, CBV2_F32_SEARCH, B, lq, cap, base, &w);
+  return (size_t)(reinterpret_cast<uint8_t*>(w.exits) - base);
+}
+
 int cbv2_score_f32(cbv2_index* ix, const float* Q, int32_t B, int32_t lq, void* ws, size_t wsb, float* out,
                    int64_t ld_out, void* stream) {
   F32Ws w;
@@ -7327,9 +7479,15 @@
       if (g_ids_mirror.w != nullptr) g_ids_mirror_used = true;
       rs.stamps = LAB_STAMPS(3);
     }
+    BandExit be;
+    if (ix->band_early_exit && fb_fused && B > kBandPairMaxB && reuse && ix->ld == kLd) {
+      be.gamma = w.gamma;
+      be.lbu = lbu;
+      be.exits = w.exits;
+    }
     if ((rc = launch_rescore(ix, &w, B, lq, w.cand, w.count, cap, cap, w.F, cap, st, nullptr,
                              B <= kBandPairMaxB ? 1 : 0, nullptr, c0, fb_fused ? w.T : nullptr,
-                             fb_fused ? w.done : nullptr, k, out_scores, out_ids, rs)))
+                             fb_fused ? w.done : nullptr, k, out_scores, out_ids, rs, TaggedCand(), be)))
       return rc;
     if (rs.mode != kSelNone) return CBV2_OK;
   }
diff --git a/hybrid-rag-colbertv2_amd/index.py b/hybrid-rag-colbertv2_amd/index.py
--- a/hybrid-rag-colbertv2_amd/index.py
+++ b/hybrid-rag-colbertv2_amd/index.py
@@ -274,6 +274,7 @@
         self.means: Optional[torch.Tensor] = None
         self._ws: Optional[torch.Tensor] = None
         self._rr_ws: Optional[torch.Tensor] = None
+        self._exits_view: Optional[torch.Tensor] = None
         self._all_filter: Optional[DocFilter] = None
         self._last_filter_batch: Optional[FilterBatch] = None
         h = ctypes.c_void_p()
@@ -334,6 +335,16 @@
         if self._ws is None or self._ws.numel() * 4 < need:
             self._ws = torch.empty(((need + 3) // 4,), dtype=torch.float32, device=self.device)
         return self._ws
+
+    def _note_exits(self, ws: torch.Tensor, B: int, lq: int, cap: int):
+        off = int(_lib.lib().cbv2_f32_band_exits_offset(self._h, B, lq, cap))
+        self._exits_view = ws[off // 4:off // 4 + B].view(torch.int32)
+
+    @property
+    def last_band_exits(self) -> torch.Tensor:
+        if self._exits_view is None:
+            raise RuntimeError("no faithful search has run on this index")
+        return self._exits_view.clone()
 
     @classmethod
     def mxfp8(cls, tokens: torch.Tensor, doclens: torch.Tensor, id_base: int = 0) -> "ColbertIndex":
@@ -676,6 +687,7 @@
                                               ws.numel() * 4, out_s.data_ptr(), out_i.data_ptr(),
                                               status.data_ptr(), _stream_ptr(self.device)))
         self.last_band = status
+        self._note_exits(ws, B, lq, cap)
         return out_s, out_i
 
     def _search_f32_global(self, Qd: torch.Tensor, B: int, lq: int, k: int, lb_reduce, cap: int = BAND_CAP):
@@ -696,6 +708,7 @@
                                             lb.data_ptr(), out_s.data_ptr(), out_i.data_ptr(), status.data_ptr(),
                                             _stream_ptr(self.device)))
         self.last_band = status
+        self._note_exits(ws, B, lq, cap)
         return out_s, out_i
 
     def rerank(self, Q: torch.Tensor, cand: torch.Tensor, k: int):
diff --git a/include/colbert_mi355x.h b/include/colbert_mi355x.h
--- a/include/colbert_mi355x.h
+++ b/include/colbert_mi355x.h
@@ -57,6 +57,7 @@
 #define CBV2_OPT_FILTER_PATH 14
 #define CBV2_OPT_FILTER_BATCH_CHUNK_DOCS 15
 #define CBV2_OPT_FILTER_BAND 16
+#define CBV2_OPT_BAND_EARLY_EXIT 17
 int cbv2_index_set_option(cbv2_index* index, int32_t option, int64_t value);
 int cbv2_index_last_scan_plan(const cbv2_index* index, int64_t* out4);
 int64_t cbv2_search_fused_slots(const cbv2_index* index, int32_t B, int32_t k, int32_t scorer);
@@ -126,6 +127,7 @@
                    float* bounds, void* stream);
 int cbv2_index_attach_residual(cbv2_index* index, const void* lo, float resid_max, float norm_max);
 size_t cbv2_f32_workspace_bytes(const cbv2_index* index, int32_t op, int32_t B, int32_t lq, int32_t cap);
+size_t cbv2_f32_band_exits_offset(const cbv2_index* index, int32_t B, int32_t lq, int32_t cap);
 int cbv2_score_f32(cbv2_index* index, const float* Q, int32_t B, int32_t lq, void* workspace,
                    size_t workspace_bytes, float* out, int64_t ld_out, void* stream);
 int cbv2_search_f32(cbv2_index* index, const float* Q, int32_t B, int32_t lq, int32_t k, int32_t cap,
```

New measurement: 1785 (median of 6 runs). About the same (+0.5%).
